# jiangzhengkai/mxdetection

Hardware: AMD Instinct MI355X
Metric: images/sec (whole node) Faster R-CNN R50-FPN 3x800x1333 (higher is better)
Workload: dtype bf16; 1 GPU; Faster R-CNN ResNet-50-FPN bf16 train step, batch 2/GPU, 3x800x1333 (padded 1344); global_batch=2, parallelism=dp1, frozen=stem+C2, frozen BN folded, optimizer=SGD momentum 0.9 wd 1e-4, launch=hipGraph replay, input=resident, wgrad_side_stream=True, rpn_branch_stream=True, grouped_wgrad=True, filter_prefetch_hints=True, params_trainable=41538304

## Files before the change

### include/mxdet.h

```cpp
#ifndef MXDET_H_
#define MXDET_H_

#include <stddef.h>
#include <stdint.h>

#ifdef __cplusplus
extern "C" {
#endif

#define MXDET_OK 0
#define MXDET_EINVAL (-1)
#define MXDET_ESHAPE (-2)
#define MXDET_EWORKSPACE (-3)
#define MXDET_EHIP (-4)
#define MXDET_ERCCL (-5)

#define MXDET_DTYPE_F32 0
#define MXDET_DTYPE_BF16 1

typedef void* mxdet_stream_t;

const char* mxdet_last_error(void);
const char* mxdet_version(void);

int mxdet_box_iou(const float* boxes_a, int64_t na, const float* boxes_b, int64_t nb, float* out,
                  mxdet_stream_t stream);

int mxdet_generate_anchors(const float* base_anchors, int32_t A, int32_t H, int32_t W, int32_t stride,
                           float* out, mxdet_stream_t stream);

size_t mxdet_nms_batched_workspace_bytes(int32_t B, int32_t n_max);
int mxdet_nms_batched(const float* boxes, const int32_t* counts, const uint8_t* invalid, int32_t B,
                      int32_t n_max, float thresh, int32_t max_keep, int32_t* keep_idx,
                      int32_t* num_keep, void* workspace, size_t workspace_bytes,
                      mxdet_stream_t stream);

size_t mxdet_detection_postprocess_workspace_bytes(int32_t N, int32_t rois_per_image, int32_t num_classes);
int mxdet_detection_postprocess(const void* cls_logits, const void* bbox_pred, int32_t dtype, int32_t ld_cls,
                                int32_t ld_reg, const float* rois, const int32_t* num_rois, const float* im_info,
                                int32_t N, int32_t rois_per_image, int32_t num_classes, const float* means,
                                const float* stds, float score_thresh, float nms_thresh, int32_t max_per_image,
                                float* dets, int32_t* num_dets, void* workspace, size_t workspace_bytes,
                                mxdet_stream_t stream);

int mxdet_soft_nms_batched(const float* boxes, const float* scores, const int32_t* counts, int32_t B, int32_t n_max,
                           int32_t method, float nms_thresh, float sigma, float min_score, int32_t max_keep,
                           int32_t* keep_idx, float* keep_scores, int32_t* num_keep, mxdet_stream_t stream);
int mxdet_detection_postprocess_soft(const void* cls_logits, const void* bbox_pred, int32_t dtype, int32_t ld_cls,
                                     int32_t ld_reg, const float* rois, const int32_t* num_rois, const float* im_info,
                                     int32_t N, int32_t rois_per_image, int32_t num_classes, const float* means,
                                     const float* stds, float score_thresh, float nms_thresh, int32_t max_per_image,
                                     float* dets, int32_t* num_dets, void* workspace, size_t workspace_bytes,
                                     int32_t method, float sigma, mxdet_stream_t stream);

typedef struct {
  int32_t num_levels;
  int32_t A;
  int32_t H[8], W[8], stride[8];
  const void* cls[8];
  const void* reg[8];
  int64_t cls_sn[8], cls_sy[8], cls_sx[8], cls_sa[8];
  int64_t reg_sn[8], reg_sy[8], reg_sx[8], reg_sc[8];
  int32_t dtype;
  int32_t classes;
  const float* base_anchors[8];
} mxdet_pyramid_t;

size_t mxdet_proposal_workspace_bytes(const mxdet_pyramid_t* p, int32_t N, int32_t pre_nms_top_n);
int mxdet_proposal(const mxdet_pyramid_t* p, int32_t N, const float* im_info ,
                   int32_t pre_nms_top_n, int32_t post_nms_top_n, float nms_thresh, float min_size,
                   float* rois, float* roi_scores, int32_t* roi_anchor, int32_t* num_rois,
                   void* workspace, size_t workspace_bytes, mxdet_stream_t stream);

size_t mxdet_anchor_target_workspace_bytes(int32_t N, int64_t A_total, int32_t G_max);
int mxdet_anchor_target(const float* anchors, int64_t A_total, const float* gt_boxes, int32_t N,
                        int32_t G_max, const float* im_info, float fg_thresh, float bg_thresh,
                        float allowed_border, int32_t batch_size, float fg_fraction, uint32_t seed,
                        uint32_t step, const uint32_t* step_dev, uint32_t image_offset, int32_t* labels,
                        int32_t* matched_gt,
                        float* bbox_targets, float* max_iou, void* workspace, size_t workspace_bytes,
                        mxdet_stream_t stream);

size_t mxdet_atss_assign_workspace_bytes(int32_t N, int64_t A_total, int32_t G_max);
int mxdet_atss_assign(const float* anchors, int64_t A_total, const int64_t* level_offsets , int32_t L,
                      const float* gt_boxes, int32_t N, int32_t G_max, int32_t topk,
                      int32_t* labels, int32_t* matched_gt, float* bbox_targets, float* matched_iou ,
                      void* workspace, size_t workspace_bytes, mxdet_stream_t stream);

int mxdet_proposal_target(const float* rois, const int32_t* num_rois, int32_t rois_stride,
                          const float* gt_boxes, int32_t N, int32_t G_max, int32_t rois_per_image,
                          float fg_fraction, float fg_thresh, float bg_hi, float bg_lo,
                          int32_t num_classes, int32_t class_agnostic,
                          const float* means , const float* stds ,
                          uint32_t seed, uint32_t step, const uint32_t* step_dev,
                          uint32_t image_offset, float* out_rois, int32_t* labels,
                          float* bbox_targets, float* bbox_weights, int32_t* matched_gt,
                          int32_t* num_fg, mxdet_stream_t stream);

int mxdet_ohem_roi_score(const void* cls_logits, const void* bbox_pred, int32_t dtype, int32_t ld_cls, int32_t ld_reg,
                         const int32_t* labels, const float* bbox_targets, const float* bbox_weights, const float* rois,
                         const int32_t* matched_gt, const float* gt_boxes, int32_t N, int32_t G_max, int64_t R,
                         int32_t num_classes, int32_t reg_dim, int32_t kind, float sigma, float std_x, float std_y,
                         float std_w, float std_h, float reg_weight, float* score, mxdet_stream_t stream);
size_t mxdet_ohem_select_workspace_bytes(int32_t N, int32_t P);
int mxdet_ohem_select(const float* score, const int32_t* labels, const float* rois, int32_t N, int32_t P, int32_t R,
                      float nms_thresh, int32_t* sel, int32_t* num_sel, int32_t* num_fg, void* workspace,
                      size_t workspace_bytes, mxdet_stream_t stream);
int mxdet_ohem_gather(const int32_t* sel, const float* pool_rois, const int32_t* pool_labels,
                      const int32_t* pool_matched_gt, const float* pool_bbox_targets, const float* pool_bbox_weights,
                      int32_t N, int32_t P, int32_t R, int32_t reg_dim, float* out_rois, int32_t* labels,
                      float* bbox_targets, float* bbox_weights, int32_t* matched_gt, mxdet_stream_t stream);

int mxdet_fpn_level_map(const float* rois, int64_t R, int32_t lvl_min, int32_t lvl_max,
                        int32_t* levels, mxdet_stream_t stream);
typedef struct {
  int32_t num_levels, lvl_min;
  int32_t H[8], W[8];
  float spatial_scale[8];
  void* feat[8];
} mxdet_feat_pyramid_t;
int mxdet_roi_align_fwd(const mxdet_feat_pyramid_t* f, int32_t N, int32_t C, const float* rois,
                        const int32_t* levels, int64_t R, int32_t PH, int32_t PW,
                        int32_t sampling_ratio, uint16_t* out, mxdet_stream_t stream);
int mxdet_roi_align_bwd(const mxdet_feat_pyramid_t* f, int32_t N, int32_t C, const float* rois,
                        const int32_t* levels, int64_t R, int32_t PH, int32_t PW,
                        int32_t sampling_ratio, const uint16_t* grad_out, mxdet_stream_t stream);
size_t mxdet_roi_align_bwd_gather_workspace_bytes(const mxdet_feat_pyramid_t* f, int32_t N, int64_t R);
int mxdet_roi_align_bwd_gather(const mxdet_feat_pyramid_t* f, int32_t N, int32_t C, const float* rois,
                               const int32_t* levels, int64_t R, int32_t PH, int32_t PW, int32_t sampling_ratio,
                               const uint16_t* grad_out, int32_t accumulate, void* workspace, size_t workspace_bytes,
                               mxdet_stream_t stream);
int mxdet_roi_align_bwd_gather_prepare(const mxdet_feat_pyramid_t* f, int32_t N, const float* rois,
                                       const int32_t* levels, int64_t R, int32_t PH, int32_t PW, int32_t sampling_ratio,
                                       void* workspace, size_t workspace_bytes, mxdet_stream_t stream);
int mxdet_roi_align_bwd_gather_prepared(const mxdet_feat_pyramid_t* f, int32_t N, int32_t C, const float* rois,
                                        const int32_t* levels, int64_t R, int32_t PH, int32_t PW, int32_t sampling_ratio,
                                        const uint16_t* grad_out, int32_t accumulate, void* workspace,
                                        size_t workspace_bytes, mxdet_stream_t stream);

typedef struct {
  mxdet_feat_pyramid_t pyr;
  int32_t N, C;
  int32_t PH, PW;
  int32_t sample_per_part;
  float trans_std;
  int32_t modulated;
  int32_t trans_stride, mask_stride;
  int32_t accumulate;
} mxdet_dpool_desc_t;
int mxdet_dpool_fwd(const mxdet_dpool_desc_t* d, const float* rois, const int32_t* levels, int64_t R,
                    const uint16_t* trans, const uint16_t* mask_logit, uint16_t* out, mxdet_stream_t stream);
int mxdet_dpool_bwd_trans(const mxdet_dpool_desc_t* d, const float* rois, const int32_t* levels, int64_t R,
                          const uint16_t* trans, const uint16_t* mask_logit, const uint16_t* dout, uint16_t* d_trans,
                          uint16_t* d_mask, mxdet_stream_t stream);
size_t mxdet_dpool_bwd_feat_workspace_bytes(const mxdet_dpool_desc_t* d, int64_t R);
int mxdet_dpool_bwd_feat(const mxdet_dpool_desc_t* d, const float* rois, const int32_t* levels, int64_t R,
                         const uint16_t* trans, const uint16_t* mask_logit, const uint16_t* dout, void* workspace,
                         size_t workspace_bytes, mxdet_stream_t stream);

int mxdet_smooth_l1_fwd(const float* pred, const float* target, const float* weight, int64_t n,
                        float sigma, float* out, mxdet_stream_t stream);
int mxdet_smooth_l1_bwd(const float* pred, const float* target, const float* weight,
                        const float* grad_out, int64_t n, float sigma, int32_t accumulate,
                        float* grad_pred, mxdet_stream_t stream);

size_t mxdet_loss_workspace_bytes(int64_t n);
int mxdet_focal_loss(const void* logits, int32_t dtype, const int32_t* labels, int64_t n, int32_t C,
                     float alpha, float gamma, float grad_scale, float* loss_out, void* grad_logits,
                     void* workspace, size_t workspace_bytes, mxdet_stream_t stream);

int mxdet_anchor_class_labels(const int32_t* labels, const int32_t* matched_gt, const float* gt_boxes, int32_t N,
                              int64_t A_total, int32_t G_max, int32_t* cls_labels, int32_t* num_fg,
                              mxdet_stream_t stream);
int32_t mxdet_retina_loss_num_partials(int32_t N, int32_t H, int32_t W, int32_t A);
int mxdet_retina_loss_level(const uint16_t* cls, const uint16_t* reg, int32_t N, int32_t H, int32_t W, int32_t A,
                            int32_t C, int32_t ld_cls, int32_t ld_reg, const int32_t* cls_labels,
                            const float* bbox_targets, int64_t A_total, int64_t level_offset, float alpha,
                            float gamma, float sigma, const int32_t* num_fg, float loss_scale, uint16_t* grad_cls,
                            uint16_t* grad_reg, float* partial, mxdet_stream_t stream);

int32_t mxdet_rpn_loss_num_partials(int32_t N, int32_t H, int32_t W);
int mxdet_rpn_loss_level(const uint16_t* head, int32_t N, int32_t H, int32_t W, int32_t A,
                         int32_t Cpad, const int32_t* labels, const float* bbox_targets,
                         int64_t A_total, int64_t level_offset, float sigma, float norm,
                         float loss_scale, uint16_t* grad_head, float* partial,
                         mxdet_stream_t stream);
int mxdet_loss_finalize(const float* partial, int32_t count, int32_t ncomp, float* out,
                        mxdet_stream_t stream);

int mxdet_rcnn_loss(const void* cls_logits, const void* bbox_pred, int32_t dtype, int32_t ld_cls,
                    int32_t ld_reg, const int32_t* labels, const float* bbox_targets,
                    const float* bbox_weights, int64_t R, int32_t num_classes, int32_t reg_dim,
                    float sigma, float norm, float loss_scale, float* loss_out, void* grad_cls,
                    void* grad_reg, void* workspace, size_t workspace_bytes, mxdet_stream_t stream);

#define MXDET_IOU_LOSS_IOU 0
#define MXDET_IOU_LOSS_GIOU 1
#define MXDET_IOU_LOSS_DIOU 2
int mxdet_box_iou_loss(const float* boxes, const float* gt, const void* deltas, int32_t dtype, int32_t ld,
                       const float* weight, int64_t n, int32_t kind, float std_x, float std_y, float std_w, float std_h,
                       float grad_scale, float* loss, void* grad_deltas, mxdet_stream_t stream);
int mxdet_rcnn_loss_iou(const void* cls_logits, const void* bbox_pred, int32_t dtype, int32_t ld_cls, int32_t ld_reg,
                        const int32_t* labels, const float* rois, const int32_t* matched_gt, const float* gt_boxes,
                        int32_t N, int32_t G_max, int64_t R, int32_t num_classes, int32_t reg_dim, int32_t kind,
                        float std_x, float std_y, float std_w, float std_h, float reg_weight, float norm, float loss_scale,
                        float* loss_out, void* grad_cls, void* grad_reg, void* workspace, size_t workspace_bytes,
                        mxdet_stream_t stream);
int mxdet_retina_loss_level_iou(const uint16_t* cls, const uint16_t* reg, int32_t N, int32_t H, int32_t W, int32_t A,
                                int32_t C, int32_t ld_cls, int32_t ld_reg, const int32_t* cls_labels, const float* anchors,
                                const int32_t* matched_gt, const float* gt_boxes, int32_t G_max, int64_t A_total,
                                int64_t level_offset, float alpha, float gamma, int32_t kind, float std_x, float std_y,
                                float std_w, float std_h, float reg_weight, const int32_t* num_fg, float loss_scale,
                                uint16_t* grad_cls, uint16_t* grad_reg, float* partial, mxdet_stream_t stream);

#define MXDET_CLS_LOSS_QFL 1
#define MXDET_CLS_LOSS_VFL 2
int mxdet_quality_focal_loss(const void* logits, int32_t dtype, const int32_t* labels, const float* quality, int64_t n,
                             int32_t C, int32_t cls_kind, float alpha, float gamma, float grad_scale, float* loss_out,
                             void* grad_logits, void* workspace, size_t workspace_bytes, mxdet_stream_t stream);
int mxdet_retina_loss_level_quality(const uint16_t* cls, const uint16_t* reg, int32_t N, int32_t H, int32_t W, int32_t A,
                                    int32_t C, int32_t ld_cls, int32_t ld_reg, const int32_t* cls_labels,
                                    const float* anchors, const int32_t* matched_gt, const float* gt_boxes, int32_t G_max,
                                    int64_t A_total, int64_t level_offset, int32_t cls_kind, float alpha, float gamma,
                                    int32_t kind, float std_x, float std_y, float std_w, float std_h, float reg_weight,
                                    const int32_t* num_fg, float loss_scale, uint16_t* grad_cls, uint16_t* grad_reg,
                                    float* partial, mxdet_stream_t stream);

#define MXDET_CLS_LOSS_FOCAL 0
#define MXDET_REG_MAX_LIMIT 31
int mxdet_box_dist_loss(const float* boxes, const float* gt, const void* logits, int32_t dtype, int32_t ld, int64_t n,
                        int32_t reg_max, float stride, int32_t kind, float reg_weight, float dfl_weight, float grad_scale,
                        float* loss_box, float* loss_dfl, float* quality, void* grad_logits, mxdet_stream_t stream);
int mxdet_retina_loss_level_dfl(const uint16_t* cls, const uint16_t* reg, int32_t N, int32_t H, int32_t W, int32_t A,
                                int32_t C, int32_t ld_cls, int32_t ld_reg, const int32_t* cls_labels, const float* anchors,
                                const int32_t* matched_gt, const float* gt_boxes, int32_t G_max, int64_t A_total,
                                int64_t level_offset, int32_t cls_kind, float alpha, float gamma, int32_t kind,
                                int32_t reg_max, float stride, float reg_weight, float dfl_weight, const int32_t* num_fg,
                                float loss_scale, uint16_t* grad_cls, uint16_t* grad_reg, float* partial,
                                mxdet_stream_t stream);

int mxdet_mask_target(const float* rois, const int32_t* matched_gt, const int32_t* labels,
                      const uint8_t* gt_masks, int64_t R, int32_t G_max, int32_t H, int32_t W, int32_t S,
                      uint8_t* targets, int32_t* cls_out, mxdet_stream_t stream);
int mxdet_pixel_shuffle2(const uint16_t* x, int64_t R, int32_t H, int32_t W, int32_t C, int32_t inverse,
                         uint16_t* y, mxdet_stream_t stream);
int mxdet_pixel_shuffle2_inv_relu(const uint16_t* dy_up, const uint16_t* act, int64_t R, int32_t H, int32_t W, int32_t C,
                                  uint16_t* dx, mxdet_stream_t stream);
size_t mxdet_mask_loss_workspace_bytes(int64_t R, int32_t S);
int mxdet_mask_loss(const uint16_t* logits, const int32_t* cls, const uint8_t* targets, int64_t R, int32_t S,
                    int32_t Cpad, float loss_scale, float* loss_out, uint16_t* grad, void* workspace,
                    size_t workspace_bytes, mxdet_stream_t stream);
size_t mxdet_mask_paste_workspace_bytes(int64_t R, int32_t S);
int mxdet_mask_paste(const uint16_t* logits, const float* dets, int64_t R, int32_t S, int32_t Cpad, int32_t H, int32_t W,
                     float thresh, uint8_t* masks, void* workspace, size_t workspace_bytes, mxdet_stream_t stream);
size_t mxdet_maskiou_target_workspace_bytes(int32_t N, int32_t G);
int mxdet_maskiou_target(const float* rois, const int32_t* matched_gt, const int32_t* cls, const float* gt_boxes,
                         const uint8_t* gt_masks, const uint16_t* logits, const uint8_t* targets, int64_t R, int32_t N,
                         int32_t G, int32_t G_boxes, int32_t H, int32_t W, int32_t S, int32_t Cpad, float* out,
                         void* workspace, size_t workspace_bytes, mxdet_stream_t stream);
int mxdet_maskiou_input(const uint16_t* mpooled, const uint16_t* logits, const int32_t* cls, int64_t R, int32_t S,
                        int32_t C, int32_t Cpad, int32_t Ctot, uint16_t* out, mxdet_stream_t stream);
int mxdet_maskiou_input_bwd(const uint16_t* d_in, int64_t pixels, int32_t C, int32_t Ctot, uint16_t* d_mpooled,
                            mxdet_stream_t stream);
int mxdet_maskiou_loss(const uint16_t* pred, const int32_t* cls, const float* targets, int64_t R, int32_t ld,
                       float loss_scale, float weight, float* loss_out, uint16_t* grad, mxdet_stream_t stream);
int mxdet_maskiou_score(const float* dets, const uint16_t* pred, int64_t R, int32_t ld, float* scores,
                        mxdet_stream_t stream);

int mxdet_keypoint_target(const float* rois, const int32_t* matched_gt, const int32_t* labels, const float* gt_keypoints,
                          int64_t R, int32_t N, int32_t G, int32_t K, int32_t S_in, int32_t* targets, mxdet_stream_t stream);
size_t mxdet_keypoint_loss_workspace_bytes(int64_t R);
int mxdet_keypoint_loss(const uint16_t* logits, const int32_t* targets, int64_t R, int32_t S_in, int32_t Kpad, int32_t K,
                        float loss_scale, float weight, float* loss_out, uint16_t* grad, void* workspace,
                        size_t workspace_bytes, mxdet_stream_t stream);
int mxdet_keypoint_decode(const uint16_t* logits, const float* dets, int64_t R, int32_t S_in, int32_t Kpad, int32_t K,
                          float* out, mxdet_stream_t stream);

typedef struct {
  int32_t N, H, W, Cin;
  int32_t Cout, KH, KW;
  int32_t stride, pad;
  int32_t Ho, Wo;
  int32_t relu;
  int32_t res_upsample;
  int32_t accumulate;
  const void* prefetch;
  int64_t prefetch_bytes;
  void* relu_bits;
} mxdet_conv_desc_t;

int mxdet_conv2d_fwd(const mxdet_conv_desc_t* d, const uint16_t* x, const uint16_t* w,
                     const float* bias, const uint16_t* residual, uint16_t* y,
                     mxdet_stream_t stream);
int mxdet_conv2d_fwd_chain(const mxdet_conv_desc_t* d, const uint16_t* x, const uint16_t* w, const float* bias,
                           const uint16_t* w2, const float* bias2, int32_t cout2, int32_t relu2,
                           const uint16_t* residual2, uint16_t* y2, const uint16_t* w3, const float* bias3,
                           int32_t cout3, int32_t relu3, uint16_t* y3, mxdet_stream_t stream);
size_t mxdet_conv2d_fwd_splitk_workspace_bytes(const mxdet_conv_desc_t* d, int32_t ksplit);
int mxdet_conv2d_fwd_splitk(const mxdet_conv_desc_t* d, const uint16_t* x, const uint16_t* w, const float* bias,
                            const uint16_t* residual, uint16_t* y, int32_t ksplit, void* workspace,
                            size_t workspace_bytes, mxdet_stream_t stream);
int mxdet_conv2d_dgrad(const mxdet_conv_desc_t* d, const uint16_t* dy, const uint16_t* wt,
                       const uint16_t* residual, const uint16_t* relu_mask, uint16_t* dx,
                       mxdet_stream_t stream);
size_t mxdet_conv2d_wgrad_workspace_bytes(const mxdet_conv_desc_t* d);
int mxdet_conv2d_wgrad(const mxdet_conv_desc_t* d, const uint16_t* x, const uint16_t* dy, float* dw,
                       float* db, void* workspace, size_t workspace_bytes, mxdet_stream_t stream);
typedef struct {
  mxdet_conv_desc_t desc;
  const void* src;
  const void* filt;
  const float* bias;
  const void* residual;
  const void* relu_mask;
  void* dst;
} mxdet_conv_item_t;
size_t mxdet_conv2d_grouped_table_bytes(int32_t n);
int mxdet_conv2d_grouped_plan(const mxdet_conv_item_t* items, int32_t n, int32_t kind, void* table_host,
                              size_t table_bytes, int32_t* cfg, int32_t* grid);
int mxdet_conv2d_grouped(const void* table_dev, int32_t n, int32_t kind, int32_t cfg, int32_t grid,
                         mxdet_stream_t stream);
typedef struct {
  mxdet_conv_desc_t desc;
  const void* x;
  const void* dy;
  float* dw;
  float* db;
} mxdet_wgrad_item_t;
size_t mxdet_conv2d_wgrad_grouped_table_bytes(int32_t n);
int mxdet_conv2d_wgrad_grouped_plan(const mxdet_wgrad_item_t* items, int32_t n, void* table_host, size_t table_bytes,
                                    size_t* workspace_bytes, int32_t* grid_wgrad, int32_t* grid_big,
                                    int32_t* grid_reduce);
int mxdet_conv2d_wgrad_grouped(const void* table_dev, int32_t n, int32_t grid_wgrad, int32_t grid_big,
                               int32_t grid_reduce, void* workspace, size_t workspace_bytes, size_t workspace_needed,
                               mxdet_stream_t stream);
int mxdet_conv2d_wgrad_grouped_parts(const void* table_dev, int32_t n, int32_t grid_wgrad, int32_t grid_big,
                                     int32_t grid_reduce, int32_t parts, void* workspace, size_t workspace_bytes,
                                     size_t workspace_needed, mxdet_stream_t stream);
int mxdet_filter_transpose(const uint16_t* w, int32_t Cout, int32_t KH, int32_t KW, int32_t Cin,
                           uint16_t* wt, mxdet_stream_t stream);

int mxdet_filter_transpose_batched(const void* descs_dev, int32_t ndesc, int32_t total_tiles,
                                   mxdet_stream_t stream);

#define MXDET_RPN_SPARSE_MAX_LEVELS 8
#define MXDET_RPN_SPARSE_ZERO 1
#define MXDET_RPN_SPARSE_DT 2
#define MXDET_RPN_SPARSE_WGRAD 4
#define MXDET_RPN_SPARSE_DGRAD 8
#define MXDET_RPN_SPARSE_DTMAP 16
#define MXDET_RPN_SPARSE_WGRAD_ORDERED 32
#define MXDET_RPN_ORDERED_WORK_INTS(smax) (10 * (smax) + 32)
typedef struct {
  int32_t kind;
  int32_t H, W;
  int32_t halves_per_slab;
  int32_t slab0;
  int32_t fold_ksplit;
  int32_t bias_pixels;
  int32_t bias_splits;
} mxdet_rpn_ordered_item_t;
typedef struct {
  int32_t num_levels, N, A, C, Ch, smax;
  int32_t H[MXDET_RPN_SPARSE_MAX_LEVELS], W[MXDET_RPN_SPARSE_MAX_LEVELS];
  int32_t accumulate[MXDET_RPN_SPARSE_MAX_LEVELS];
  const void* P[MXDET_RPN_SPARSE_MAX_LEVELS];
  const void* t[MXDET_RPN_SPARSE_MAX_LEVELS];
  const void* tbits[MXDET_RPN_SPARSE_MAX_LEVELS];
  const void* gh[MXDET_RPN_SPARSE_MAX_LEVELS];
  void* dP[MXDET_RPN_SPARSE_MAX_LEVELS];
  void* dt[MXDET_RPN_SPARSE_MAX_LEVELS];
  const mxdet_rpn_ordered_item_t* ordered;
  void* ordered_work;
} mxdet_rpn_sparse_t;
int mxdet_rpn_sparse_list(const mxdet_rpn_sparse_t* d, const int32_t* labels, int32_t* list, int32_t* state,
                          int32_t* map, mxdet_stream_t stream);
int mxdet_rpn_sparse_backward(const mxdet_rpn_sparse_t* d, const int32_t* list, const int32_t* state,
                              const int32_t* map, const uint16_t* wt_out, const uint16_t* wt_conv, uint16_t* dts,
                              uint16_t* ghs, float* dw_out, float* db_out, float* dw_conv, float* db_conv,
                              int32_t parts, mxdet_stream_t stream);
int mxdet_rpn_ordered_schedule(const void* table_host, int32_t n, int32_t num_levels, mxdet_rpn_ordered_item_t* items);

typedef struct {
  int32_t N, H, W, C;
  int32_t Ho, Wo;
  int32_t KH, KW;
  int32_t stride, pad;
  int32_t groups;
  int32_t modulated;
  int32_t off_channels;
  int32_t accumulate;
} mxdet_deform_desc_t;
int mxdet_deform_im2col(const mxdet_deform_desc_t* d, const uint16_t* x, const uint16_t* off, uint16_t* col,
                        mxdet_stream_t stream);
int mxdet_deform_col2im_coord(const mxdet_deform_desc_t* d, const uint16_t* x, const uint16_t* off,
                              const uint16_t* dcol, uint16_t* doff, mxdet_stream_t stream);
size_t mxdet_deform_col2im_workspace_bytes(const mxdet_deform_desc_t* d);
int mxdet_deform_col2im(const mxdet_deform_desc_t* d, const uint16_t* off, const uint16_t* dcol, uint16_t* dx,
                        void* workspace, size_t workspace_bytes, mxdet_stream_t stream);

typedef struct {
  int32_t N, HW, C, G;
  float eps;
  int32_t relu;
  int32_t accumulate;
} mxdet_gn_desc_t;
size_t mxdet_group_norm_workspace_bytes(const mxdet_gn_desc_t* d, int32_t backward);
int mxdet_group_norm_fwd(const mxdet_gn_desc_t* d, const uint16_t* x, const float* gamma, const float* beta, uint16_t* y,
                         float* mean, float* rstd, void* workspace, size_t workspace_bytes, mxdet_stream_t stream);
int mxdet_group_norm_bwd(const mxdet_gn_desc_t* d, const uint16_t* x, const uint16_t* dy, const uint16_t* y,
                         const float* mean, const float* rstd, const float* gamma, const float* beta, uint16_t* dx,
                         float* dgamma, float* dbeta, void* workspace, size_t workspace_bytes, mxdet_stream_t stream);

int mxdet_stem_conv7x7(const void* image, int32_t dtype, int32_t N, int32_t H, int32_t W,
                       const uint16_t* w, const float* bias, uint16_t* y, mxdet_stream_t stream);
int mxdet_stem_conv7x7_pool(const void* image, int32_t dtype, int32_t N, int32_t H, int32_t W,
                            const uint16_t* w, const float* bias, uint16_t* y, mxdet_stream_t stream);
int mxdet_maxpool3x3s2(const uint16_t* x, int32_t N, int32_t H, int32_t W, int32_t C, uint16_t* y,
                       mxdet_stream_t stream);
int mxdet_subsample2(const uint16_t* x, int32_t N, int32_t H, int32_t W, int32_t C, uint16_t* y,
                     mxdet_stream_t stream);
int mxdet_subsample2_bwd(const uint16_t* dy, int32_t N, int32_t H, int32_t W, int32_t C,
                         int32_t accumulate, uint16_t* dx, mxdet_stream_t stream);
int mxdet_upsample2_bwd(const uint16_t* dfine, int32_t N, int32_t Hf, int32_t Wf, int32_t C,
                        int32_t accumulate, uint16_t* dcoarse, mxdet_stream_t stream);
size_t mxdet_retina_detect_workspace_bytes(const mxdet_pyramid_t* p, int32_t N, int32_t pre_nms_top_n);
int mxdet_retina_detect(const mxdet_pyramid_t* p, int32_t N, const float* im_info, int32_t pre_nms_top_n,
                        float score_thresh, float nms_thresh, int32_t max_per_image, float* dets, int32_t* num_dets,
                        void* workspace, size_t workspace_bytes, mxdet_stream_t stream);
int mxdet_retina_detect_soft(const mxdet_pyramid_t* p, int32_t N, const float* im_info, int32_t pre_nms_top_n,
                             float score_thresh, float nms_thresh, int32_t max_per_image, float* dets,
                             int32_t* num_dets, void* workspace, size_t workspace_bytes, int32_t method, float sigma,
                             mxdet_stream_t stream);
int mxdet_retina_detect_dfl(const mxdet_pyramid_t* p, int32_t N, const float* im_info, int32_t pre_nms_top_n,
                            float score_thresh, float nms_thresh, int32_t max_per_image, float* dets, int32_t* num_dets,
                            void* workspace, size_t workspace_bytes, int32_t method, float sigma, int32_t reg_max,
                            mxdet_stream_t stream);

typedef struct {
  const uint8_t* src;
  int32_t src_h, src_w;
  int32_t dst_h, dst_w;
  int32_t flip;
  int32_t pad_;
  double inv_scale;
} mxdet_image_desc_t;
#define MXDET_PREPROCESS_MAX_BATCH 64
int mxdet_image_preprocess(const mxdet_image_desc_t* images , int32_t N, int32_t Hp, int32_t Wp,
                           const float* mean3 , const float* std3 , int32_t swap_rb,
                           uint16_t* out, mxdet_stream_t stream);

int mxdet_polygon_masks(const float* verts, const int32_t* poly_start, const int32_t* inst_first, int32_t N,
                        int32_t G, int32_t H, int32_t W, uint8_t* masks, mxdet_stream_t stream);

int mxdet_add_bf16(const uint16_t* a, const uint16_t* b, int64_t n, uint16_t* out,
                   mxdet_stream_t stream);
int mxdet_relu_bwd_bf16(const uint16_t* dy, const uint16_t* y, int64_t n, uint16_t* dx,
                        mxdet_stream_t stream);
int mxdet_f32_to_bf16(const float* x, int64_t n, uint16_t* y, mxdet_stream_t stream);
int mxdet_f32_accum_to_bf16(const float* x, int64_t n, int32_t accumulate, uint16_t* y,
                            mxdet_stream_t stream);
int mxdet_nchw_to_nhwc_bf16(const void* x, int32_t dtype, int32_t N, int32_t C, int32_t H, int32_t W,
                            uint16_t* y, mxdet_stream_t stream);
int mxdet_nhwc_to_nchw_f32(const uint16_t* x, int32_t N, int32_t C, int32_t H, int32_t W, float* y,
                           mxdet_stream_t stream);

int mxdet_sgd_momentum_update(float* w, const float* grad, float* mom, uint16_t* w_bf16, int64_t n,
                              float lr, float momentum, float wd, float rescale,
                              mxdet_stream_t stream);
int mxdet_sgd_momentum_update_sched(float* w, const float* grad, float* mom, uint16_t* w_bf16, int64_t n,
                                    const float* lr_dev, float momentum, float wd, float rescale,
                                    mxdet_stream_t stream);

typedef struct mxdet_comm mxdet_comm_t;
#define MXDET_COMM_ID_BYTES 128
#define MXDET_COMM_MAX_INFLIGHT 64
int mxdet_comm_unique_id(uint8_t* id );
int mxdet_comm_create(const uint8_t* id, int32_t world, int32_t rank, mxdet_comm_t** comm_out);
int mxdet_comm_destroy(mxdet_comm_t* comm);
int mxdet_allreduce_bucket(mxdet_comm_t* comm, float* grad, int64_t count, mxdet_stream_t stream,
                           int32_t* ticket_out);
int mxdet_comm_wait(mxdet_comm_t* comm, int32_t ticket, mxdet_stream_t stream);
int mxdet_comm_broadcast(mxdet_comm_t* comm, void* buf, size_t bytes, int32_t root, mxdet_stream_t stream);

#ifdef __cplusplus
}
#endif
#endif
```

### mxdetection_amd/_lib.py

```python
import ctypes as C
import os

_HERE = os.path.dirname(os.path.abspath(__file__))
LIB_PATH = os.environ.get("MXDET_LIB") or os.path.join(_HERE, "libmxdet_hip.so")

c_i32, c_i64, c_u32, c_f32, c_sz, c_vp = C.c_int32, C.c_int64, C.c_uint32, C.c_float, C.c_size_t, C.c_void_p


class PyramidT(C.Structure):
    _fields_ = [
        ("num_levels", c_i32), ("A", c_i32),
        ("H", c_i32 * 8), ("W", c_i32 * 8), ("stride", c_i32 * 8),
        ("cls", c_vp * 8), ("reg", c_vp * 8),
        ("cls_sn", c_i64 * 8), ("cls_sy", c_i64 * 8), ("cls_sx", c_i64 * 8), ("cls_sa", c_i64 * 8),
        ("reg_sn", c_i64 * 8), ("reg_sy", c_i64 * 8), ("reg_sx", c_i64 * 8), ("reg_sc", c_i64 * 8),
        ("dtype", c_i32), ("classes", c_i32),
        ("base_anchors", c_vp * 8),
    ]


class FeatPyramidT(C.Structure):
    _fields_ = [
        ("num_levels", c_i32), ("lvl_min", c_i32),
        ("H", c_i32 * 8), ("W", c_i32 * 8),
        ("spatial_scale", c_f32 * 8),
        ("feat", c_vp * 8),
    ]


class ImageDescT(C.Structure):
    _fields_ = [("src", C.c_void_p), ("src_h", C.c_int32), ("src_w", C.c_int32), ("dst_h", C.c_int32),
                ("dst_w", C.c_int32), ("flip", C.c_int32), ("pad_", C.c_int32), ("inv_scale", C.c_double)]


class WgradItemT(C.Structure):
    pass


class ConvItemT(C.Structure):
    pass


class ConvDescT(C.Structure):
    _fields_ = [
        ("N", c_i32), ("H", c_i32), ("W", c_i32), ("Cin", c_i32),
        ("Cout", c_i32), ("KH", c_i32), ("KW", c_i32),
        ("stride", c_i32), ("pad", c_i32),
        ("Ho", c_i32), ("Wo", c_i32),
        ("relu", c_i32), ("res_upsample", c_i32), ("accumulate", c_i32),
        ("prefetch", c_vp), ("prefetch_bytes", c_i64), ("relu_bits", c_vp),
    ]


class DeformDescT(C.Structure):
    _fields_ = [
        ("N", c_i32), ("H", c_i32), ("W", c_i32), ("C", c_i32),
        ("Ho", c_i32), ("Wo", c_i32), ("KH", c_i32), ("KW", c_i32),
        ("stride", c_i32), ("pad", c_i32), ("groups", c_i32), ("modulated", c_i32),
        ("off_channels", c_i32), ("accumulate", c_i32),
    ]


class DpoolDescT(C.Structure):
    _fields_ = [
        ("pyr", FeatPyramidT), ("N", c_i32), ("C", c_i32), ("PH", c_i32), ("PW", c_i32),
        ("sample_per_part", c_i32), ("trans_std", c_f32), ("modulated", c_i32),
        ("trans_stride", c_i32), ("mask_stride", c_i32), ("accumulate", c_i32),
    ]


class GnDescT(C.Structure):
    _fields_ = [("N", c_i32), ("HW", c_i32), ("C", c_i32), ("G", c_i32), ("eps", c_f32), ("relu", c_i32),
                ("accumulate", c_i32)]


class RpnOrderedItemT(C.Structure):
    _fields_ = [("kind", c_i32), ("H", c_i32), ("W", c_i32), ("halves_per_slab", c_i32), ("slab0", c_i32),
                ("fold_ksplit", c_i32), ("bias_pixels", c_i32), ("bias_splits", c_i32)]


class RpnSparseT(C.Structure):
    _fields_ = [("num_levels", c_i32), ("N", c_i32), ("A", c_i32), ("C", c_i32), ("Ch", c_i32), ("smax", c_i32),
                ("H", c_i32 * 8), ("W", c_i32 * 8), ("accumulate", c_i32 * 8),
                ("P", c_vp * 8), ("t", c_vp * 8), ("tbits", c_vp * 8), ("gh", c_vp * 8), ("dP", c_vp * 8), ("dt", c_vp * 8),
                ("ordered", C.POINTER(RpnOrderedItemT)), ("ordered_work", c_vp)]


WgradItemT._fields_ = [("desc", ConvDescT), ("x", c_vp), ("dy", c_vp), ("dw", c_vp), ("db", c_vp)]
ConvItemT._fields_ = [("desc", ConvDescT), ("src", c_vp), ("filt", c_vp), ("bias", c_vp), ("residual", c_vp),
                      ("relu_mask", c_vp), ("dst", c_vp)]

P = C.POINTER

SIGNATURES = {
    "mxdet_last_error": (C.c_char_p, []),
    "mxdet_version": (C.c_char_p, []),
    "mxdet_box_iou": (c_i32, [c_vp, c_i64, c_vp, c_i64, c_vp, c_vp]),
    "mxdet_generate_anchors": (c_i32, [c_vp, c_i32, c_i32, c_i32, c_i32, c_vp, c_vp]),
    "mxdet_nms_batched_workspace_bytes": (c_sz, [c_i32, c_i32]),
    "mxdet_nms_batched": (c_i32, [c_vp, c_vp, c_vp, c_i32, c_i32, c_f32, c_i32, c_vp, c_vp, c_vp, c_sz, c_vp]),
    "mxdet_soft_nms_batched": (c_i32, [c_vp, c_vp, c_vp, c_i32, c_i32, c_i32, c_f32, c_f32, c_f32, c_i32, c_vp, c_vp, c_vp,
                                       c_vp]),
    "mxdet_pixel_shuffle2_inv_relu": (c_i32, [c_vp, c_vp, c_i64, c_i32, c_i32, c_i32, c_vp, c_vp]),
    "mxdet_mask_paste_workspace_bytes": (c_sz, [c_i64, c_i32]),
    "mxdet_mask_paste": (c_i32, [c_vp, c_vp, c_i64, c_i32, c_i32, c_i32, c_i32, c_f32, c_vp, c_vp, c_sz, c_vp]),
    "mxdet_retina_detect_workspace_bytes": (c_sz, [c_vp, c_i32, c_i32]),
    "mxdet_retina_detect": (c_i32, [c_vp, c_i32, c_vp, c_i32, c_f32, c_f32, c_i32, c_vp, c_vp, c_vp, c_sz, c_vp]),
    "mxdet_retina_detect_soft": (c_i32, [c_vp, c_i32, c_vp, c_i32, c_f32, c_f32, c_i32, c_vp, c_vp, c_vp, c_sz, c_i32, c_f32,
                                         c_vp]),
    "mxdet_retina_detect_dfl": (c_i32, [c_vp, c_i32, c_vp, c_i32, c_f32, c_f32, c_i32, c_vp, c_vp, c_vp, c_sz, c_i32, c_f32,
                                        c_i32, c_vp]),
    "mxdet_debug_preprocess_direct": (c_i32, [c_i32]),
    "mxdet_image_preprocess": (c_i32, [c_vp, c_i32, c_i32, c_i32, c_vp, c_vp, c_i32, c_vp, c_vp]),
    "mxdet_polygon_masks": (c_i32, [c_vp, c_vp, c_vp, c_i32, c_i32, c_i32, c_i32, c_vp, c_vp]),
    "mxdet_detection_postprocess_workspace_bytes": (c_sz, [c_i32, c_i32, c_i32]),
    "mxdet_detection_postprocess": (c_i32, [c_vp, c_vp, c_i32, c_i32, c_i32, c_vp, c_vp, c_vp, c_i32, c_i32, c_i32,
                                            P(c_f32), P(c_f32), c_f32, c_f32, c_i32, c_vp, c_vp, c_vp, c_sz, c_vp]),
    "mxdet_detection_postprocess_soft": (c_i32, [c_vp, c_vp, c_i32, c_i32, c_i32, c_vp, c_vp, c_vp, c_i32, c_i32, c_i32,
                                                 P(c_f32), P(c_f32), c_f32, c_f32, c_i32, c_vp, c_vp, c_vp, c_sz, c_i32,
                                                 c_f32, c_vp]),
    "mxdet_proposal_workspace_bytes": (c_sz, [P(PyramidT), c_i32, c_i32]),
    "mxdet_proposal": (c_i32, [P(PyramidT), c_i32, c_vp, c_i32, c_i32, c_f32, c_f32, c_vp, c_vp, c_vp, c_vp,
                               c_vp, c_sz, c_vp]),
    "mxdet_anchor_target_workspace_bytes": (c_sz, [c_i32, c_i64, c_i32]),
    "mxdet_anchor_target": (c_i32, [c_vp, c_i64, c_vp, c_i32, c_i32, c_vp, c_f32, c_f32, c_f32, c_i32, c_f32,
                                    c_u32, c_u32, c_vp, c_u32, c_vp, c_vp, c_vp, c_vp, c_vp, c_sz, c_vp]),
    "mxdet_atss_assign_workspace_bytes": (c_sz, [c_i32, c_i64, c_i32]),
    "mxdet_atss_assign": (c_i32, [c_vp, c_i64, P(c_i64), c_i32, c_vp, c_i32, c_i32, c_i32, c_vp, c_vp, c_vp, c_vp, c_vp, c_sz,
                                  c_vp]),
    "mxdet_proposal_target": (c_i32, [c_vp, c_vp, c_i32, c_vp, c_i32, c_i32, c_i32, c_f32, c_f32, c_f32, c_f32,
                                      c_i32, c_i32, P(c_f32), P(c_f32), c_u32, c_u32, c_vp, c_u32, c_vp, c_vp, c_vp,
                                      c_vp, c_vp, c_vp, c_vp]),
    "mxdet_ohem_roi_score": (c_i32, [c_vp, c_vp, c_i32, c_i32, c_i32, c_vp, c_vp, c_vp, c_vp, c_vp, c_vp, c_i32, c_i32, c_i64,
                                     c_i32, c_i32, c_i32, c_f32, c_f32, c_f32, c_f32, c_f32, c_f32, c_vp, c_vp]),
    "mxdet_ohem_select_workspace_bytes": (c_sz, [c_i32, c_i32]),
    "mxdet_ohem_select": (c_i32, [c_vp, c_vp, c_vp, c_i32, c_i32, c_i32, c_f32, c_vp, c_vp, c_vp, c_vp, c_sz, c_vp]),
    "mxdet_ohem_gather": (c_i32, [c_vp, c_vp, c_vp, c_vp, c_vp, c_vp, c_i32, c_i32, c_i32, c_i32, c_vp, c_vp, c_vp, c_vp,
                                  c_vp, c_vp]),
    "mxdet_fpn_level_map": (c_i32, [c_vp, c_i64, c_i32, c_i32, c_vp, c_vp]),
    "mxdet_roi_align_fwd": (c_i32, [P(FeatPyramidT), c_i32, c_i32, c_vp, c_vp, c_i64, c_i32, c_i32, c_i32, c_vp,
                                    c_vp]),
    "mxdet_roi_align_bwd": (c_i32, [P(FeatPyramidT), c_i32, c_i32, c_vp, c_vp, c_i64, c_i32, c_i32, c_i32, c_vp,
                                    c_vp]),
    "mxdet_roi_align_bwd_gather_workspace_bytes": (c_sz, [P(FeatPyramidT), c_i32, c_i64]),
    "mxdet_roi_align_bwd_gather": (c_i32, [P(FeatPyramidT), c_i32, c_i32, c_vp, c_vp, c_i64, c_i32, c_i32, c_i32, c_vp,
                                           c_i32, c_vp, c_sz, c_vp]),
    "mxdet_roi_align_bwd_gather_prepare": (c_i32, [P(FeatPyramidT), c_i32, c_vp, c_vp, c_i64, c_i32, c_i32, c_i32,
                                                   c_vp, c_sz, c_vp]),
    "mxdet_roi_align_bwd_gather_prepared": (c_i32, [P(FeatPyramidT), c_i32, c_i32, c_vp, c_vp, c_i64, c_i32, c_i32, c_i32,
                                                    c_vp, c_i32, c_vp, c_sz, c_vp]),
    "mxdet_smooth_l1_fwd": (c_i32, [c_vp, c_vp, c_vp, c_i64, c_f32, c_vp, c_vp]),
    "mxdet_smooth_l1_bwd": (c_i32, [c_vp, c_vp, c_vp, c_vp, c_i64, c_f32, c_i32, c_vp, c_vp]),
    "mxdet_loss_workspace_bytes": (c_sz, [c_i64]),
    "mxdet_focal_loss": (c_i32, [c_vp, c_i32, c_vp, c_i64, c_i32, c_f32, c_f32, c_f32, c_vp, c_vp, c_vp, c_sz,
                                 c_vp]),
    "mxdet_anchor_class_labels": (c_i32, [c_vp, c_vp, c_vp, c_i32, c_i64, c_i32, c_vp, c_vp, c_vp]),
    "mxdet_retina_loss_num_partials": (c_i32, [c_i32, c_i32, c_i32, c_i32]),
    "mxdet_retina_loss_level": (c_i32, [c_vp, c_vp, c_i32, c_i32, c_i32, c_i32, c_i32, c_i32, c_i32, c_vp, c_vp, c_i64,
                                        c_i64, c_f32, c_f32, c_f32, c_vp, c_f32, c_vp, c_vp, c_vp, c_vp]),
    "mxdet_rpn_loss_num_partials": (c_i32, [c_i32, c_i32, c_i32]),
    "mxdet_rpn_loss_level": (c_i32, [c_vp, c_i32, c_i32, c_i32, c_i32, c_i32, c_vp, c_vp, c_i64, c_i64, c_f32,
                                     c_f32, c_f32, c_vp, c_vp, c_vp]),
    "mxdet_loss_finalize": (c_i32, [c_vp, c_i32, c_i32, c_vp, c_vp]),
    "mxdet_rcnn_loss": (c_i32, [c_vp, c_vp, c_i32, c_i32, c_i32, c_vp, c_vp, c_vp, c_i64, c_i32, c_i32, c_f32,
                                c_f32, c_f32, c_vp, c_vp, c_vp, c_vp, c_sz, c_vp]),
    "mxdet_box_iou_loss": (c_i32, [c_vp, c_vp, c_vp, c_i32, c_i32, c_vp, c_i64, c_i32, c_f32, c_f32, c_f32, c_f32, c_f32, c_vp,
                                   c_vp, c_vp]),
    "mxdet_rcnn_loss_iou": (c_i32, [c_vp, c_vp, c_i32, c_i32, c_i32, c_vp, c_vp, c_vp, c_vp, c_i32, c_i32, c_i64, c_i32, c_i32,
                                    c_i32, c_f32, c_f32, c_f32, c_f32, c_f32, c_f32, c_f32, c_vp, c_vp, c_vp, c_vp, c_sz,
                                    c_vp]),
    "mxdet_retina_loss_level_iou": (c_i32, [c_vp, c_vp, c_i32, c_i32, c_i32, c_i32, c_i32, c_i32, c_i32, c_vp, c_vp, c_vp, c_vp,
                                            c_i32, c_i64, c_i64, c_f32, c_f32, c_i32, c_f32, c_f32, c_f32, c_f32, c_f32, c_vp,
                                            c_f32, c_vp, c_vp, c_vp, c_vp]),
    "mxdet_quality_focal_loss": (c_i32, [c_vp, c_i32, c_vp, c_vp, c_i64, c_i32, c_i32, c_f32, c_f32, c_f32, c_vp, c_vp, c_vp, c_sz,
                                         c_vp]),
    "mxdet_retina_loss_level_quality": (c_i32, [c_vp, c_vp, c_i32, c_i32, c_i32, c_i32, c_i32, c_i32, c_i32, c_vp, c_vp, c_vp,
                                                c_vp, c_i32, c_i64, c_i64, c_i32, c_f32, c_f32, c_i32, c_f32, c_f32, c_f32, c_f32,
                                                c_f32, c_vp, c_f32, c_vp, c_vp, c_vp, c_vp]),
    "mxdet_box_dist_loss": (c_i32, [c_vp, c_vp, c_vp, c_i32, c_i32, c_i64, c_i32, c_f32, c_i32, c_f32, c_f32, c_f32, c_vp, c_vp,
                                    c_vp, c_vp, c_vp]),
    "mxdet_retina_loss_level_dfl": (c_i32, [c_vp, c_vp, c_i32, c_i32, c_i32, c_i32, c_i32, c_i32, c_i32, c_vp, c_vp, c_vp, c_vp,
                                            c_i32, c_i64, c_i64, c_i32, c_f32, c_f32, c_i32, c_i32, c_f32, c_f32, c_f32, c_vp,
                                            c_f32, c_vp, c_vp, c_vp, c_vp]),
    "mxdet_mask_target": (c_i32, [c_vp, c_vp, c_vp, c_vp, c_i64, c_i32, c_i32, c_i32, c_i32, c_vp, c_vp, c_vp]),
    "mxdet_pixel_shuffle2": (c_i32, [c_vp, c_i64, c_i32, c_i32, c_i32, c_i32, c_vp, c_vp]),
    "mxdet_mask_loss_workspace_bytes": (c_sz, [c_i64, c_i32]),
    "mxdet_mask_loss": (c_i32, [c_vp, c_vp, c_vp, c_i64, c_i32, c_i32, c_f32, c_vp, c_vp, c_vp, c_sz, c_vp]),
    "mxdet_maskiou_target_workspace_bytes": (c_sz, [c_i32, c_i32]),
    "mxdet_maskiou_target": (c_i32, [c_vp, c_vp, c_vp, c_vp, c_vp, c_vp, c_vp, c_i64, c_i32, c_i32, c_i32, c_i32, c_i32, c_i32,
                                     c_i32, c_vp, c_vp, c_sz, c_vp]),
    "mxdet_maskiou_input": (c_i32, [c_vp, c_vp, c_vp, c_i64, c_i32, c_i32, c_i32, c_i32, c_vp, c_vp]),
    "mxdet_maskiou_input_bwd": (c_i32, [c_vp, c_i64, c_i32, c_i32, c_vp, c_vp]),
    "mxdet_maskiou_loss": (c_i32, [c_vp, c_vp, c_vp, c_i64, c_i32, c_f32, c_f32, c_vp, c_vp, c_vp]),
    "mxdet_maskiou_score": (c_i32, [c_vp, c_vp, c_i64, c_i32, c_vp, c_vp]),
    "mxdet_keypoint_target": (c_i32, [c_vp, c_vp, c_vp, c_vp, c_i64, c_i32, c_i32, c_i32, c_i32, c_vp, c_vp]),
    "mxdet_keypoint_loss_workspace_bytes": (c_sz, [c_i64]),
    "mxdet_keypoint_loss": (c_i32, [c_vp, c_vp, c_i64, c_i32, c_i32, c_i32, c_f32, c_f32, c_vp, c_vp, c_vp, c_sz, c_vp]),
    "mxdet_keypoint_decode": (c_i32, [c_vp, c_vp, c_i64, c_i32, c_i32, c_i32, c_vp, c_vp]),
    "mxdet_conv2d_fwd": (c_i32, [P(ConvDescT), c_vp, c_vp, c_vp, c_vp, c_vp, c_vp]),
    "mxdet_conv2d_fwd_chain": (c_i32, [P(ConvDescT), c_vp, c_vp, c_vp, c_vp, c_vp, c_i32, c_i32, c_vp, c_vp, c_vp, c_vp, c_i32,
                                       c_i32, c_vp, c_vp]),
    "mxdet_conv2d_fwd_splitk_workspace_bytes": (c_sz, [P(ConvDescT), c_i32]),
    "mxdet_conv2d_fwd_splitk": (c_i32, [P(ConvDescT), c_vp, c_vp, c_vp, c_vp, c_vp, c_i32, c_vp, c_sz, c_vp]),
    "mxdet_conv2d_dgrad": (c_i32, [P(ConvDescT), c_vp, c_vp, c_vp, c_vp, c_vp, c_vp]),
    "mxdet_conv2d_wgrad_workspace_bytes": (c_sz, [P(ConvDescT)]),
    "mxdet_conv2d_wgrad": (c_i32, [P(ConvDescT), c_vp, c_vp, c_vp, c_vp, c_vp, c_sz, c_vp]),
    "mxdet_conv2d_grouped_table_bytes": (c_sz, [c_i32]),
    "mxdet_conv2d_grouped_plan": (c_i32, [P(ConvItemT), c_i32, c_i32, c_vp, c_sz, P(c_i32), P(c_i32)]),
    "mxdet_conv2d_grouped": (c_i32, [c_vp, c_i32, c_i32, c_i32, c_i32, c_vp]),
    "mxdet_conv2d_wgrad_grouped_table_bytes": (c_sz, [c_i32]),
    "mxdet_conv2d_wgrad_grouped_plan": (c_i32, [P(WgradItemT), c_i32, c_vp, c_sz, P(c_sz), P(c_i32), P(c_i32), P(c_i32)]),
    "mxdet_conv2d_wgrad_grouped": (c_i32, [c_vp, c_i32, c_i32, c_i32, c_i32, c_vp, c_sz, c_sz, c_vp]),
    "mxdet_conv2d_wgrad_grouped_parts": (c_i32, [c_vp, c_i32, c_i32, c_i32, c_i32, c_i32, c_vp, c_sz, c_sz, c_vp]),
    "mxdet_debug_force_conv_cfg": (c_i32, [c_i32]),
    "mxdet_debug_force_wgrad_ksplit": (c_i32, [c_i32]),
    "mxdet_rpn_sparse_list": (c_i32, [P(RpnSparseT), c_vp, c_vp, c_vp, c_vp, c_vp]),
    "mxdet_rpn_sparse_backward": (c_i32, [P(RpnSparseT), c_vp, c_vp, c_vp, c_vp, c_vp, c_vp, c_vp, c_vp, c_vp, c_vp, c_vp,
                                          c_i32, c_vp]),
    "mxdet_rpn_ordered_schedule": (c_i32, [c_vp, c_i32, c_i32, P(RpnOrderedItemT)]),
    "mxdet_filter_transpose": (c_i32, [c_vp, c_i32, c_i32, c_i32, c_i32, c_vp, c_vp]),
    "mxdet_filter_transpose_batched": (c_i32, [c_vp, c_i32, c_i32, c_vp]),
    "mxdet_deform_im2col": (c_i32, [P(DeformDescT), c_vp, c_vp, c_vp, c_vp]),
    "mxdet_deform_col2im_coord": (c_i32, [P(DeformDescT), c_vp, c_vp, c_vp, c_vp, c_vp]),
    "mxdet_deform_col2im_workspace_bytes": (c_sz, [P(DeformDescT)]),
    "mxdet_deform_col2im": (c_i32, [P(DeformDescT), c_vp, c_vp, c_vp, c_vp, c_sz, c_vp]),
    "mxdet_dpool_fwd": (c_i32, [P(DpoolDescT), c_vp, c_vp, c_i64, c_vp, c_vp, c_vp, c_vp]),
    "mxdet_dpool_bwd_trans": (c_i32, [P(DpoolDescT), c_vp, c_vp, c_i64, c_vp, c_vp, c_vp, c_vp, c_vp, c_vp]),
    "mxdet_dpool_bwd_feat_workspace_bytes": (c_sz, [P(DpoolDescT), c_i64]),
    "mxdet_dpool_bwd_feat": (c_i32, [P(DpoolDescT), c_vp, c_vp, c_i64, c_vp, c_vp, c_vp, c_vp, c_sz, c_vp]),
    "mxdet_group_norm_workspace_bytes": (c_sz, [P(GnDescT), c_i32]),
    "mxdet_group_norm_fwd": (c_i32, [P(GnDescT), c_vp, c_vp, c_vp, c_vp, c_vp, c_vp, c_vp, c_sz, c_vp]),
    "mxdet_group_norm_bwd": (c_i32, [P(GnDescT), c_vp, c_vp, c_vp, c_vp, c_vp, c_vp, c_vp, c_vp, c_vp, c_vp, c_vp, c_sz,
                                     c_vp]),
    "mxdet_debug_group_norm_route": (c_i32, [P(GnDescT)]),
    "mxdet_stem_conv7x7": (c_i32, [c_vp, c_i32, c_i32, c_i32, c_i32, c_vp, c_vp, c_vp, c_vp]),
    "mxdet_stem_conv7x7_pool": (c_i32, [c_vp, c_i32, c_i32, c_i32, c_i32, c_vp, c_vp, c_vp, c_vp]),
    "mxdet_maxpool3x3s2": (c_i32, [c_vp, c_i32, c_i32, c_i32, c_i32, c_vp, c_vp]),
    "mxdet_subsample2": (c_i32, [c_vp, c_i32, c_i32, c_i32, c_i32, c_vp, c_vp]),
    "mxdet_subsample2_bwd": (c_i32, [c_vp, c_i32, c_i32, c_i32, c_i32, c_i32, c_vp, c_vp]),
    "mxdet_upsample2_bwd": (c_i32, [c_vp, c_i32, c_i32, c_i32, c_i32, c_i32, c_vp, c_vp]),
    "mxdet_add_bf16": (c_i32, [c_vp, c_vp, c_i64, c_vp, c_vp]),
    "mxdet_relu_bwd_bf16": (c_i32, [c_vp, c_vp, c_i64, c_vp, c_vp]),
    "mxdet_f32_to_bf16": (c_i32, [c_vp, c_i64, c_vp, c_vp]),
    "mxdet_f32_accum_to_bf16": (c_i32, [c_vp, c_i64, c_i32, c_vp, c_vp]),
    "mxdet_nchw_to_nhwc_bf16": (c_i32, [c_vp, c_i32, c_i32, c_i32, c_i32, c_i32, c_vp, c_vp]),
    "mxdet_nhwc_to_nchw_f32": (c_i32, [c_vp, c_i32, c_i32, c_i32, c_i32, c_vp, c_vp]),
    "mxdet_sgd_momentum_update": (c_i32, [c_vp, c_vp, c_vp, c_vp, c_i64, c_f32, c_f32, c_f32, c_f32, c_vp]),
    "mxdet_sgd_momentum_update_sched": (c_i32, [c_vp, c_vp, c_vp, c_vp, c_i64, c_vp, c_f32, c_f32, c_f32, c_vp]),
    "mxdet_comm_unique_id": (c_i32, [c_vp]),
    "mxdet_comm_create": (c_i32, [c_vp, c_i32, c_i32, P(c_vp)]),
    "mxdet_comm_destroy": (c_i32, [c_vp]),
    "mxdet_allreduce_bucket": (c_i32, [c_vp, c_vp, c_i64, c_vp, P(c_i32)]),
    "mxdet_comm_wait": (c_i32, [c_vp, c_i32, c_vp]),
    "mxdet_comm_broadcast": (c_i32, [c_vp, c_vp, c_sz, c_i32, c_vp]),
    "mxdet_debug_set_tuning": (c_i32, [c_i32, c_i64]),
    "mxdet_debug_get_tuning": (c_i64, [c_i32]),
    "mxdet_debug_route_probe": (c_i32, [c_i32]),
    "mxdet_debug_route_read": (c_i32, [P(c_i32), c_i32]),
}

DEBUG_SYMBOLS = ("mxdet_debug_force_conv_cfg", "mxdet_debug_force_wgrad_ksplit", "mxdet_debug_preprocess_direct",
                 "mxdet_debug_set_tuning", "mxdet_debug_get_tuning", "mxdet_debug_route_probe", "mxdet_debug_route_read",
                 "mxdet_debug_group_norm_route")
TUNING_KEYS = {"T64": 0, "T128": 1, "PAR64": 2, "WG_TARGET": 3, "WG_MINSTEPS": 4, "WG_MAXSTEPS": 5, "T3_ENABLE": 6,
               "T3_TARGET": 7, "T3_MINSTEPS": 8, "T3_NS": 9, "TAIL": 10, "WG_NS": 11, "ROI_TABLE": 12, "ROI_ROWS": 13, "STATIC_TAPS": 14,
               "T128W": 15, "T3_MIX": 16, "SPLITK_TILE": 17, "T3_PER_ITEM": 18}
ROUTE_KINDS = {"CONV": 1, "WGRAD": 2, "CONV_GROUPED": 3, "WGRAD_GROUPED": 4, "RETINA_LOSS": 5, "RETINA_LOSS_IOU": 6,
               "RETINA_LOSS_QUALITY": 7, "RETINA_LOSS_DFL": 8}

IOU_LOSS_KINDS = {"iou": 0, "giou": 1, "diou": 2}
CLS_LOSS_KINDS = {"qfl": 1, "vfl": 2}
CLS_LOSS_KINDS_DFL = {"focal": 0, "qfl": 1, "vfl": 2}
REG_MAX_LIMIT = 31

_lib = None


class MxdetError(RuntimeError):
    pass


def load():
    global _lib
    if _lib is not None:
        return _lib
    if not os.path.exists(LIB_PATH):
        raise MxdetError(
            "libmxdet_hip.so not found at %s -- build it with `python -m mxdetection_amd.build` "
            "(there is no CPU fallback)" % LIB_PATH)
    import torch
    lib = C.CDLL(LIB_PATH)
    for name, (res, args) in SIGNATURES.items():
        fn = getattr(lib, name, None)
        if fn is None:
            continue
        fn.restype = res
        fn.argtypes = args
    _lib = lib
    for key, idx in TUNING_KEYS.items():
        v = os.environ.get("MXDET_TUNE_" + key)
        if v:
            lib.mxdet_debug_set_tuning(idx, int(v))
    return lib


def check(rc, what=""):
    if rc != 0:
        msg = load().mxdet_last_error().decode("utf-8", "replace")
        raise MxdetError("%s failed (%d): %s" % (what or "mxdet call", rc, msg))


def ptr(t):
    return None if t is None else C.c_void_p(t.data_ptr())


def stream_ptr():
    import torch
    return C.c_void_p(torch.cuda.current_stream().cuda_stream)
```

### mxdetection_amd/csrc/conv.hip

```cpp
#include <stdlib.h>

#include "common.h"

namespace mxdet {

struct ConvP {
  const uint16_t* x;
  const uint16_t* w;
  const float* bias;
  const uint16_t* res;
  const uint16_t* mask;
  uint16_t* y;
  int N, Hs, Ws, C;
  int Hd, Wd, Ncols;
  int KH, KW, stride, pad;
  int relu, res_up;
  int M;
  int tiles_m, tiles_n;
  int par_tile0[5];
  int par_hc[2], par_wc[2];
  int par_h0[2], par_w0[2];
  int m_begin;
  int ksplit;
  float* partial;
  const void* pf;
  long long pf_bytes;
  unsigned char* bits_out;
  const unsigned char* bits_in;
  int force_cfg;
  const uint16_t* chain_w;
  const float* chain_bias;
  const uint16_t* chain_res;
  uint16_t* chain_y;
  int chain_relu;
  const uint16_t* chain3_w;
  const float* chain3_bias;
  uint16_t* chain3_y;
  int chain3_relu;
};

__device__ __forceinline__ int lds_off(int row, int chunk) {
  return row * 64 + ((chunk ^ ((row >> 1) & 7)) << 3);
}

#ifdef MXDET_CONV_STAMP
__device__ unsigned long long g_conv_stamp[2][8];
#define MXDET_CS(k) do { if (cs_on) cs[k] = __builtin_amdgcn_s_memtime(); } while (0)
#else
#define MXDET_CS(k) do { } while (0)
#endif

template <int BM, int BN, int WM, int WN, int NS, bool DGRAD, bool PAR = false, int TAPS = 0, int CHAIN = 0>
__device__ __forceinline__ void conv_igemm_tile(const ConvP& p, int bid, const int nwg) {
  constexpr int NW = WM * WN, NTHR = 64 * NW;
  constexpr int WTM = BM / WM, WTN = BN / WN;
  constexpr int MT = WTM / 16, NT = WTN / 16;
  constexpr int RPI = 8;
  constexpr int GA = BM / RPI / NW, GB = BN / RPI / NW;
  constexpr int STAGE = (BM + BN) * 64;
  static_assert(BM % (RPI * NW) == 0 && BN % (RPI * NW) == 0, "rows must split evenly over the waves");
  static_assert(MT % 2 == 0, "epilogue stages two m-tiles at a time");
  static_assert(NS >= 2 && (NS - 2) * (GA + GB) <= 63, "vmcnt is a 6-bit counter");
  static_assert(TAPS == 0 || ((TAPS == 1 || TAPS == 9) && !PAR), "static taps: 1x1 or 3x3");
  constexpr int EP_STRIDE = WTN + 4;
  constexpr int EP_BYTES = NW * 32 * EP_STRIDE * 4;
  constexpr int MAIN_BYTES = NS * STAGE * 2;
  static_assert(CHAIN == 0 || (TAPS == 9 && !DGRAD && WN == 1 && BN == 64 && CHAIN % (8 * NW) == 0),
                "chain: forward 3x3 whose waves own all 64 mid channels of their rows");
  constexpr int CHAIN_OFF = MAIN_BYTES > EP_BYTES ? MAIN_BYTES : EP_BYTES;
  constexpr int SMEM_BYTES = CHAIN_OFF + CHAIN * 128;
  __shared__ __attribute__((aligned(1024))) unsigned char smem_raw[SMEM_BYTES];
  uint16_t* smem = (uint16_t*)smem_raw;

  const int tid = threadIdx.x, lane = tid & 63;
  const int wid = __builtin_amdgcn_readfirstlane(tid >> 6);
  const int wm = wid / WN, wn = wid % WN;
#ifdef MXDET_CONV_STAMP
  const bool cs_on = (blockIdx.x == 0 || blockIdx.x == 300) && wid == 0;
  unsigned long long cs[8] = {0, 0, 0, 0, 0, 0, 0, 0};
#endif
  MXDET_CS(0);

  const int pf_bid = bid, pf_nwg = nwg;
  int ks = 0, sl_begin = 0, sl_end = p.C >> 6;
  int nwg_ = nwg;
  if constexpr (TAPS == 1) {
    if (p.ksplit > 1) {
      const int tiles = p.tiles_m * p.tiles_n;
      ks = bid / tiles;
      bid -= ks * tiles;
      nwg_ = tiles;
      const int per = ((p.C >> 6) + p.ksplit - 1) / p.ksplit;
      sl_begin = ks * per;
      sl_end = sl_begin + per < sl_end ? sl_begin + per : sl_end;
      sl_end = sl_end < sl_begin ? sl_begin : sl_end;
    }
  }
  if constexpr (!PAR) {
    bid = xcd_tile_order(bid, nwg_);
  }
  const int tile_m = bid / p.tiles_n, tile_n = bid - tile_m * p.tiles_n;
  int m0 = p.m_begin + tile_m * BM;
  const int n0 = tile_n * BN;
  int par_ph = 0, par_pw = 0, par_rows = 0, par_hc = 1, par_wc = 1, nkh = p.KH, nkw = p.KW;
  if constexpr (PAR) {
    int c = 0;
    while (c < 3 && tile_m >= p.par_tile0[c + 1]) ++c;
    par_ph = c >> 1; par_pw = c & 1;
    par_hc = p.par_hc[par_ph]; par_wc = p.par_wc[par_pw];
    par_rows = p.N * par_hc * par_wc;
    m0 = (tile_m - p.par_tile0[c]) * BM;
    nkh = (p.KH - par_ph + 1) >> 1; nkw = (p.KW - par_pw + 1) >> 1;
    nkh = nkh < 0 ? 0 : nkh; nkw = nkw < 0 ? 0 : nkw;
  }

  const int lrow = lane >> 3, lslot = lane & 7;
  constexpr int SWZ = 7;
  const __amdgpu_buffer_rsrc_t rsrc_x = make_rsrc(p.x, 2u * (unsigned)(p.N * p.Hs * p.Ws) * (unsigned)p.C);
  const __amdgpu_buffer_rsrc_t rsrc_w = make_rsrc(p.w, 2u * (unsigned)p.Ncols * (unsigned)(p.KH * p.KW * p.C));
  const int ntaps = p.KH * p.KW;
  const int hw_d = p.Hd * p.Wd;
  const bool smallm = p.M < (1 << 24);
  const float rcp_hw = 1.0f / (float)hw_d, rcp_w = 1.0f / (float)p.Wd;
  const int Ktot = ntaps * p.C;
  const int KT = PAR ? (nkh * nkw * p.C) >> 6 : Ktot >> 6;
  int wrow[GB];
#pragma unroll
  for (int i = 0; i < GB; ++i) {
    int rb = (wid * GB + i) * RPI + lrow;
    int n = n0 + rb;
    n = n < p.Ncols ? n : p.Ncols - 1;
    wrow[i] = n * Ktot + ((lslot ^ ((rb >> 1) & SWZ)) << 3);
  }
  auto issue_b = [&](int buf, int tap, int c0, bool live) {
    const int so_b = live ? 2 * (tap * p.C + c0) : 0;
    unsigned char* sbase = smem_raw + (size_t)buf * (STAGE * 2);
#pragma unroll
    for (int i = 0; i < GB; ++i)
#if !defined(MXDET_ABL_NOLOAD) && !defined(MXDET_ABL_NOBLOAD)
      __builtin_amdgcn_raw_ptr_buffer_load_lds(rsrc_w, (lptr_t)(sbase + BM * 128 + (wid * GB + i) * 1024), 16,
                                               (int)(2u * (unsigned)wrow[i]), so_b, 0, 0);
#else
      asm volatile("" ::"v"(wrow[i]), "s"(so_b));
#endif
  };
  if constexpr (TAPS > 0) {
#pragma unroll
    for (int s0 = 0; s0 < NS - 1; ++s0)
      issue_b(s0, s0 % TAPS, (sl_begin + s0 / TAPS) * 64, s0 < (sl_end - sl_begin) * TAPS);
  }
  if constexpr (CHAIN > 0) {
    const __amdgpu_buffer_rsrc_t rsrc_c = make_rsrc(p.chain_w, 2u * (unsigned)CHAIN * 64u);
#pragma unroll
    for (int i = 0; i < CHAIN / 8 / NW; ++i) {
      const int r = (wid * (CHAIN / 8 / NW) + i) * 8 + lrow;
      const unsigned vo = 2u * (unsigned)(r * 64 + ((lslot ^ ((r >> 1) & 7)) << 3));
      __builtin_amdgcn_raw_ptr_buffer_load_lds(rsrc_c, (lptr_t)(smem_raw + CHAIN_OFF + (wid * (CHAIN / 8 / NW) + i) * 1024), 16,
                                               (int)vo, 0, 0, 0);
    }
  }
  int a_off[GA];
  unsigned a_mask[GA];
#pragma unroll
  for (int i = 0; i < GA; ++i) {
    int ra = (wid * GA + i) * RPI + lrow;
    int m = m0 + ra;
    int coff = (lslot ^ ((ra >> 1) & SWZ)) << 3;
    unsigned mask = 0;
    int off = 0;
    if constexpr (PAR) {
      if (m < par_rows) {
        int img = m / (par_hc * par_wc);
        int rem = m - img * (par_hc * par_wc);
        int ih = rem / par_wc, iw = rem - ih * par_wc;
        int hd = p.par_h0[par_ph] + 2 * ih, wd = p.par_w0[par_pw] + 2 * iw;
        int hs0 = (hd + p.pad - par_ph) >> 1, ws0 = (wd + p.pad - par_pw) >> 1;
        off = ((img * p.Hs + hs0) * p.Ws + ws0) * p.C + coff;
        for (int a = 0; a < nkh; ++a)
          for (int b = 0; b < nkw; ++b) {
            int hs = hs0 - a, ws = ws0 - b;
            if (hs >= 0 && ws >= 0 && hs < p.Hs && ws < p.Ws) mask |= 1u << (a * nkw + b);
          }
      }
    } else if (ntaps == 1 && p.stride == 1 && p.pad == 0) {
      if (m < p.M) { off = m * p.C + coff; mask = 1u; }
    } else
    if (m < p.M) {
      int img, hd, wd, rem;
      if (smallm) {
        img = fast_divmod(m, hw_d, rcp_hw, &rem);
        hd = fast_divmod(rem, p.Wd, rcp_w, &wd);
      } else {
        img = m / hw_d; rem = m - img * hw_d;
        hd = rem / p.Wd; wd = rem - hd * p.Wd;
      }
      int h0, w0;
      if (DGRAD) {
        if (p.stride == 1) { h0 = hd + p.pad; w0 = wd + p.pad; }
        else { h0 = (hd + p.pad) / p.stride; w0 = (wd + p.pad) / p.stride; }
      } else { h0 = hd * p.stride - p.pad; w0 = wd * p.stride - p.pad; }
      off = ((img * p.Hs + h0) * p.Ws + w0) * p.C + coff;
      if (DGRAD && p.stride != 1) {
        for (int kh = 0; kh < p.KH; ++kh)
          for (int kw = 0; kw < p.KW; ++kw) {
            int th = hd + p.pad - kh, tw = wd + p.pad - kw;
            int hs = th / p.stride, ws = tw / p.stride;
            bool ok = th >= 0 && tw >= 0 && th == hs * p.stride && tw == ws * p.stride && hs < p.Hs && ws < p.Ws;
            if (ok) mask |= 1u << (kh * p.KW + kw);
          }
      } else if (TAPS == 9) {
        const unsigned rlo = (DGRAD ? h0 < p.Hs : h0 >= 0) ? 1u : 0u, rhi = (DGRAD ? h0 - 2 >= 0 : h0 + 2 < p.Hs) ? 4u : 0u;
        const unsigned clo = (DGRAD ? w0 < p.Ws : w0 >= 0) ? 1u : 0u, chi = (DGRAD ? w0 - 2 >= 0 : w0 + 2 < p.Ws) ? 4u : 0u;
        const unsigned rowm = rlo | 2u | rhi, colm = clo | 2u | chi;
        mask = ((rowm & 1u) ? colm : 0u) | (colm << 3) | ((rowm & 4u) ? colm << 6 : 0u);
      } else {
        unsigned rowm = 0, colm = 0;
        for (int kh = 0; kh < p.KH; ++kh) {
          const int hs = DGRAD ? h0 - kh : h0 + kh;
          if (hs >= 0 && hs < p.Hs) rowm |= 1u << kh;
        }
        for (int kw = 0; kw < p.KW; ++kw) {
          const int ws = DGRAD ? w0 - kw : w0 + kw;
          if (ws >= 0 && ws < p.Ws) colm |= 1u << kw;
        }
        for (int kh = 0; kh < p.KH; ++kh)
          if ((rowm >> kh) & 1u) mask |= colm << (kh * p.KW);
      }
    }
    a_off[i] = off;
    a_mask[i] = mask;
  }

  int ld_kt = 0, ld_kh = 0, ld_kw = 0, ld_c0 = 0;
  auto issue_stage = [&](int buf) {
    unsigned char* sbase = smem_raw + (size_t)buf * (STAGE * 2);
    const bool live = ld_kt < KT;
    int tap, delta, koff;
    if constexpr (PAR) {
      tap = live ? ld_kh * nkw + ld_kw : 31;
      delta = ld_c0 - (ld_kh * p.Ws + ld_kw) * p.C;
      koff = live ? ((par_ph + 2 * ld_kh) * p.KW + (par_pw + 2 * ld_kw)) * p.C + ld_c0 : 0;
    } else {
      tap = live ? ld_kh * p.KW + ld_kw : 31;
      if (DGRAD) delta = ld_c0 - ((ld_kh / p.stride) * p.Ws + (ld_kw / p.stride)) * p.C;
      else delta = ld_c0 + (ld_kh * p.Ws + ld_kw) * p.C;
      koff = live ? (ld_kh * p.KW + ld_kw) * p.C + ld_c0 : 0;
    }
#pragma unroll
    for (int i = 0; i < GA; ++i) {
      unsigned vo = ((a_mask[i] >> tap) & 1u) ? 2u * (unsigned)(a_off[i] + delta) : kDmaOob;
#ifdef MXDET_ABL_ZEROSRC
      vo = kDmaOob;
#endif
#ifndef MXDET_ABL_NOLOAD
      __builtin_amdgcn_raw_ptr_buffer_load_lds(rsrc_x, (lptr_t)(sbase + (wid * GA + i) * 1024), 16, (int)vo, 0, 0, 0);
#else
      asm volatile("" ::"v"(vo));
#endif
    }
#pragma unroll
    for (int i = 0; i < GB; ++i) {
      unsigned wo = 2u * (unsigned)(wrow[i] + koff);
#ifdef MXDET_ABL_ZEROSRC
      wo = kDmaOob;
#endif
#ifndef MXDET_ABL_NOLOAD
      __builtin_amdgcn_raw_ptr_buffer_load_lds(rsrc_w, (lptr_t)(sbase + BM * 128 + (wid * GB + i) * 1024), 16, (int)wo, 0, 0, 0);
#else
      asm volatile("" ::"v"(wo));
#endif
    }
    ++ld_kt;
    if (++ld_kw == nkw) {
      ld_kw = 0;
      if (++ld_kh == nkh) { ld_kh = 0; ld_c0 += 64; }
    }
  };

  f32x4_t acc[MT][NT];
#pragma unroll
  for (int i = 0; i < MT; ++i)
#pragma unroll
    for (int j = 0; j < NT; ++j) acc[i][j] = (f32x4_t){0.f, 0.f, 0.f, 0.f};
  MXDET_CS(1);

  const int frow = lane & 15, fq = lane >> 4;
  if constexpr (TAPS > 0) {
  constexpr int TKW = TAPS == 9 ? 3 : 1;
  constexpr int SL = (NS % TAPS == 0 || TAPS % NS == 0) ? (TAPS % NS == 0 ? 1 : NS) : NS;
  static_assert((SL * TAPS) % NS == 0, "the ring position must repeat with the unrolled block");
  const int bias_el = (p.pad * p.Ws + p.pad) * p.C;
  const int rebase = DGRAD ? ((p.KH - 1) * p.Ws + (p.KW - 1)) * p.C : 0;
  const __amdgpu_buffer_rsrc_t rsrc_xs =
      make_rsrc(p.x - bias_el, 2u * (unsigned)(p.N * p.Hs * p.Ws) * (unsigned)p.C + 2u * (unsigned)bias_el);
  unsigned voa[GA];
#pragma unroll
  for (int i = 0; i < GA; ++i) {
    voa[i] = 2u * (unsigned)(a_off[i] - rebase + bias_el);
    if (TAPS == 1) voa[i] = (a_mask[i] & 1u) ? voa[i] : kDmaOob;
  }
  auto issue_a = [&](int buf, int tap, int c0, bool live) {
    const int kh = tap / TKW, kw = tap % TKW;
    const int disp = DGRAD ? ((p.KH - 1 - kh) * p.Ws + (p.KW - 1 - kw)) * p.C : (kh * p.Ws + kw) * p.C;
    const int so_a = live ? 2 * (disp + c0) : 0;
    unsigned char* sbase = smem_raw + (size_t)buf * (STAGE * 2);
#pragma unroll
    for (int i = 0; i < GA; ++i) {
      unsigned vo = voa[i];
      if (TAPS != 1) vo = ((a_mask[i] >> tap) & 1u) ? vo : kDmaOob;
      if (!live) vo = kDmaOob;
#ifndef MXDET_ABL_NOLOAD
      __builtin_amdgcn_raw_ptr_buffer_load_lds(rsrc_xs, (lptr_t)(sbase + (wid * GA + i) * 1024), 16, (int)vo, so_a, 0, 0);
#else
      asm volatile("" ::"v"(vo), "s"(so_a));
#endif
    }
  };
  const uint16_t* fa0 = smem + lds_off(wm * WTM + frow, fq);
  const uint16_t* fa1 = smem + lds_off(wm * WTM + frow, 4 + fq);
  const uint16_t* fb0 = smem + BM * 64 + lds_off(wn * WTN + frow, fq);
  const uint16_t* fb1 = smem + BM * 64 + lds_off(wn * WTN + frow, 4 + fq);
  const int nslices = sl_end;
#pragma unroll
  for (int s0 = 0; s0 < NS - 1; ++s0)
    issue_a(s0, s0 % TAPS, (sl_begin + s0 / TAPS) * 64, s0 < (sl_end - sl_begin) * TAPS);
  asm volatile("s_waitcnt vmcnt(%0)" ::"n"((NS - 2) * GA) : "memory");
#ifdef MXDET_ABL_NOBFRAG
  bf16x8_t bf0[NT], bf1[NT];
#pragma unroll
  for (int j = 0; j < NT; ++j) { bf0[j] = *(const bf16x8_t*)(fb0 + j * 1024); bf1[j] = *(const bf16x8_t*)(fb1 + j * 1024); }
#endif
#ifdef MXDET_ABL_NOKLOOP
  for (int cs = sl_begin; cs < sl_begin; cs += SL) {
#else
  for (int cs = sl_begin; cs < nslices; cs += SL) {
#endif
#pragma unroll
    for (int sl = 0; sl < SL; ++sl) {
      if (SL > 1 && cs + sl >= nslices) break;
#pragma unroll
      for (int tp = 0; tp < TAPS; ++tp) {
        const int step = sl * TAPS + tp;
        const int cur = step % NS, nxt = (step + NS - 1) % NS;
        asm volatile("s_waitcnt vmcnt(%0)" ::"n"((NS - 2) * (GA + GB)) : "memory");
        __builtin_amdgcn_s_barrier();
        asm volatile("" ::: "memory");
#ifdef MXDET_ABL_NOBFRAG
        bf16x8_t af0[MT], af1[MT];
#else
        bf16x8_t af0[MT], bf0[NT], af1[MT], bf1[NT];
#endif
#pragma unroll
        for (int i = 0; i < MT; ++i) af0[i] = *(const bf16x8_t*)(fa0 + cur * STAGE + i * 1024);
#ifndef MXDET_ABL_NOBFRAG
#pragma unroll
        for (int j = 0; j < NT; ++j) bf0[j] = *(const bf16x8_t*)(fb0 + cur * STAGE + j * 1024);
#endif
#pragma unroll
        for (int i = 0; i < MT; ++i) af1[i] = *(const bf16x8_t*)(fa1 + cur * STAGE + i * 1024);
#ifndef MXDET_ABL_NOBFRAG
#pragma unroll
        for (int j = 0; j < NT; ++j) bf1[j] = *(const bf16x8_t*)(fb1 + cur * STAGE + j * 1024);
#endif
        __builtin_amdgcn_sched_barrier(0);
        {
          const int ahead = tp + NS - 1;
          const int atap = ahead % TAPS, aslice = ahead / TAPS;
          issue_a(nxt, atap, (cs + sl + aslice) * 64, cs + sl + aslice < nslices);
          issue_b(nxt, atap, (cs + sl + aslice) * 64, cs + sl + aslice < nslices);
        }
        __builtin_amdgcn_sched_barrier(0);
        __builtin_amdgcn_s_setprio(1);
#ifndef MXDET_ABL_NOMFMA
#pragma unroll
        for (int i = 0; i < MT; ++i)
#pragma unroll
          for (int j = 0; j < NT; ++j)
            acc[i][j] = __builtin_amdgcn_mfma_f32_16x16x32_bf16(af0[i], bf0[j], acc[i][j], 0, 0, 0);
#pragma unroll
        for (int i = 0; i < MT; ++i)
#pragma unroll
          for (int j = 0; j < NT; ++j)
            acc[i][j] = __builtin_amdgcn_mfma_f32_16x16x32_bf16(af1[i], bf1[j], acc[i][j], 0, 0, 0);
#else
#pragma unroll
        for (int i = 0; i < MT; ++i) { asm volatile("" ::"v"(af0[i])); asm volatile("" ::"v"(af1[i])); }
#pragma unroll
        for (int j = 0; j < NT; ++j) { asm volatile("" ::"v"(bf0[j])); asm volatile("" ::"v"(bf1[j])); }
#endif
        __builtin_amdgcn_sched_barrier(0);
        __builtin_amdgcn_s_setprio(0);
      }
    }
  }
  } else {
#pragma unroll
  for (int s0 = 0; s0 < NS - 1; ++s0) issue_stage(s0);

  int cur = 0, nxt = NS - 1;
  for (int kt = 0; kt < KT; ++kt) {
    asm volatile("s_waitcnt vmcnt(%0)" ::"n"((NS - 2) * (GA + GB)) : "memory");
    __builtin_amdgcn_s_barrier();
    asm volatile("" ::: "memory");
#ifdef MXDET_CONV_STAMP
    if (kt == 0) MXDET_CS(2);
#endif
    const uint16_t* sa = smem + cur * STAGE;
    const uint16_t* sb = sa + BM * 64;
    bf16x8_t af0[MT], bf0[NT], af1[MT], bf1[NT];
#pragma unroll
    for (int i = 0; i < MT; ++i) af0[i] = *(const bf16x8_t*)(sa + lds_off(wm * WTM + i * 16 + frow, fq));
#pragma unroll
    for (int j = 0; j < NT; ++j) bf0[j] = *(const bf16x8_t*)(sb + lds_off(wn * WTN + j * 16 + frow, fq));
    issue_stage(nxt);
    __builtin_amdgcn_s_setprio(1);
    __builtin_amdgcn_sched_barrier(0);
#pragma unroll
    for (int i = 0; i < MT; ++i) af1[i] = *(const bf16x8_t*)(sa + lds_off(wm * WTM + i * 16 + frow, 4 + fq));
#pragma unroll
    for (int j = 0; j < NT; ++j) bf1[j] = *(const bf16x8_t*)(sb + lds_off(wn * WTN + j * 16 + frow, 4 + fq));
#ifndef MXDET_ABL_NOMFMA
#pragma unroll
    for (int i = 0; i < MT; ++i)
#pragma unroll
      for (int j = 0; j < NT; ++j)
        acc[i][j] = __builtin_amdgcn_mfma_f32_16x16x32_bf16(af0[i], bf0[j], acc[i][j], 0, 0, 0);
#pragma unroll
    for (int g = 0; g < MT + NT; ++g) {
      __builtin_amdgcn_sched_group_barrier(0x008, (MT * NT) / (MT + NT), 0);
      __builtin_amdgcn_sched_group_barrier(0x100, 1, 0);
    }
#pragma unroll
    for (int i = 0; i < MT; ++i)
#pragma unroll
      for (int j = 0; j < NT; ++j)
        acc[i][j] = __builtin_amdgcn_mfma_f32_16x16x32_bf16(af1[i], bf1[j], acc[i][j], 0, 0, 0);
#else
#pragma unroll
    for (int i = 0; i < MT; ++i) { asm volatile("" ::"v"(af0[i])); asm volatile("" ::"v"(af1[i])); }
#pragma unroll
    for (int j = 0; j < NT; ++j) { asm volatile("" ::"v"(bf0[j])); asm volatile("" ::"v"(bf1[j])); }
#endif
    __builtin_amdgcn_sched_barrier(0);
    __builtin_amdgcn_s_setprio(0);
    cur = (cur + 1 == NS) ? 0 : cur + 1;
    nxt = (nxt + 1 == NS) ? 0 : nxt + 1;
  }
  }
  MXDET_CS(3);
  asm volatile("s_waitcnt vmcnt(0)" ::: "memory");
  __syncthreads();
  MXDET_CS(4);

  uint4 pfv[4] = {make_uint4(0u, 0u, 0u, 0u), make_uint4(0u, 0u, 0u, 0u), make_uint4(0u, 0u, 0u, 0u), make_uint4(0u, 0u, 0u, 0u)};
  if (p.pf != nullptr) {
    const long long pf_stride = (long long)pf_nwg * NTHR * 16;
    long long off = ((long long)pf_bid * NTHR + tid) * 16;
#pragma unroll
    for (int k = 0; k < 4; ++k, off += pf_stride)
      if (off + 16 <= p.pf_bytes) pfv[k] = *(const uint4*)((const char*)p.pf + off);
  }

  float* ep = (float*)smem_raw + wid * 32 * EP_STRIDE;
  constexpr int LPR = WTN / 8;
  constexpr int RPP = 64 / LPR;
  constexpr int PASSES = 32 / RPP;
  const int rl = lane / LPR, cg = lane - rl * LPR;
  bf16x8_t af2[CHAIN > 0 ? MT : 1][2];
  if constexpr (CHAIN > 0) {
#pragma unroll
    for (int i = 0; i < MT; ++i)
#pragma unroll
      for (int j = 0; j < NT; ++j)
#pragma unroll
        for (int r = 0; r < 4; ++r)
          ep[(i * 16 + fq * 4 + r) * EP_STRIDE + j * 16 + frow] = acc[i][j][r];
#pragma unroll
    for (int hf = 0; hf < 2; ++hf) {
      float4 c0 = make_float4(0.f, 0.f, 0.f, 0.f), c1 = c0;
      if (p.bias) {
        c0 = *(const float4*)(p.bias + hf * 32 + fq * 8);
        c1 = *(const float4*)(p.bias + hf * 32 + fq * 8 + 4);
      }
#pragma unroll
      for (int i = 0; i < MT; ++i) {
        const float4 v0 = *(const float4*)(ep + (i * 16 + frow) * EP_STRIDE + hf * 32 + fq * 8);
        const float4 v1 = *(const float4*)(ep + (i * 16 + frow) * EP_STRIDE + hf * 32 + fq * 8 + 4);
        float v[8] = {v0.x + c0.x, v0.y + c0.y, v0.z + c0.z, v0.w + c0.w, v1.x + c1.x, v1.y + c1.y, v1.z + c1.z, v1.w + c1.w};
        if (p.relu) {
#pragma unroll
          for (int k = 0; k < 8; ++k) v[k] = v[k] > 0.0f ? v[k] : 0.0f;
        }
        af2[i][hf] = __builtin_bit_cast(bf16x8_t, pack8_bf16_hw(v));
      }
    }
  }
  static_assert(CHAIN == 0 || MT == 2, "chain: one epilogue half covers the wave's rows");
  constexpr int NCH = CHAIN > 0 ? CHAIN / BN : 1;
  const bool c3 = CHAIN > 0 && p.chain3_w != nullptr;
  f32x4_t acc3[CHAIN > 0 ? MT : 1][CHAIN > 0 ? NT : 1];
  if constexpr (CHAIN > 0) {
#pragma unroll
    for (int i = 0; i < MT; ++i)
#pragma unroll
      for (int j = 0; j < NT; ++j) acc3[i][j] = f32x4_t{0.f, 0.f, 0.f, 0.f};
  }
#pragma unroll 1
  for (int chunk = 0; chunk < (CHAIN > 0 ? NCH + (c3 ? 1 : 0) : 1); ++chunk) {
  const bool last3 = CHAIN > 0 && chunk == NCH;
  const int e_ncols = CHAIN > 0 ? (last3 ? BN : CHAIN) : p.Ncols;
  const float* const e_bias = CHAIN > 0 ? (last3 ? p.chain3_bias : p.chain_bias) : p.bias;
  const uint16_t* const e_res = CHAIN > 0 ? (last3 ? nullptr : p.chain_res) : p.res;
  uint16_t* const e_y = CHAIN > 0 ? (last3 ? p.chain3_y : p.chain_y) : p.y;
  const int e_relu = CHAIN > 0 ? (last3 ? p.chain3_relu : p.chain_relu) : p.relu;
  const int n0c = CHAIN > 0 ? (last3 ? 0 : chunk * BN) : n0;
  if constexpr (CHAIN > 0) {
    if (last3) {
#pragma unroll
      for (int i = 0; i < MT; ++i)
#pragma unroll
        for (int j = 0; j < NT; ++j) acc[i][j] = acc3[i][j];
    }
  }
  bf16x8_t b3[2][CHAIN > 0 ? NT : 1];
  if constexpr (CHAIN > 0) {
    if (c3 && !last3) {
#pragma unroll
      for (int hf = 0; hf < 2; ++hf)
#pragma unroll
        for (int j = 0; j < NT; ++j)
          b3[hf][j] = *(const bf16x8_t*)(p.chain3_w + (size_t)(j * 16 + frow) * CHAIN + chunk * BN + hf * 32 + fq * 8);
    }
  }
  if (CHAIN > 0 && !last3) {
    const uint16_t* wl = (const uint16_t*)(smem_raw + CHAIN_OFF);
#pragma unroll
    for (int i = 0; i < MT; ++i)
#pragma unroll
      for (int j = 0; j < NT; ++j) acc[i][j] = f32x4_t{0.f, 0.f, 0.f, 0.f};
#pragma unroll
    for (int hf = 0; hf < 2; ++hf) {
      bf16x8_t bw[NT];
#pragma unroll
      for (int j = 0; j < NT; ++j) bw[j] = *(const bf16x8_t*)(wl + lds_off(n0c + j * 16 + frow, hf * 4 + fq));
#pragma unroll
      for (int i = 0; i < MT; ++i)
#pragma unroll
        for (int j = 0; j < NT; ++j)
          acc[i][j] = __builtin_amdgcn_mfma_f32_16x16x32_bf16(af2[i][hf], bw[j], acc[i][j], 0, 0, 0);
    }
  }
  const int col = n0c + wn * WTN + cg * 8;
  const bool colok = col < e_ncols;
  float4 b0 = make_float4(0.f, 0.f, 0.f, 0.f), b1 = b0;
  if (e_bias) {
    const int cb = colok ? col : 0;
    b0 = *(const float4*)(e_bias + cb);
    b1 = *(const float4*)(e_bias + cb + 4);
  }
#pragma unroll
  for (int h = 0; h < MT / 2; ++h) {
    size_t pixs[PASSES];
    bool oks[PASSES];
    uint4 rres[PASSES], rmsk[PASSES];
#pragma unroll
    for (int ps = 0; ps < PASSES; ++ps) {
      const int row = ps * RPP + rl;
      const int m = m0 + wm * WTM + h * 32 + row;
      bool rowok = m < p.M;
      size_t pix = (size_t)m;
      if constexpr (PAR) {
        rowok = m < par_rows;
        int img = m / (par_hc * par_wc);
        int rem = m - img * (par_hc * par_wc);
        int ih = rem / par_wc, iw = rem - ih * par_wc;
        pix = (size_t)(img * p.Hd + p.par_h0[par_ph] + 2 * ih) * p.Wd + (p.par_w0[par_pw] + 2 * iw);
      }
      oks[ps] = rowok && colok;
      pixs[ps] = oks[ps] ? pix : 0;
    }
    if (e_res) {
#pragma unroll
      for (int ps = 0; ps < PASSES; ++ps) {
        size_t ri = pixs[ps] * e_ncols + (oks[ps] ? col : 0);
        if (CHAIN == 0 && p.res_up) {
          const int m = (int)pixs[ps];
          int img = m / (p.Hd * p.Wd);
          int rem = m - img * (p.Hd * p.Wd);
          int hd = rem / p.Wd, wd = rem - hd * p.Wd;
          int Hc = (p.Hd + 1) >> 1, Wc = (p.Wd + 1) >> 1;
          ri = ((size_t)(img * Hc + (hd >> 1)) * Wc + (wd >> 1)) * e_ncols + (oks[ps] ? col : 0);
        }
        rres[ps] = *(const uint4*)(e_res + ri);
      }
    }
    if (CHAIN == 0 && p.mask) {
#pragma unroll
      for (int ps = 0; ps < PASSES; ++ps)
        rmsk[ps] = *(const uint4*)(p.mask + pixs[ps] * e_ncols + (oks[ps] ? col : 0));
    }
    unsigned rbits[PASSES];
    if (CHAIN == 0 && p.bits_in) {
#pragma unroll
      for (int ps = 0; ps < PASSES; ++ps)
        rbits[ps] = p.bits_in[(pixs[ps] * e_ncols + (oks[ps] ? col : 0)) >> 3];
    }
#pragma unroll
    for (int t = 0; t < 2; ++t)
#pragma unroll
      for (int j = 0; j < NT; ++j)
#pragma unroll
        for (int r = 0; r < 4; ++r)
          ep[(t * 16 + fq * 4 + r) * EP_STRIDE + j * 16 + frow] = acc[2 * h + t][j][r];
#pragma unroll
    for (int ps = 0; ps < PASSES; ++ps) {
      const int row = ps * RPP + rl;
      float4 v0 = *(const float4*)(ep + row * EP_STRIDE + cg * 8);
      float4 v1 = *(const float4*)(ep + row * EP_STRIDE + cg * 8 + 4);
      if constexpr (TAPS == 1) {
        if (p.ksplit > 1) {
          if (oks[ps]) {
            float* dst = p.partial + ((size_t)ks * p.M + pixs[ps]) * e_ncols + col;
            *(float4*)dst = v0;
            *(float4*)(dst + 4) = v1;
          }
          continue;
        }
      }
      float v[8] = {v0.x + b0.x, v0.y + b0.y, v0.z + b0.z, v0.w + b0.w, v1.x + b1.x, v1.y + b1.y, v1.z + b1.z, v1.w + b1.w};
      if (e_res) {
        const uint4 rv = rres[ps];
        v[0] += __uint_as_float(rv.x << 16); v[1] += __uint_as_float(rv.x & 0xffff0000u);
        v[2] += __uint_as_float(rv.y << 16); v[3] += __uint_as_float(rv.y & 0xffff0000u);
        v[4] += __uint_as_float(rv.z << 16); v[5] += __uint_as_float(rv.z & 0xffff0000u);
        v[6] += __uint_as_float(rv.w << 16); v[7] += __uint_as_float(rv.w & 0xffff0000u);
      }
      if (CHAIN == 0 && p.mask) {
        const unsigned mm[4] = {rmsk[ps].x, rmsk[ps].y, rmsk[ps].z, rmsk[ps].w};
#pragma unroll
        for (int k = 0; k < 4; ++k) {
          unsigned lo = mm[k] & 0xffffu, hi = mm[k] >> 16;
          if (!(lo != 0u && lo < 0x8000u)) v[2 * k] = 0.0f;
          if (!(hi != 0u && hi < 0x8000u)) v[2 * k + 1] = 0.0f;
        }
      }
      if (CHAIN == 0 && p.bits_in) {
        const unsigned mb = rbits[ps];
#pragma unroll
        for (int k = 0; k < 8; ++k)
          if (!((mb >> k) & 1u)) v[k] = 0.0f;
      }
      if (e_relu && (CHAIN > 0 || (!p.mask && !p.bits_in))) {
#pragma unroll
        for (int k = 0; k < 8; ++k) v[k] = v[k] > 0.0f ? v[k] : 0.0f;
      }
      const uint4 o = pack8_bf16_hw(v);
      if (oks[ps]) *(uint4*)(e_y + pixs[ps] * e_ncols + col) = o;
      if constexpr (CHAIN > 0) {
        if (c3 && !last3) *(uint4*)((unsigned char*)ep + row * (EP_STRIDE * 4) + ((cg ^ (row & 7)) << 4)) = o;
      }
      if (CHAIN == 0 && p.bits_out && oks[ps]) {
        const unsigned w4[4] = {o.x, o.y, o.z, o.w};
        unsigned mb = 0;
#pragma unroll
        for (int k = 0; k < 4; ++k) {
          const unsigned lo = w4[k] & 0xffffu, hi = w4[k] >> 16;
          mb |= ((lo != 0u && lo < 0x8000u) ? 1u : 0u) << (2 * k);
          mb |= ((hi != 0u && hi < 0x8000u) ? 1u : 0u) << (2 * k + 1);
        }
        p.bits_out[(pixs[ps] * e_ncols + col) >> 3] = (unsigned char)mb;
      }
    }
  }
  if constexpr (CHAIN > 0) {
    if (c3 && !last3) {
#pragma unroll
      for (int hf = 0; hf < 2; ++hf) {
        bf16x8_t a3[MT];
#pragma unroll
        for (int i = 0; i < MT; ++i)
          a3[i] = *(const bf16x8_t*)((const unsigned char*)ep + (i * 16 + frow) * (EP_STRIDE * 4) +
                                     (((hf * 4 + fq) ^ ((i * 16 + frow) & 7)) << 4));
#pragma unroll
        for (int i = 0; i < MT; ++i)
#pragma unroll
          for (int j = 0; j < NT; ++j)
            acc3[i][j] = __builtin_amdgcn_mfma_f32_16x16x32_bf16(a3[i], b3[hf][j], acc3[i][j], 0, 0, 0);
      }
    }
  }
  }
  if (p.pf != nullptr) asm volatile("" ::"v"(pfv[0].x), "v"(pfv[1].x), "v"(pfv[2].x), "v"(pfv[3].x));
#ifdef MXDET_CONV_STAMP
  if (cs_on) {
    asm volatile("s_waitcnt vmcnt(0)" ::: "memory");
    cs[5] = __builtin_amdgcn_s_memtime();
    if (lane == 0)
      for (int k = 0; k < 6; ++k) g_conv_stamp[blockIdx.x == 0 ? 0 : 1][k] = cs[k];
  }
#endif
}

template <int BM, int BN, int WM, int WN, int NS, bool DGRAD, bool PAR = false, int TAPS = 0, int CHAIN = 0>
__global__ void __launch_bounds__(64 * WM * WN)
conv_igemm_kernel(ConvP p) {
  conv_igemm_tile<BM, BN, WM, WN, NS, DGRAD, PAR, TAPS, CHAIN>(p, (int)blockIdx.x, (int)gridDim.x);
}

struct ConvG {
  ConvP p;
  int block0, nblocks;
};

template <int BM, int BN, int WM, int WN, int NS, bool DGRAD, int TAPS = 0>
__global__ void __launch_bounds__(64 * WM * WN)
conv_igemm_grouped_kernel(const ConvG* __restrict__ table, int n) {
  int lo = 0, hi = n - 1;
  const int bid = (int)blockIdx.x;
  while (lo < hi) {
    int mid = (lo + hi + 1) >> 1;
    if (table[mid].block0 <= bid) lo = mid; else hi = mid - 1;
  }
  const int b = bid - table[lo].block0;
  const int nb = table[lo].nblocks;
  if (b >= nb) return;
  const ConvP p = table[lo].p;
  conv_igemm_tile<BM, BN, WM, WN, NS, DGRAD, false, TAPS>(p, b, nb);
}

static thread_local int g_force_cfg = 0;

static int thr_t64() { return (int)tuning(MXDET_TUNE_T64); }
static int thr_t128() { return (int)tuning(MXDET_TUNE_T128); }
static int thr_par64() { return (int)tuning(MXDET_TUNE_PAR64); }

template <int BM_, int BN_, int WM_, int WN_, int NS_>
struct Tile { static constexpr int BM = BM_, BN = BN_, WM = WM_, WN = WN_, NS = NS_; };
using T128x64 = Tile<128, 64, 4, 1, 2>;
using T128x128 = Tile<128, 128, 2, 2, 2>;
using T64x128 = Tile<64, 128, 2, 2, 2>;
using T64x64 = Tile<64, 64, 2, 2, 3>;
using T128x128w8 = Tile<128, 128, 2, 4, 2>;
using T256x256 = Tile<256, 256, 2, 4, 2>;
using T128x128s4 = Tile<128, 128, 2, 2, 4>;
#define MXDET_GROUPED_TILES(X) X(0, T128x64) X(1, T128x128) X(2, T64x128) X(3, T64x64)

template <class T, bool DGRAD, bool PAR = false, int TAPS = 0, int CHAIN = 0>
static int launch_cfg(ConvP& p, hipStream_t s) {
  constexpr int BM = T::BM, BN = T::BN, WM = T::WM, WN = T::WN, NS = T::NS;
  if (PAR) {
    int t = 0;
    for (int c = 0; c < 4; ++c) {
      p.par_tile0[c] = t;
      t += ceil_div(p.N * p.par_hc[c >> 1] * p.par_wc[c & 1], BM);
    }
    p.par_tile0[4] = t;
    p.tiles_m = t;
  }
  if (p.tiles_m <= 0) p.tiles_m = ceil_div(p.M - p.m_begin, BM);
  p.tiles_n = ceil_div(p.Ncols, BN);
  long long nwg = (long long)p.tiles_m * p.tiles_n;
  if (TAPS == 1 && p.ksplit > 1) nwg *= p.ksplit;
  if (route_probe_on()) {
    const int32_t rec[kRouteWords] = {MXDET_ROUTE_CONV, BM, BN, WM, WN, NS, DGRAD, PAR, TAPS, CHAIN, p.tiles_m, p.tiles_n,
                                      p.m_begin, p.ksplit, (int32_t)nwg, 0};
    route_record(rec);
    return MXDET_OK;
  }
  hipLaunchKernelGGL((conv_igemm_kernel<BM, BN, WM, WN, NS, DGRAD, PAR, TAPS, CHAIN>), dim3((unsigned)nwg),
                     dim3(64 * WM * WN), 0, s, p);
  return check_launch("conv2d");
}

template <bool DGRAD>
static int launch(ConvP& p, hipStream_t s) {
  const int force = g_force_cfg;
  const long long t128 = (long long)ceil_div(p.M, 128) * ceil_div(p.Ncols, 128);
  const long long t64 = (long long)ceil_div(p.M, 64) * ceil_div(p.Ncols, 128);
  const int K = p.KH * p.KW * p.C;
#define MXDET_FORCE_ST(T) (p.KH * p.KW == 1 ? launch_cfg<T, DGRAD, false, 1>(p, s) : launch_cfg<T, DGRAD, false, 9>(p, s))
  switch (force) {
    case 3: return launch_cfg<T128x128s4, DGRAD>(p, s);
    case 5: return launch_cfg<T64x64, DGRAD>(p, s);
    case 6: return launch_cfg<T64x128, DGRAD>(p, s);
    case 7: return launch_cfg<T128x128, DGRAD>(p, s);
    case 8: return launch_cfg<T128x64, DGRAD>(p, s);
    case 15: return launch_cfg<T256x256, DGRAD>(p, s);
    case 40: return MXDET_FORCE_ST(T64x64);
    case 41: return MXDET_FORCE_ST(T64x128);
    case 45: return MXDET_FORCE_ST(T128x128);
    case 46: return MXDET_FORCE_ST(T128x64);
    case 49: return MXDET_FORCE_ST(T128x128w8);
    default: break;
  }
#undef MXDET_FORCE_ST
  const int taps = p.KH * p.KW;
  const int st = ((p.stride != 1 && (DGRAD || taps == 1)) || tuning(MXDET_TUNE_STATIC_TAPS) == 0) ? 0
                 : (taps == 1 && p.pad == 0) ? 1 : (p.KH == 3 && p.KW == 3 && p.pad == 1) ? 9 : 0;
#define MXDET_LAUNCH_ST(T)                                      \
  (st == 1 ? launch_cfg<T, DGRAD, false, 1>(p, s)               \
           : st == 9 ? launch_cfg<T, DGRAD, false, 9>(p, s)     \
                     : launch_cfg<T, DGRAD>(p, s))
  if constexpr (DGRAD) {
    if (p.stride == 2 && force == 0) {
      for (int par = 0; par < 2; ++par) {
        int h0 = ((par - p.pad) % 2 + 2) % 2, w0 = h0;
        p.par_h0[par] = h0; p.par_w0[par] = w0;
        p.par_hc[par] = p.Hd > h0 ? (p.Hd - h0 + 1) / 2 : 0;
        p.par_wc[par] = p.Wd > w0 ? (p.Wd - w0 + 1) / 2 : 0;
      }
      if (p.Ncols <= 64) return launch_cfg<T128x64, true, true>(p, s);
      if (t64 >= thr_par64()) return launch_cfg<T64x128, true, true>(p, s);
      return launch_cfg<T64x64, true, true>(p, s);
    }
  }
  if (p.Ncols <= 64) return MXDET_LAUNCH_ST(T128x64);
  if (t128 >= thr_t128() && K > 256) {
    const int tn = ceil_div(p.Ncols, 256);
    const long long full = (long long)(p.M / 256) * tn;
    const long long rounds = full / 256;
    if (rounds >= 1 && p.Ncols % 256 == 0) {
      ConvP big = p;
      big.tiles_m = (int)(rounds * 256 / tn);
      int rc = launch_cfg<T256x256, DGRAD>(big, s);
      if (rc) return rc;
      p.m_begin = big.tiles_m * 256;
      if (p.m_begin >= p.M) return rc;
    }
    switch ((int)tuning(MXDET_TUNE_TAIL)) {
      case 1: return MXDET_LAUNCH_ST(T64x128);
      case 2: return MXDET_LAUNCH_ST(T64x64);
      default: return MXDET_LAUNCH_ST(T128x128);
    }
  }
  {
    const long long t256 = (long long)(p.M / 256) * (p.Ncols / 256);
    if (p.M % 256 == 0 && p.Ncols % 256 == 0 && t256 >= 160 && t256 <= 256 && K >= 1024 && p.m_begin == 0)
      return launch_cfg<T256x256, DGRAD>(p, s);
  }
  if (st != 0 && p.Ncols >= 128 && t128 >= tuning(MXDET_TUNE_T128W)) return MXDET_LAUNCH_ST(T128x128w8);
  if (t64 >= thr_t64()) return MXDET_LAUNCH_ST(T64x128);
  return MXDET_LAUNCH_ST(T64x64);
#undef MXDET_LAUNCH_ST
}

static int validate(const mxdet_conv_desc_t* d, const char* who) {
  MXDET_REQUIRE(d != nullptr, MXDET_EINVAL, "%s: null descriptor", who);
  MXDET_REQUIRE(d->N > 0 && d->H > 0 && d->W > 0 && d->Cin > 0 && d->Cout > 0 && d->KH > 0 && d->KW > 0 &&
                    d->stride > 0 && d->pad >= 0,
                MXDET_ESHAPE, "%s: non-positive dimension", who);
  MXDET_REQUIRE(d->KH * d->KW <= 25, MXDET_ESHAPE, "%s: at most 25 filter taps (use the stem kernel for 7x7)", who);
  MXDET_REQUIRE(d->Ho == (d->H + 2 * d->pad - d->KH) / d->stride + 1 &&
                    d->Wo == (d->W + 2 * d->pad - d->KW) / d->stride + 1,
                MXDET_ESHAPE, "%s: Ho/Wo do not match the convolution arithmetic", who);
  MXDET_REQUIRE((long long)d->N * d->H * d->W * d->Cin < (1ll << 31) &&
                    (long long)d->N * d->Ho * d->Wo * d->Cout < (1ll << 31),
                MXDET_ESHAPE, "%s: tensor exceeds 2^31 elements", who);
  return MXDET_OK;
}

static void fill_fwd(ConvP& p, const mxdet_conv_desc_t* d) {
  memset(&p, 0, sizeof(p));
  p.N = d->N; p.Hs = d->H; p.Ws = d->W; p.C = d->Cin;
  p.Hd = d->Ho; p.Wd = d->Wo; p.Ncols = d->Cout;
  p.KH = d->KH; p.KW = d->KW; p.stride = d->stride; p.pad = d->pad;
  p.relu = d->relu; p.res_up = d->res_upsample;
  p.M = d->N * d->Ho * d->Wo;
  p.pf = d->prefetch; p.pf_bytes = d->prefetch ? d->prefetch_bytes : 0;
  p.bits_out = (unsigned char*)d->relu_bits;
}
static void fill_dgrad(ConvP& p, const mxdet_conv_desc_t* d) {
  memset(&p, 0, sizeof(p));
  p.N = d->N; p.Hs = d->Ho; p.Ws = d->Wo; p.C = d->Cout;
  p.Hd = d->H; p.Wd = d->W; p.Ncols = d->Cin;
  p.KH = d->KH; p.KW = d->KW; p.stride = d->stride; p.pad = d->pad;
  p.M = d->N * d->H * d->W;
  p.pf = d->prefetch; p.pf_bytes = d->prefetch ? d->prefetch_bytes : 0;
}

}

using namespace mxdet;

#ifdef MXDET_CONV_STAMP
extern "C" int mxdet_debug_read_conv_stamps(unsigned long long* out ) {
  return hipMemcpyFromSymbol(out, HIP_SYMBOL(g_conv_stamp), sizeof(unsigned long long) * 16) == hipSuccess ? 0 : -4;
}
#endif

extern "C" int mxdet_debug_force_conv_cfg(int32_t cfg) {
  g_force_cfg = cfg;
  return MXDET_OK;
}

extern "C" int mxdet_conv2d_fwd(const mxdet_conv_desc_t* d, const uint16_t* x, const uint16_t* w,
                                const float* bias, const uint16_t* residual, uint16_t* y,
                                mxdet_stream_t stream) {
  clear_error();
  int rc = validate(d, "conv2d_fwd");
  if (rc) return rc;
  MXDET_REQUIRE(d->Cin % 64 == 0, MXDET_ESHAPE, "conv2d_fwd: Cin %d must be a multiple of 64", d->Cin);
  MXDET_REQUIRE(d->Cout % 8 == 0, MXDET_ESHAPE, "conv2d_fwd: Cout %d must be a multiple of 8", d->Cout);
  MXDET_REQUIRE(x && w && y, MXDET_EINVAL, "conv2d_fwd: null pointer");
  ConvP p;
  fill_fwd(p, d);
  p.x = x; p.w = w; p.bias = bias; p.res = residual; p.y = y;
  MXDET_REQUIRE(!d->relu_bits || d->Cout % 8 == 0, MXDET_ESHAPE, "conv2d_fwd: relu_bits needs Cout %% 8 == 0");
  return launch<false>(p, as_stream(stream));
}

extern "C" int mxdet_conv2d_fwd_chain(const mxdet_conv_desc_t* d, const uint16_t* x, const uint16_t* w, const float* bias,
                                      const uint16_t* w2, const float* bias2, int32_t cout2, int32_t relu2,
                                      const uint16_t* residual2, uint16_t* y2, const uint16_t* w3, const float* bias3,
                                      int32_t cout3, int32_t relu3, uint16_t* y3, mxdet_stream_t stream) {
  clear_error();
  int rc = validate(d, "conv2d_fwd_chain");
  if (rc) return rc;
  MXDET_REQUIRE(d->KH == 3 && d->KW == 3 && d->stride == 1 && d->pad == 1, MXDET_ESHAPE,
                "conv2d_fwd_chain: the first convolution must be 3x3, stride 1, pad 1");
  MXDET_REQUIRE(d->Cin % 64 == 0 && d->Cout == 64 && cout2 == 256, MXDET_ESHAPE,
                "conv2d_fwd_chain: Cin %d must be a multiple of 64, Cout %d must be 64 and cout2 %d must be 256", d->Cin,
                d->Cout, cout2);
  MXDET_REQUIRE(!d->res_upsample && !d->relu_bits, MXDET_EINVAL, "conv2d_fwd_chain: no upsampled residual / relu_bits");
  MXDET_REQUIRE(x && w && w2 && y2, MXDET_EINVAL, "conv2d_fwd_chain: null pointer");
  MXDET_REQUIRE((long long)d->N * d->Ho * d->Wo * cout2 < (1ll << 31), MXDET_ESHAPE, "conv2d_fwd_chain: output exceeds 2^31");
  ConvP p;
  fill_fwd(p, d);
  p.x = x; p.w = w; p.bias = bias;
  p.chain_w = w2; p.chain_bias = bias2; p.chain_res = residual2; p.chain_y = y2; p.chain_relu = relu2;
  if (w3 != nullptr) {
    MXDET_REQUIRE(cout3 == 64 && y3 != nullptr, MXDET_ESHAPE, "conv2d_fwd_chain: the third convolution needs cout3 == 64 (got %d) and y3",
                  cout3);
    p.chain3_w = w3; p.chain3_bias = bias3; p.chain3_y = y3; p.chain3_relu = relu3;
  }
  return launch_cfg<T128x64, false, false, 9, 256>(p, as_stream(stream));
}

namespace mxdet {
__global__ void __launch_bounds__(256)
conv_splitk_fold_kernel(const float* __restrict__ partial, int ksplit, long long M, int Ncols, const float* __restrict__ bias,
                        const uint16_t* __restrict__ res, int relu, uint16_t* __restrict__ y) {
  const long long i = ((long long)blockIdx.x * blockDim.x + threadIdx.x) * 8;
  const long long total = M * Ncols;
  if (i >= total) return;
  const int col = (int)(i % Ncols);
  float v[8];
  {
    const float4 a = *(const float4*)(partial + i), b = *(const float4*)(partial + i + 4);
    v[0] = a.x; v[1] = a.y; v[2] = a.z; v[3] = a.w; v[4] = b.x; v[5] = b.y; v[6] = b.z; v[7] = b.w;
  }
  for (int k = 1; k < ksplit; ++k) {
    const float4 a = *(const float4*)(partial + (size_t)k * total + i), b = *(const float4*)(partial + (size_t)k * total + i + 4);
    v[0] += a.x; v[1] += a.y; v[2] += a.z; v[3] += a.w; v[4] += b.x; v[5] += b.y; v[6] += b.z; v[7] += b.w;
  }
  if (bias) {
    const float4 a = *(const float4*)(bias + col), b = *(const float4*)(bias + col + 4);
    v[0] += a.x; v[1] += a.y; v[2] += a.z; v[3] += a.w; v[4] += b.x; v[5] += b.y; v[6] += b.z; v[7] += b.w;
  }
  if (res) {
    float rf[8];
    unpack8_bf16(*(const uint4*)(res + i), rf);
#pragma unroll
    for (int k = 0; k < 8; ++k) v[k] += rf[k];
  }
  if (relu) {
#pragma unroll
    for (int k = 0; k < 8; ++k) v[k] = v[k] > 0.0f ? v[k] : 0.0f;
  }
  *(uint4*)(y + i) = pack8_bf16_hw(v);
}
}

extern "C" size_t mxdet_conv2d_fwd_splitk_workspace_bytes(const mxdet_conv_desc_t* d, int32_t ksplit) {
  if (!d || ksplit < 1) return 0;
  return (size_t)ksplit * (size_t)d->N * d->Ho * d->Wo * d->Cout * sizeof(float);
}

extern "C" int mxdet_conv2d_fwd_splitk(const mxdet_conv_desc_t* d, const uint16_t* x, const uint16_t* w, const float* bias,
                                       const uint16_t* residual, uint16_t* y, int32_t ksplit, void* workspace,
                                       size_t workspace_bytes, mxdet_stream_t stream) {
  clear_error();
  int rc = validate(d, "conv2d_fwd_splitk");
  if (rc) return rc;
  MXDET_REQUIRE(d->KH == 1 && d->KW == 1 && d->stride == 1 && d->pad == 0 && !d->res_upsample, MXDET_ESHAPE,
                "conv2d_fwd_splitk: 1x1 / stride 1 / pad 0 layers (fully connected) only");
  MXDET_REQUIRE(d->Cin % 64 == 0 && d->Cout % 8 == 0, MXDET_ESHAPE, "conv2d_fwd_splitk: Cin %% 64, Cout %% 8");
  MXDET_REQUIRE(ksplit >= 1 && ksplit <= d->Cin / 64, MXDET_ESHAPE, "conv2d_fwd_splitk: 1 <= ksplit <= Cin / 64");
  MXDET_REQUIRE(x && w && y, MXDET_EINVAL, "conv2d_fwd_splitk: null pointer");
  if (ksplit == 1) return mxdet_conv2d_fwd(d, x, w, bias, residual, y, stream);
  const size_t need = mxdet_conv2d_fwd_splitk_workspace_bytes(d, ksplit);
  MXDET_REQUIRE(workspace && workspace_bytes >= need, MXDET_EWORKSPACE, "conv2d_fwd_splitk: workspace %zu < %zu", workspace_bytes, need);
  ConvP p;
  fill_fwd(p, d);
  p.x = x; p.w = w; p.y = y;
  p.relu = 0; p.bits_out = nullptr; p.pf = nullptr; p.pf_bytes = 0;
  p.ksplit = ksplit; p.partial = (float*)workspace;
  const int big = (int)tuning(MXDET_TUNE_SPLITK_TILE);
  const int BT = big ? 128 : 64;
  const long long tiles = (long long)ceil_div(p.M, BT) * ceil_div(p.Ncols, BT);
  MXDET_REQUIRE(tiles % 8 == 0, MXDET_ESHAPE, "conv2d_fwd_splitk: the tile count (%lld) must be a multiple of 8", tiles);
  hipStream_t s = as_stream(stream);
  if (big == 1) rc = launch_cfg<T128x128, false, false, 1>(p, s);
  else if (big == 2) rc = launch_cfg<T128x128w8, false, false, 1>(p, s);
  else rc = launch_cfg<T64x64, false, false, 1>(p, s);
  if (rc || route_probe_on()) return rc;
  const long long total = (long long)p.M * p.Ncols;
  hipLaunchKernelGGL(conv_splitk_fold_kernel, dim3((unsigned)ceil_div<long long>(total / 8, 256)), dim3(256), 0, s,
                     (const float*)workspace, ksplit, (long long)p.M, p.Ncols, bias, residual, d->relu, y);
  return check_launch("conv2d_fwd_splitk");
}

extern "C" int mxdet_conv2d_dgrad(const mxdet_conv_desc_t* d, const uint16_t* dy, const uint16_t* wt,
                                  const uint16_t* residual, const uint16_t* relu_mask, uint16_t* dx,
                                  mxdet_stream_t stream) {
  clear_error();
  int rc = validate(d, "conv2d_dgrad");
  if (rc) return rc;
  MXDET_REQUIRE(d->Cout % 64 == 0, MXDET_ESHAPE, "conv2d_dgrad: Cout %d must be a multiple of 64", d->Cout);
  MXDET_REQUIRE(d->Cin % 8 == 0, MXDET_ESHAPE, "conv2d_dgrad: Cin %d must be a multiple of 8", d->Cin);
  MXDET_REQUIRE(dy && wt && dx, MXDET_EINVAL, "conv2d_dgrad: null pointer");
  ConvP p;
  fill_dgrad(p, d);
  p.x = dy; p.w = wt; p.y = dx;
  p.res = residual ? residual : (d->accumulate ? dx : nullptr);
  p.mask = (d->relu && !d->relu_bits) ? relu_mask : nullptr;
  p.bits_in = d->relu ? (const unsigned char*)d->relu_bits : nullptr;
  MXDET_REQUIRE(!d->relu || relu_mask || d->relu_bits, MXDET_EINVAL, "conv2d_dgrad: relu set without relu_mask / relu_bits");
  return launch<true>(p, as_stream(stream));
}

template <class T, bool DGRAD>
static void launch_grouped_cfg(const ConvG* table, int n, int grid, hipStream_t s, int tapclass) {
  constexpr int BM = T::BM, BN = T::BN, WM = T::WM, WN = T::WN, NS = T::NS;
  if (route_probe_on()) {
    const int32_t rec[kRouteWords] = {MXDET_ROUTE_CONV_GROUPED, BM, BN, WM, WN, NS, DGRAD, 0, tapclass == 1 ? 1 : tapclass == 2 ? 9 : 0,
                                      0, 0, 0, 0, 0, grid, n};
    route_record(rec);
    return;
  }
  if (tapclass == 1)
    hipLaunchKernelGGL((conv_igemm_grouped_kernel<BM, BN, WM, WN, NS, DGRAD, 1>), dim3((unsigned)grid), dim3(64 * WM * WN),
                       0, s, table, n);
  else if (tapclass == 2)
    hipLaunchKernelGGL((conv_igemm_grouped_kernel<BM, BN, WM, WN, NS, DGRAD, 9>), dim3((unsigned)grid), dim3(64 * WM * WN),
                       0, s, table, n);
  else
    hipLaunchKernelGGL((conv_igemm_grouped_kernel<BM, BN, WM, WN, NS, DGRAD>), dim3((unsigned)grid), dim3(64 * WM * WN),
                       0, s, table, n);
}

extern "C" size_t mxdet_conv2d_grouped_table_bytes(int32_t n) { return n > 0 ? (size_t)n * sizeof(ConvG) : 0; }

extern "C" int mxdet_conv2d_grouped_plan(const mxdet_conv_item_t* items, int32_t n, int32_t kind, void* table_host,
                                         size_t table_bytes, int32_t* cfg_out, int32_t* grid_out) {
  clear_error();
  MXDET_REQUIRE(items && n > 0 && table_host && cfg_out && grid_out, MXDET_EINVAL, "conv2d_grouped_plan: null pointer");
  MXDET_REQUIRE(kind == 0 || kind == 1, MXDET_EINVAL, "conv2d_grouped_plan: kind must be 0 (forward) or 1 (dgrad)");
  MXDET_REQUIRE(table_bytes >= (size_t)n * sizeof(ConvG), MXDET_EWORKSPACE, "conv2d_grouped_plan: table too small");
  ConvG* t = (ConvG*)table_host;
  long long t64 = 0, t128_max = 0;
  int max_cols = 0, kmax = 0;
  int tapclass = -1;
  for (int i = 0; i < n; ++i) {
    const mxdet_conv_desc_t* d = &items[i].desc;
    int rc = validate(d, "conv2d_grouped_plan");
    if (rc) return rc;
    ConvP& p = t[i].p;
    if (kind == 0) fill_fwd(p, d); else fill_dgrad(p, d);
    MXDET_REQUIRE(items[i].src && items[i].filt && items[i].dst, MXDET_EINVAL, "conv2d_grouped_plan: item %d: null pointer", i);
    if (kind == 0) {
      MXDET_REQUIRE(d->Cin % 64 == 0 && d->Cout % 8 == 0, MXDET_ESHAPE, "conv2d_grouped_plan: item %d: Cin %% 64, Cout %% 8", i);
      p.x = (const uint16_t*)items[i].src; p.w = (const uint16_t*)items[i].filt; p.bias = items[i].bias;
      p.res = (const uint16_t*)items[i].residual; p.y = (uint16_t*)items[i].dst;
    } else {
      MXDET_REQUIRE(d->Cout % 64 == 0 && d->Cin % 8 == 0, MXDET_ESHAPE, "conv2d_grouped_plan: item %d: Cout %% 64, Cin %% 8", i);
      MXDET_REQUIRE(d->stride == 1, MXDET_ESHAPE, "conv2d_grouped_plan: item %d: strided data gradients are not grouped", i);
      MXDET_REQUIRE(!d->relu || items[i].relu_mask || d->relu_bits, MXDET_EINVAL, "conv2d_grouped_plan: item %d: relu without mask", i);
      p.x = (const uint16_t*)items[i].src; p.w = (const uint16_t*)items[i].filt; p.y = (uint16_t*)items[i].dst;
      p.res = items[i].residual ? (const uint16_t*)items[i].residual : (d->accumulate ? (const uint16_t*)items[i].dst : nullptr);
      p.mask = (d->relu && !d->relu_bits) ? (const uint16_t*)items[i].relu_mask : nullptr;
      p.bits_in = d->relu ? (const unsigned char*)d->relu_bits : nullptr;
    }
    {
      const int tc = (d->stride != 1 && (kind == 1 || d->KH * d->KW == 1)) ? 0
                     : (d->KH == 1 && d->KW == 1 && d->pad == 0) ? 1 : (d->KH == 3 && d->KW == 3 && d->pad == 1) ? 2 : 0;
      tapclass = tapclass < 0 ? tc : (tapclass == tc ? tc : 0);
    }
    t64 += (long long)ceil_div(p.M, 64) * ceil_div(p.Ncols, 128);
    long long t128 = (long long)ceil_div(p.M, 128) * ceil_div(p.Ncols, 128);
    t128_max = t128 > t128_max ? t128 : t128_max;
    max_cols = p.Ncols > max_cols ? p.Ncols : max_cols;
    kmax = p.KH * p.KW * p.C > kmax ? p.KH * p.KW * p.C : kmax;
  }
  int cfg;
  if (max_cols <= 64) cfg = 0;
  else if (t128_max >= thr_t128() && kmax > 256) cfg = 1;
  else if (t64 >= thr_t64()) cfg = 2;
  else cfg = 3;
  int BM = 0, BN = 0;
  switch (cfg) {
#define X(k, T) case k: BM = T::BM; BN = T::BN; break;
    MXDET_GROUPED_TILES(X)
#undef X
  }
  long long blocks = 0;
  for (int i = 0; i < n; ++i) {
    ConvP& p = t[i].p;
    p.tiles_m = ceil_div(p.M, BM);
    p.tiles_n = ceil_div(p.Ncols, BN);
    t[i].nblocks = p.tiles_m * p.tiles_n;
    t[i].block0 = (int)blocks;
    blocks += (long long)align_up((size_t)t[i].nblocks, 8);
    MXDET_REQUIRE(blocks < (1ll << 30), MXDET_ESHAPE, "conv2d_grouped_plan: group too large");
  }
  if (tuning(MXDET_TUNE_STATIC_TAPS) == 0 || tapclass < 0) tapclass = 0;
  *cfg_out = cfg + 4 * tapclass;
  *grid_out = (int32_t)blocks;
  return MXDET_OK;
}

extern "C" int mxdet_conv2d_grouped(const void* table_dev, int32_t n, int32_t kind, int32_t cfg, int32_t grid,
                                    mxdet_stream_t stream) {
  clear_error();
  MXDET_REQUIRE(table_dev && n > 0 && grid > 0, MXDET_EINVAL, "conv2d_grouped: empty group");
  MXDET_REQUIRE((kind == 0 || kind == 1) && cfg >= 0 && cfg <= 11, MXDET_EINVAL, "conv2d_grouped: bad kind / cfg");
  const ConvG* t = (const ConvG*)table_dev;
  hipStream_t s = as_stream(stream);
  const int tc = cfg >> 2;
  cfg &= 3;
  switch (cfg) {
#define X(k, T)                                                            \
    case k:                                                                \
      if (kind == 0) launch_grouped_cfg<T, false>(t, n, grid, s, tc);      \
      else launch_grouped_cfg<T, true>(t, n, grid, s, tc);                 \
      break;
    MXDET_GROUPED_TILES(X)
#undef X
  }
  if (route_probe_on()) return MXDET_OK;
  return check_launch("conv2d_grouped");
}
```

### mxdetection_amd/models/necks/fpn.py

```python
import torch

from ...ops import dense
from ..utils.layers import ConvLayer, cached_buf


class FPN:
    def __init__(self, in_channels, out_channels, arena, ws, device, gen, extra_p6=True):
        kw = dict(arena=arena, ws=ws, device=device, gen=gen)
        L = len(in_channels)
        self.outs = [ConvLayer("fpn.out%d" % (i + 2), out_channels, out_channels, 3,
                               init_std=(1.0 / (9 * out_channels)) ** 0.5, **kw) for i in range(L)]
        self.lats = [ConvLayer("fpn.lat%d" % (i + 2), in_channels[i], out_channels, 1,
                               init_std=(1.0 / in_channels[i]) ** 0.5, **kw) for i in range(L)]
        self.L, self.C, self.extra_p6 = L, out_channels, extra_p6
        self.device = device
        self.bufs = {}
        self.inner = self.feats = self.P = None

    def layers(self):
        return self.outs + self.lats

    def plan(self, c_shapes):
        for i, s in enumerate(c_shapes):
            self.lats[i].plan(s)
            self.outs[i].plan((s[0], s[1], s[2], self.C))

    def _buf(self, key, shape):
        return cached_buf(self.bufs, key, shape, torch.bfloat16, self.device)

    def forward(self, feats):
        L = self.L
        self.feats = feats
        inner = [None] * L
        for i in reversed(range(L)):
            shape = feats[i].shape[:3] + (self.C,)
            res = inner[i + 1] if i + 1 < L else None
            inner[i] = self.lats[i].forward(feats[i], residual=res, res_upsample=res is not None,
                                            out=self._buf("inner%d" % i, shape))
        P = [self._buf("P%d" % i, inner[i].shape) for i in range(L)]
        self.outs[0].forward(inner[0], out=P[0])
        dense.conv2d_group("fwd", [self.outs[i].fwd_call(inner[i], out=P[i]) for i in range(1, L)], self.device)
        if self.extra_p6:
            N, H, W, Cc = P[-1].shape
            P.append(dense.subsample2(P[-1], self._buf("P6", (N, (H + 1) // 2, (W + 1) // 2, Cc))))
        self.inner, self.P = inner, P
        return P

    def backward(self, dP, dC, c_needs_grad):
        L = self.L
        if self.extra_p6:
            dense.subsample2_backward(dP[L], dP[L - 1], accumulate=True)
        dinner = [self._buf("dinner%d" % i, self.inner[i].shape) for i in range(L)]
        for i in range(L):
            self.outs[i].backward_weight(self.inner[i], dP[i])
        self.outs[0].backward_data(dP[0], self.inner[0].shape, out=dinner[0])
        dense.conv2d_group("dgrad", [self.outs[i].dgrad_call(dP[i], self.inner[i].shape, out=dinner[i])
                                     for i in range(1, L)], self.device)
        for i in range(1, L):
            dense.upsample2_backward(dinner[i - 1], dinner[i], accumulate=True)
        calls = []
        for i in range(L):
            self.lats[i].backward_weight(self.feats[i], dinner[i])
            if c_needs_grad[i]:
                top = i == L - 1
                calls.append(self.lats[i].dgrad_call(dinner[i], self.feats[i].shape,
                                                     relu_mask=self.feats[i] if top else None, out=dC[i]))
        if calls:
            dense.conv2d_group("dgrad", calls, self.device)

class RetinaFPN:

    def __init__(self, in_channels, out_channels, arena, ws, device, gen):
        kw = dict(arena=arena, ws=ws, device=device, gen=gen)
        L = len(in_channels)
        xav = lambda cin, k: (1.0 / (k * k * cin)) ** 0.5
        self.p7 = ConvLayer("fpn.p7", out_channels, out_channels, 3, 2, init_std=xav(out_channels, 3), **kw)
        self.outs = [ConvLayer("fpn.out%d" % (i + 3), out_channels, out_channels, 3, init_std=xav(out_channels, 3), **kw)
                     for i in range(L)]
        self.p6 = ConvLayer("fpn.p6", in_channels[-1], out_channels, 3, 2, init_std=xav(in_channels[-1], 3), **kw)
        self.lats = [ConvLayer("fpn.lat%d" % (i + 3), in_channels[i], out_channels, 1, init_std=xav(in_channels[i], 1), **kw)
                     for i in range(L)]
        self.L, self.C, self.device = L, out_channels, device
        self.bufs = {}

    def layers(self):
        return [self.p7] + self.outs + [self.p6] + self.lats

    def _buf(self, key, shape):
        return cached_buf(self.bufs, key, shape, torch.bfloat16, self.device)

    def plan(self, c_shapes):
        for i, s in enumerate(c_shapes):
            self.lats[i].plan(s)
            self.outs[i].plan((s[0], s[1], s[2], self.C))
        self.p6.plan(c_shapes[-1])
        self.p7.plan(self.p6.out_shape(c_shapes[-1]))
        s6 = self.p6.out_shape(c_shapes[-1])
        return [(s[0], s[1], s[2], self.C) for s in c_shapes] + [s6, self.p7.out_shape(s6)]

    def forward(self, feats):
        L = self.L
        self.feats = feats
        inner = [None] * L
        for i in reversed(range(L)):
            res = inner[i + 1] if i + 1 < L else None
            inner[i] = self.lats[i].forward(feats[i], residual=res, res_upsample=res is not None,
                                            out=self._buf("inner%d" % i, feats[i].shape[:3] + (self.C,)))
        P = [self.outs[i].forward(inner[i], out=self._buf("P%d" % i, inner[i].shape)) for i in range(L)]
        self.p6_raw = self.p6.forward(feats[-1], out=self._buf("P6", self.p6.out_shape(feats[-1].shape)))
        self.p6_relu = dense.relu_forward(self.p6_raw, self._buf("P6r", self.p6_raw.shape))
        p7 = self.p7.forward(self.p6_relu, out=self._buf("P7", self.p7.out_shape(self.p6_relu.shape)))
        self.inner, self.P = inner, P + [self.p6_raw, p7]
        return self.P

    def backward(self, dP, dC):
        L = self.L
        self.p7.backward_weight(self.p6_relu, dP[L + 1])
        t = self.p7.backward_data(dP[L + 1], self.p6_relu.shape, relu_mask=self.p6_relu, out=self._buf("dP6r", self.p6_relu.shape))
        dense.add_bf16(dP[L], t, dP[L])
        dinner = [None] * L
        for i in range(L):
            self.outs[i].backward_weight(self.inner[i], dP[i])
            dinner[i] = self.outs[i].backward_data(dP[i], self.inner[i].shape, out=self._buf("dinner%d" % i, self.inner[i].shape))
            if i > 0:
                dense.upsample2_backward(dinner[i - 1], dinner[i], accumulate=True)
        self.p6.backward_weight(self.feats[-1], dP[L])
        self.p6.backward_data(dP[L], self.feats[-1].shape, out=dC[L - 1])
        for i in range(L):
            self.lats[i].backward_weight(self.feats[i], dinner[i])
            top = i == L - 1
            self.lats[i].backward_data(dinner[i], self.feats[i].shape, residual=dC[i] if top else None,
                                       relu_mask=self.feats[i] if top else None, out=dC[i])
```

### mxdetection_amd/models/rpn_heads/rpn_head.py

```python
import os

import torch

from ...core import anchor as A_
from ...core import loss as L_
from ...ops import dense
from ...ops.proposal import PyramidProposal
from ...ops import rpn_sparse as RS
from ...ops.rpn_sparse import MAX_SLOTS, RPNSparse
from ..utils.layers import ConvLayer, cached_buf

HEAD_CPAD = 64


RELU_BITS = os.environ.get("MXDET_TUNE_RELU_BITS", "1") == "1"
RPN_SPARSE = int(os.environ.get("MXDET_TUNE_RPN_SPARSE", "1"))
RPN_ORDERED = int(os.environ.get("MXDET_TUNE_RPN_ORDERED", "1"))


class RPNHead:
    def __init__(self, channels, strides, arena, ws, device, gen, ratios=(0.5, 1.0, 2.0), scales=(8,),
                 pre_nms_top_n=2000, post_nms_top_n=2000, nms_thresh=0.7, min_size=0.0, batch_size=256,
                 fg_fraction=0.5, fg_thresh=0.7, bg_thresh=0.3, sigma=3.0, seed=99):
        kw = dict(arena=arena, ws=ws, device=device, gen=gen)
        self.A = len(ratios) * len(scales)
        assert 5 * self.A <= HEAD_CPAD
        self.out = ConvLayer("rpn.out", channels, HEAD_CPAD, 1, init_std=0.01, cout_real=5 * self.A, **kw)
        self.conv = ConvLayer("rpn.conv", channels, channels, 3, init_std=0.01, **kw)
        self.strides = list(strides)
        self.base = [torch.from_numpy(A_.generate_base_anchors(s, ratios, scales)).to(device) for s in strides]
        self.proposal = PyramidProposal(self.base, strides, pre_nms_top_n, post_nms_top_n, nms_thresh, min_size)
        self.batch_size, self.fg_fraction, self.fg_thresh, self.bg_thresh = batch_size, fg_fraction, fg_thresh, bg_thresh
        self.sigma, self.seed, self.device, self.C = sigma, seed, device, channels
        self.bufs = {}
        self.anchors = None
        self.level_shapes = None

    def layers(self):
        return [self.out, self.conv]

    def _buf(self, key, shape, dtype=torch.bfloat16, zero=False):
        return cached_buf(self.bufs, key, shape, dtype, self.device, zero)

    def plan(self, p_shapes, g_max):
        for s in p_shapes:
            self.conv.plan(s)
            self.out.plan(s)
        self.level_shapes = [(s[1], s[2]) for s in p_shapes]
        N = p_shapes[0][0]
        self.anchors = torch.cat([A_.generate_anchors(self.base[l], H, W, self.strides[l])
                                  for l, (H, W) in enumerate(self.level_shapes)])
        self.level_offsets = [0]
        for (H, W) in self.level_shapes:
            self.level_offsets.append(self.level_offsets[-1] + H * W * self.A)
        At = self.anchors.shape[0]
        self.at_ws = A_.AnchorTargetWorkspace(N, At, g_max, self.device)
        self.at_out = (torch.empty((N, At), dtype=torch.int32, device=self.device),
                       torch.empty((N, At), dtype=torch.int32, device=self.device),
                       torch.empty((N, At, 4), dtype=torch.float32, device=self.device),
                       torch.empty((N, At), dtype=torch.float32, device=self.device))
        self.nparts = [L_.rpn_loss_num_partials(N, H, W) for (H, W) in self.level_shapes]
        self.partial = torch.zeros((2 * sum(self.nparts),), dtype=torch.float32, device=self.device)
        self.loss = torch.zeros((2,), dtype=torch.float32, device=self.device)
        smax = N * self.batch_size
        self.sparse = (RPNSparse(self.level_shapes, N, self.A, self.C, HEAD_CPAD, smax, self.device)
                       if RPN_SPARSE and 0 < smax <= MAX_SLOTS else None)
        self.sparse_wgrad = int(RPN_SPARSE) == 2
        self.dt_map = None
        if self.sparse is not None and not self.sparse_wgrad:
            sizes = [s[0] * s[1] * s[2] * s[3] for s in p_shapes]
            flat = self._buf("dt_map", (sum(sizes),))
            self.dt_map, off = [], 0
            for s, n in zip(p_shapes, sizes):
                self.dt_map.append(flat[off:off + n].view(tuple(s)))
                off += n

    def forward(self, P):
        self.P = P
        tb = [self._buf("t%d" % l, p.shape) for l, p in enumerate(P)]
        hb = [self._buf("h%d" % l, p.shape[:3] + (HEAD_CPAD,)) for l, p in enumerate(P)]
        self.tbits = [self._buf("tb%d" % l, p.shape[:3] + (p.shape[3] // 8,), dtype=torch.uint8) if RELU_BITS else None
                      for l, p in enumerate(P)]
        self.conv.forward(P[0], relu=True, out=tb[0], bits_out=self.tbits[0])
        dense.conv2d_group("fwd", [self.conv.fwd_call(P[l], relu=True, out=tb[l], bits_out=self.tbits[l])
                                   for l in range(1, len(P))], self.device)
        self.out.forward(tb[0], out=hb[0])
        dense.conv2d_group("fwd", [self.out.fwd_call(tb[l], out=hb[l]) for l in range(1, len(P))], self.device)
        self.t, self.h = tb, hb
        return self.h

    def get_proposals(self, im_info):
        return self.proposal(self.h, self.h, im_info, layout="nhwc_fused")

    def assign_targets(self, gt_boxes, im_info, step, image_offset, step_dev=None):
        labels, _, targets, _ = A_.assign_anchor(self.anchors, gt_boxes, im_info, self.fg_thresh, self.bg_thresh, 0.0,
                                                 self.batch_size, self.fg_fraction, self.seed, step, image_offset,
                                                 self.at_ws, self.at_out, step_dev)
        self._assigned = (labels, targets)
        if self.sparse is not None:
            self.sparse.build_list(labels)

    def loss_and_grad(self, gt_boxes, im_info, step, image_offset, loss_scale=1.0, step_dev=None, assigned=False):
        if not assigned:
            self.assign_targets(gt_boxes, im_info, step, image_offset, step_dev)
        labels, targets = self._assigned
        N = gt_boxes.shape[0]
        norm = 1.0 / float(N * self.batch_size)
        self.gh = []
        off = 0
        for l, h in enumerate(self.h):
            g = self._buf("gh%d" % l, h.shape)
            L_.rpn_loss_level(h, self.A, labels, targets, self.level_offsets[l], self.sigma, norm, loss_scale, g,
                              self.partial[2 * off:])
            off += self.nparts[l]
            self.gh.append(g)
        L_.loss_finalize(self.partial, off, 2, self.loss)
        return self.loss

    def backward(self, dP, dP_has_grad, flush=True):
        if self.sparse is not None:
            return self._backward_sparse(dP, dP_has_grad, flush)
        L = len(self.h)
        dt = [self._buf("dt%d" % l, self.t[l].shape) for l in range(L)]
        grouped = self.out.ws.grouping
        for l in range(L):
            self.out.backward_weight(self.t[l], self.gh[l], accumulate=(l > 0) and not grouped)
        self.out.backward_data(self.gh[0], self.t[0].shape, relu_mask=self.t[0], out=dt[0], relu_bits=self.tbits[0])
        dense.conv2d_group("dgrad", [self.out.dgrad_call(self.gh[l], self.t[l].shape, relu_mask=self.t[l], out=dt[l],
                                                         relu_bits=self.tbits[l])
                                     for l in range(1, L)], self.device)
        for l in range(L):
            self.conv.backward_weight(self.P[l], dt[l], accumulate=(l > 0) and not grouped)
        self.conv.backward_data(dt[0], self.P[0].shape, accumulate=dP_has_grad[0], out=dP[0])
        dense.conv2d_group("dgrad", [self.conv.dgrad_call(dt[l], self.P[l].shape, accumulate=dP_has_grad[l], out=dP[l])
                                     for l in range(1, L)], self.device)
        if flush:
            self.out.ws.flush()

    def _backward_sparse(self, dP, dP_has_grad, flush=True):
        g = self.out.arena
        grads = (g.view(self.out.wi, "g"), g.view(self.out.bi, "g"), g.view(self.conv.wi, "g"), g.view(self.conv.bi, "g"))
        if self.sparse_wgrad:
            self.sparse.backward(self.P, self.t, self.tbits, self.gh, dP, dP_has_grad, self.out.wt, self.conv.wt, *grads)
            return
        L = len(self.h)
        grouped = self.out.ws.grouping
        if grouped and RPN_ORDERED and self.out.train_bias and self.conv.train_bias:
            if self.sparse.ordered is None and not torch.cuda.is_current_stream_capturing():
                self.sparse.plan_ordered(
                    [(self.t[l], self.gh[l], 1, 1, 1, 0, grads[0], grads[1], False) for l in range(L)] +
                    [(self.P[l], self.dt_map[l], 3, 3, 1, 1, grads[2], grads[3], False) for l in range(L)])
            if self.sparse.ordered is not None:
                self.sparse.backward(self.P, self.t, self.tbits, self.gh, dP, dP_has_grad, self.out.wt, self.conv.wt, *grads,
                                     parts=RS.ZERO | RS.DT | RS.DGRAD | RS.WGRAD_ORDERED)
                return
        for l in range(L):
            self.out.backward_weight(self.t[l], self.gh[l], accumulate=(l > 0) and not grouped)
        self.sparse.backward(self.P, self.t, self.tbits, self.gh, dP, dP_has_grad, self.out.wt, self.conv.wt, *grads,
                             parts=RS.ZERO | RS.DT | RS.DTMAP | RS.DGRAD, dt=self.dt_map)
        for l in range(L):
            self.conv.backward_weight(self.P[l], self.dt_map[l], accumulate=(l > 0) and not grouped)
        if flush:
            self.out.ws.flush()
```

### mxdetection_amd/models/utils/layers.py

```python
import contextlib
import functools
import math
import os

import torch

from ...ops import dense


def cached_buf(bufs, key, shape, dtype=torch.bfloat16, device=None, zero=False):
    k = (key, tuple(shape), dtype)
    b = bufs.get(k)
    if b is None:
        b = (torch.zeros if zero else torch.empty)(tuple(shape), dtype=dtype, device=device)
        bufs[k] = b
    return b


def buf_cache(device):
    bufs = {}
    return bufs, functools.partial(cached_buf, bufs, device=device)


class Workspace:
    abl_skip = frozenset()

    def __init__(self, device):
        self.device = device
        self.need = 0
        self.buf = None
        self._retired = []
        self.side = None
        self.grouping = False
        self.pending = []
        self.plans = {}
        self.gbuf = None

    def defer(self, layer, x, dy):
        self.pending.append((layer, x, dy))

    def flush(self):
        if not self.pending:
            return
        items, self.pending = self.pending, []
        if "wgrad" in self.abl_skip:
            return
        key = tuple((id(l), x.data_ptr(), dy.data_ptr()) for l, x, dy in items)
        plan = self.plans.get(key)
        capturing = torch.cuda.is_current_stream_capturing()
        if plan is None and not capturing:
            calls = [(x, dy, l.k, l.k, l.stride, l.pad, l.arena.view(l.wi, "g"),
                      l.arena.view(l.bi, "g") if l.train_bias else None, False) for l, x, dy in items]
            plan = dense.GroupedWgrad(calls, self.device)
            self.plans[key] = plan
            if self.gbuf is None or self.gbuf.numel() < plan.workspace_bytes:
                self._retired.append(self.gbuf)
                self.gbuf = torch.empty((max(plan.workspace_bytes, 256),), dtype=torch.uint8, device=self.device)
        ctx = self.fork()
        with (ctx if ctx is not None else contextlib.nullcontext()):
            if plan is None or self.gbuf is None or self.gbuf.numel() < plan.workspace_bytes:
                for l, x, dy in items:
                    dense.conv2d_wgrad(x, dy, l.k, l.k, l.stride, l.pad, l.arena.view(l.wi, "g"),
                                       l.arena.view(l.bi, "g") if l.train_bias else None, False, self.get())
            else:
                plan.launch(self.gbuf)
    def fork(self):
        if self.side is None:
            return None
        self.side.wait_stream(torch.cuda.current_stream())
        return torch.cuda.stream(self.side)

    def join(self):
        if self.side is not None:
            torch.cuda.current_stream().wait_stream(self.side)

    def require(self, nbytes):
        self.need = max(self.need, int(nbytes))

    def get(self):
        if self.buf is None or self.buf.numel() < self.need:
            self._retired.append(self.buf)
            self.buf = torch.empty((self.need,), dtype=torch.uint8, device=self.device)
        return self.buf


class ParamArena:
    def __init__(self, device):
        self.device = device
        self.entries = []
        self.size = 0
        self.w = self.g = self.m = self.wb = None

    def register(self, name, shape):
        n = 1
        for s in shape:
            n *= s
        off = self.size
        self.entries.append((name, tuple(shape), off, n))
        self.size += (n + 63) // 64 * 64
        return len(self.entries) - 1

    def finalize(self):
        dev = self.device
        self.w = torch.zeros((self.size,), dtype=torch.float32, device=dev)
        self.g = torch.zeros((self.size,), dtype=torch.float32, device=dev)
        self.m = torch.zeros((self.size,), dtype=torch.float32, device=dev)
        self.wb = torch.zeros((self.size,), dtype=torch.bfloat16, device=dev)

    def view(self, idx, which):
        _, shape, off, n = self.entries[idx]
        return getattr(self, which)[off:off + n].view(shape)

    def offset_of(self, idx):
        return self.entries[idx][2]

    def refresh_bf16(self):
        dense.f32_to_bf16(self.w, self.wb)

    def sgd_step(self, lr, momentum, wd, rescale):
        dense.sgd_momentum_update(self.w, self.g, self.m, self.wb, lr, momentum, wd, rescale)


class ConvLayer:

    def __init__(self, name, cin, cout, k, stride=1, pad=None, bias=True, trainable=True, arena=None, ws=None,
                 device="cuda", gen=None, init_std=None, zero_init=False, train_bias=True, cout_real=None):
        self.name, self.cin, self.cout, self.k, self.stride = name, cin, cout, k, stride
        self.pad = (k // 2) if pad is None else pad
        self.trainable = trainable
        self.arena, self.ws = arena, ws
        self.has_bias = bias
        std = init_std if init_std is not None else math.sqrt(2.0 / (k * k * cin))
        w0 = torch.zeros((cout, k, k, cin)) if zero_init else torch.randn((cout, k, k, cin), generator=gen) * std
        self.cout_real = cout if cout_real is None else cout_real
        if self.cout_real < cout:
            w0[self.cout_real:] = 0
        self._w0 = w0
        self.train_bias = bias and trainable and train_bias
        self.frozen_bias = None
        if bias and not self.train_bias:
            self.frozen_bias = torch.zeros((cout,), dtype=torch.float32, device=device)
        if trainable:
            self.wi = arena.register(name + ".weight", (cout, k, k, cin))
            self.bi = arena.register(name + ".bias", (cout,)) if self.train_bias else None
        else:
            self.w_bf16 = w0.to(torch.bfloat16).to(device)
            self.bias_f32 = self.frozen_bias
        self.wt = None
        self.device = device
        self.pf_fwd = self.pf_bwd = None

    def materialize(self):
        if not self.trainable:
            return
        self.arena.view(self.wi, "w").copy_(self._w0.to(self.device))
        self.w_bf16 = self.arena.view(self.wi, "wb")
        self.bias_f32 = self.arena.view(self.bi, "w") if self.train_bias else self.frozen_bias
        self.wt = torch.empty((self.cin, self.k, self.k, self.cout), dtype=torch.bfloat16, device=self.device)
        self._w0 = None

    def plan(self, x_shape):
        if self.trainable:
            self.ws.require(dense.conv2d_wgrad_workspace_bytes(x_shape, self.cout, self.k, self.k, self.stride, self.pad))

    def out_shape(self, x_shape):
        N, H, W, _ = x_shape
        return (N, (H + 2 * self.pad - self.k) // self.stride + 1, (W + 2 * self.pad - self.k) // self.stride + 1,
                self.cout)

    def refresh_transposed(self):
        if self.trainable:
            dense.filter_transpose(self.w_bf16, self.wt)

    def forward(self, x, relu=False, residual=None, res_upsample=False, out=None, bits_out=None):
        if dense.PF_TRACE is not None:
            dense.PF_TRACE.append((self, "f", dense.mem_range(self.w_bf16), None))
        return dense.conv2d_forward(x, self.w_bf16, self.bias_f32, residual, self.stride, self.pad, relu, res_upsample,
                                    out, prefetch=self.pf_fwd, bits_out=bits_out)

    def fwd_call(self, x, relu=False, residual=None, res_upsample=False, out=None, bits_out=None):
        t = (x, self.w_bf16, self.bias_f32, residual, self.stride, self.pad, relu, res_upsample, out)
        return t if bits_out is None else t + (bits_out,)

    def dgrad_call(self, dy, x_shape, residual=None, relu_mask=None, accumulate=False, out=None, relu_bits=None):
        t = (dy, self.wt, tuple(x_shape), self.k, self.k, self.stride, self.pad, residual, relu_mask, accumulate, out)
        return t if relu_bits is None else t + (relu_bits,)

    def backward_data(self, dy, x_shape, residual=None, relu_mask=None, accumulate=False, out=None, relu_bits=None):
        if dense.PF_TRACE is not None:
            dense.PF_TRACE.append((self, "b", dense.mem_range(self.wt), None))
        return dense.conv2d_dgrad(dy, self.wt, x_shape, self.k, self.k, self.stride, self.pad, residual,
                                  None if relu_bits is not None else relu_mask, accumulate, out, prefetch=self.pf_bwd,
                                  relu_bits=relu_bits)

    def backward_weight(self, x, dy, accumulate=False):
        if self.ws.grouping and not accumulate:
            self.ws.defer(self, x, dy)
            return
        dw = self.arena.view(self.wi, "g")
        db = self.arena.view(self.bi, "g") if self.train_bias else None
        ctx = self.ws.fork()
        if ctx is None:
            dense.conv2d_wgrad(x, dy, self.k, self.k, self.stride, self.pad, dw, db, accumulate, self.ws.get())
        else:
            with ctx:
                dense.conv2d_wgrad(x, dy, self.k, self.k, self.stride, self.pad, dw, db, accumulate, self.ws.get())


class GroupNormLayer:
    trainable = True

    def __init__(self, name, channels, groups, arena, device="cuda", eps=1e-5):
        if groups <= 0 or channels % groups or (channels // groups) % 8:
            raise ValueError("GroupNorm %s: %d groups do not divide %d channels into multiples of 8" % (name, groups, channels))
        self.name, self.C, self.G, self.eps = name, channels, groups, eps
        self.arena, self.device = arena, device
        self.gi = arena.register(name + ".gamma", (channels,))
        self.bi = arena.register(name + ".beta", (channels,))
        self.bufs = {}
        self.plans = {}
        self.gamma = self.beta = None
        self.x = self.y = self.mean = self.rstd = None
        self.relu = False

    def materialize(self):
        self.gamma, self.beta = self.arena.view(self.gi, "w"), self.arena.view(self.bi, "w")
        self.gamma.fill_(1.0)
        self.beta.zero_()

    def named_params(self):
        return [(self.name + ".gamma", self.gi), (self.name + ".beta", self.bi)]

    def plan(self, x_shape):
        x_shape = tuple(x_shape)
        p = self.plans.get(x_shape)
        if p is None:
            from ...ops import group_norm as GN
            stats = [cached_buf(self.bufs, k, (x_shape[0], self.G), torch.float32, self.device) for k in ("mean", "rstd")]
            ws = [cached_buf(self.bufs, "ws%d" % b, (max(GN.workspace_bytes(x_shape, self.G, bool(b)), 256),), torch.uint8,
                             self.device) for b in (0, 1)]
            p = self.plans[x_shape] = (stats[0], stats[1], ws[0], ws[1])
        return p

    def forward(self, x, relu=False, out=None):
        from ...ops import group_norm as GN
        mean, rstd, ws, _ = self.plan(x.shape)
        y, _, _ = GN.group_norm_forward(x, self.gamma, self.beta, self.G, self.eps, relu, out=out, mean=mean, rstd=rstd,
                                        workspace=ws)
        self.x, self.y, self.mean, self.rstd, self.relu = x, y, mean, rstd, relu
        return y

    def backward(self, dy, out=None):
        from ...ops import group_norm as GN
        return GN.group_norm_backward(self.x, dy, self.mean, self.rstd, self.gamma, self.G, self.arena.view(self.gi, "g"),
                                      self.arena.view(self.bi, "g"), y=None, beta=self.beta, eps=self.eps, relu=self.relu,
                                      out=out, workspace=self.plan(self.x.shape)[3])


def fc_ksplit():
    return int(os.environ.get("MXDET_TUNE_FC1_KSPLIT", "4"))


def fc_forward(fc, x, ksplit, buf, relu=True, out=None):
    R = x.shape[0]
    if ksplit > 1 and (R * fc.cout) % (64 * 64 * 8) == 0 and R % 64 == 0:
        ws = buf(("splitk", fc.name), (4 * ksplit * R * fc.cout,), dtype=torch.uint8)
        return dense.conv2d_forward_splitk(x, fc.w_bf16, fc.bias_f32, None, relu, ksplit, out, ws)
    return fc.forward(x, relu=relu, out=out)


class LayerChain:

    def __init__(self, specs, arena, ws, device, gen, norm="none", gn_groups=32):
        n = len(specs)
        self.gn = norm == "gn"
        self.relu = [s.get("relu", True) for s in specs]
        self.split = [s.get("split", False) for s in specs]
        self.ksplit = fc_ksplit() if any(self.split) else 1
        self.convs, self.norms = [None] * n, [None] * n
        for i in reversed(range(n)):
            s = {k: v for k, v in specs[i].items() if k not in ("relu", "split")}
            if self.gn:
                self.norms[i] = GroupNormLayer(s["name"] + "_gn", s["cout"], gn_groups, arena, device)
            self.convs[i] = ConvLayer(bias=not self.gn, arena=arena, ws=ws, device=device, gen=gen, **s)
        self.acts = None

    def layers(self):
        return list(reversed(self.convs))

    def norm_layers(self):
        return [n for n in reversed(self.norms) if n is not None]

    def plan(self, x_shape):
        for c, n in zip(self.convs, self.norms):
            c.plan(x_shape)
            x_shape = c.out_shape(x_shape)
            if n is not None:
                n.plan(x_shape)
        return x_shape

    def forward(self, x, buf):
        self.acts = [x]
        for c, n, relu, split in zip(self.convs, self.norms, self.relu, self.split):
            out = buf(("a", c.name), c.out_shape(x.shape))
            if n is not None:
                x = n.forward(c.forward(x, out=buf(("c", c.name), out.shape)), relu=relu, out=out)
            elif split:
                x = fc_forward(c, x, self.ksplit, buf, relu=relu, out=out)
            else:
                x = c.forward(x, relu=relu, out=out)
            self.acts.append(x)
        return x

    def _mask(self, i):
        return self.acts[i] if i > 0 and self.relu[i - 1] and not self.gn else None

    @property
    def out_mask(self):
        return self._mask(len(self.convs))

    def backward(self, g, buf, first_mask=None, add_to=None):
        for i in reversed(range(len(self.convs))):
            c, n, x = self.convs[i], self.norms[i], self.acts[i]
            if n is not None:
                g = n.backward(g, out=buf(("dn", c.name), g.shape))
            c.backward_weight(x, g)
            mask = self._mask(i) if i > 0 else first_mask
            if i == 0 and add_to is not None:
                g = c.backward_data(g, x.shape, relu_mask=mask, accumulate=True, out=add_to)
            else:
                g = c.backward_data(g, x.shape, relu_mask=mask, out=buf(("g", c.name), x.shape))
        return g


class DeformConvLayer:

    def __init__(self, name, cin, cout, stride=1, groups=1, modulated=True, arena=None, ws=None, device="cuda", gen=None,
                 train_bias=False):
        self.name, self.cin, self.cout, self.stride, self.pad = name, cin, cout, stride, 1
        self.groups, self.modulated = groups, bool(modulated)
        self.k = 3
        self.trainable = True
        self.conv = ConvLayer(name, 9 * cin, cout, 1, 1, 0, arena=arena, ws=ws, device=device, gen=gen,
                              train_bias=train_bias)
        self.conv.dcn_khwc = (3, 3, cin)
        nreal = (27 if self.modulated else 18) * groups
        self.offset = ConvLayer(name + "_offset", cin, (nreal + 63) // 64 * 64, 3, stride, 1, arena=arena, ws=ws,
                                device=device, gen=gen, zero_init=True, cout_real=nreal)
        self.ws = ws
        self.device = device
        self.bufs, self._buf = buf_cache(device)
        self.x = self.off = self.col = None

    def layers(self):
        return [self.conv, self.offset]

    def out_shape(self, x_shape):
        return self.offset.out_shape(x_shape)[:3] + (self.cout,)

    def plan(self, x_shape):
        N, Ho, Wo, _ = self.out_shape(x_shape)
        self.offset.plan(x_shape)
        self.conv.plan((N, Ho, Wo, 9 * self.cin))

    def forward(self, x, relu=False, residual=None, out=None, bits_out=None):
        from ...ops import deform_conv
        N, Ho, Wo, _ = self.out_shape(x.shape)
        off = self.offset.forward(x, out=self._buf("off", (N, Ho, Wo, self.offset.cout)))
        col = deform_conv.im2col(x, off, self.stride, self.pad, self.groups, self.modulated,
                                 out=self._buf("col", (N, Ho, Wo, 9 * self.cin)))
        self.x, self.off, self.col = x, off, col
        return self.conv.forward(col, relu=relu, residual=residual, out=out, bits_out=bits_out)

    def backward_weight(self, x, dy, accumulate=False):
        self.conv.backward_weight(self.col, dy, accumulate)

    def backward_data(self, dy, x_shape, residual=None, relu_mask=None, accumulate=False, out=None, relu_bits=None):
        from ...ops import deform_conv
        assert residual is None and not accumulate, "DeformConvLayer.backward_data: no residual / accumulate"
        x_shape = tuple(x_shape)
        dcol = self.conv.backward_data(dy, self.col.shape, out=self._buf("dcol", self.col.shape))
        a = (self.stride, self.pad, self.groups, self.modulated)
        doff = deform_conv.col2im_coord(self.x, self.off, dcol, *a, out=self._buf("doff", self.off.shape))
        nws = deform_conv.col2im_workspace_bytes(x_shape, *a, self.off.shape[3])
        dxu = deform_conv.col2im(self.off, dcol, x_shape, *a, out=self._buf("dxu", x_shape),
                                 workspace=self._buf("c2i_ws", (max(nws, 256),), torch.uint8))
        self.offset.backward_weight(self.x, doff)
        return self.offset.backward_data(doff, x_shape, residual=dxu, relu_mask=relu_mask, out=out, relu_bits=relu_bits)
```

### mxdetection_amd/ops/dense.py

```python
import ctypes as C

import torch

from .. import _lib
from .._lib import ConvDescT, check, ptr, stream_ptr

_DT = {torch.float32: 0, torch.bfloat16: 1}


def mem_range(*tensors):
    spans = [(t.data_ptr(), t.numel() * t.element_size()) for t in tensors]
    bases = {t.untyped_storage().data_ptr() for t in tensors}
    if len(bases) == 1:
        lo = min(p for p, _ in spans)
        hi = max(p + n for p, n in spans)
        if hi - lo <= 2 * sum(n for _, n in set(spans)):
            return (lo, hi - lo)
    return spans[0]


def conv_desc(N, H, W, Cin, Cout, KH, KW, stride, pad, relu=False, res_upsample=False, accumulate=False, prefetch=None,
              relu_bits=None):
    d = ConvDescT()
    if relu_bits is not None:
        d.relu_bits = relu_bits.data_ptr()
    if prefetch is not None:
        d.prefetch, d.prefetch_bytes = prefetch if isinstance(prefetch, tuple) else mem_range(prefetch)
    d.N, d.H, d.W, d.Cin, d.Cout, d.KH, d.KW, d.stride, d.pad = N, H, W, Cin, Cout, KH, KW, stride, pad
    d.Ho = (H + 2 * pad - KH) // stride + 1
    d.Wo = (W + 2 * pad - KW) // stride + 1
    d.relu, d.res_upsample, d.accumulate = int(relu), int(res_upsample), int(accumulate)
    return d


def conv2d_forward(x, w, bias=None, residual=None, stride=1, pad=0, relu=False, res_upsample=False, out=None, prefetch=None,
                   bits_out=None):
    lib = _lib.load()
    N, H, W, Cin = x.shape
    Cout, KH, KW, _ = w.shape
    d = conv_desc(N, H, W, Cin, Cout, KH, KW, stride, pad, relu, res_upsample, prefetch=prefetch, relu_bits=bits_out)
    if out is None:
        out = torch.empty((N, d.Ho, d.Wo, Cout), dtype=torch.bfloat16, device=x.device)
    check(lib.mxdet_conv2d_fwd(C.byref(d), ptr(x), ptr(w), ptr(bias), ptr(residual), ptr(out), stream_ptr()),
          "conv2d_fwd")
    return out


def conv2d_forward_splitk(x, w, bias=None, residual=None, relu=False, ksplit=4, out=None, workspace=None):
    lib = _lib.load()
    N, H, W, Cin = x.shape
    Cout = w.shape[0]
    d = conv_desc(N, H, W, Cin, Cout, 1, 1, 1, 0, relu, False)
    if out is None:
        out = torch.empty((N, d.Ho, d.Wo, Cout), dtype=torch.bfloat16, device=x.device)
    need = lib.mxdet_conv2d_fwd_splitk_workspace_bytes(C.byref(d), ksplit)
    if workspace is None or workspace.numel() < need:
        workspace = torch.empty((need,), dtype=torch.uint8, device=x.device)
    check(lib.mxdet_conv2d_fwd_splitk(C.byref(d), ptr(x), ptr(w), ptr(bias), ptr(residual), ptr(out), ksplit, ptr(workspace),
                                      workspace.numel(), stream_ptr()), "conv2d_fwd_splitk")
    return out


def conv2d_forward_chain(x, w, bias, w2, bias2=None, residual2=None, relu=True, relu2=True, out=None, prefetch=None,
                         w3=None, bias3=None, relu3=True, out3=None):
    lib = _lib.load()
    N, H, W, Cin = x.shape
    Cmid, Cout2 = w.shape[0], w2.shape[0]
    d = conv_desc(N, H, W, Cin, Cmid, 3, 3, 1, 1, relu, False, prefetch=prefetch)
    if out is None:
        out = torch.empty((N, H, W, Cout2), dtype=torch.bfloat16, device=x.device)
    if w3 is not None and out3 is None:
        out3 = torch.empty((N, H, W, w3.shape[0]), dtype=torch.bfloat16, device=x.device)
    check(lib.mxdet_conv2d_fwd_chain(C.byref(d), ptr(x), ptr(w), ptr(bias), ptr(w2), ptr(bias2), Cout2, int(relu2),
                                     ptr(residual2), ptr(out), ptr(w3), ptr(bias3), 0 if w3 is None else w3.shape[0],
                                     int(relu3), ptr(out3), stream_ptr()), "conv2d_fwd_chain")
    return out if w3 is None else (out, out3)


def conv2d_dgrad(dy, wt, x_shape, KH, KW, stride=1, pad=0, residual=None, relu_mask=None, accumulate=False, out=None,
                 prefetch=None, relu_bits=None):
    lib = _lib.load()
    N, H, W, Cin = x_shape
    Cout = dy.shape[3]
    d = conv_desc(N, H, W, Cin, Cout, KH, KW, stride, pad, relu=(relu_mask is not None or relu_bits is not None),
                  accumulate=accumulate, prefetch=prefetch, relu_bits=relu_bits)
    if out is None:
        out = torch.empty(tuple(x_shape), dtype=torch.bfloat16, device=dy.device)
    check(lib.mxdet_conv2d_dgrad(C.byref(d), ptr(dy), ptr(wt), ptr(residual), ptr(relu_mask), ptr(out), stream_ptr()),
          "conv2d_dgrad")
    return out


def conv2d_wgrad_workspace_bytes(x_shape, Cout, KH, KW, stride, pad):
    N, H, W, Cin = x_shape
    d = conv_desc(N, H, W, Cin, Cout, KH, KW, stride, pad)
    return _lib.load().mxdet_conv2d_wgrad_workspace_bytes(C.byref(d))


def conv2d_wgrad(x, dy, KH, KW, stride=1, pad=0, dw=None, db=None, accumulate=False, workspace=None):
    lib = _lib.load()
    N, H, W, Cin = x.shape
    Cout = dy.shape[3]
    d = conv_desc(N, H, W, Cin, Cout, KH, KW, stride, pad, accumulate=accumulate)
    need = lib.mxdet_conv2d_wgrad_workspace_bytes(C.byref(d))
    if workspace is None:
        workspace = torch.empty((need,), dtype=torch.uint8, device=x.device)
    if dw is None:
        dw = torch.empty((Cout, KH, KW, Cin), dtype=torch.float32, device=x.device)
    check(lib.mxdet_conv2d_wgrad(C.byref(d), ptr(x), ptr(dy), ptr(dw), ptr(db), ptr(workspace), workspace.numel(),
                                 stream_ptr()), "conv2d_wgrad")
    return dw


class GroupedConv:

    def __init__(self, kind, calls, device, hint=None):
        lib = _lib.load()
        n = len(calls)
        items = (_lib.ConvItemT * n)()
        self.keep, self.kind = calls, 0 if kind == "fwd" else 1
        self.flops = 0.0
        dp = lambda t: None if t is None else t.data_ptr()
        for it, c in zip(items, calls):
            if self.kind == 0:
                x, w, bias, residual, stride, pad, relu, res_up, out = c[:9]
                bits = c[9] if len(c) > 9 else None
                N, H, W, Cin = x.shape
                Cout, KH, KW, _ = w.shape
                it.desc = conv_desc(N, H, W, Cin, Cout, KH, KW, stride, pad, relu, res_up, prefetch=hint, relu_bits=bits)
                hint = None
                it.src, it.filt, it.bias, it.residual, it.relu_mask, it.dst = dp(x), dp(w), dp(bias), dp(residual), None, dp(out)
                self.flops += 2.0 * N * it.desc.Ho * it.desc.Wo * Cout * KH * KW * Cin
            else:
                dy, wt, x_shape, KH, KW, stride, pad, residual, relu_mask, accumulate, out = c[:11]
                bits = c[11] if len(c) > 11 else None
                N, H, W, Cin = x_shape
                Cout = dy.shape[3]
                it.desc = conv_desc(N, H, W, Cin, Cout, KH, KW, stride, pad, relu=(relu_mask is not None or bits is not None),
                                    accumulate=accumulate, prefetch=hint, relu_bits=bits)
                hint = None
                it.src, it.filt, it.bias, it.residual, it.relu_mask, it.dst = (dp(dy), dp(wt), None, dp(residual),
                                                                              None if bits is not None else dp(relu_mask), dp(out))
                self.flops += 2.0 * N * dy.shape[1] * dy.shape[2] * Cout * KH * KW * Cin
        nbytes = lib.mxdet_conv2d_grouped_table_bytes(n)
        host = (C.c_ubyte * nbytes)()
        cfg, grid = C.c_int32(0), C.c_int32(0)
        check(lib.mxdet_conv2d_grouped_plan(items, n, self.kind, host, nbytes, C.byref(cfg), C.byref(grid)),
              "conv2d_grouped_plan")
        self.table = torch.frombuffer(bytearray(host), dtype=torch.uint8).clone().to(device)
        self.n, self.cfg, self.grid = n, cfg.value, grid.value

    def launch(self):
        check(_lib.load().mxdet_conv2d_grouped(ptr(self.table), self.n, self.kind, self.cfg, self.grid, stream_ptr()),
              "conv2d_grouped")


_group_plans = {}


PF_TRACE = None
GROUP_HINTS = {}


def conv2d_group(kind, calls, device):
    key = (kind,) + tuple(tuple(t.data_ptr() if torch.is_tensor(t) else t for t in c) for c in calls)
    if PF_TRACE is not None and calls:
        PF_TRACE.append((None, "g", mem_range(*[c[1] for c in calls]), key if len(calls) > 1 else None))
    if len(calls) == 1:
        plan = None
    else:
        plan = _group_plans.get(key)
        if plan is None and not torch.cuda.is_current_stream_capturing():
            plan = GroupedConv(kind, calls, device, GROUP_HINTS.get(key))
            _group_plans[key] = plan
    if plan is not None:
        plan.launch()
        return
    for c in calls:
        if kind == "fwd":
            x, w, bias, residual, stride, pad, relu, res_up, out = c[:9]
            conv2d_forward(x, w, bias, residual, stride, pad, relu, res_up, out, bits_out=c[9] if len(c) > 9 else None)
        else:
            dy, wt, x_shape, KH, KW, stride, pad, residual, relu_mask, accumulate, out = c[:11]
            conv2d_dgrad(dy, wt, x_shape, KH, KW, stride, pad, residual, relu_mask, accumulate, out,
                         relu_bits=c[11] if len(c) > 11 else None)


def plan_wgrad_group(calls):
    lib = _lib.load()
    n = len(calls)
    items = (_lib.WgradItemT * n)()
    for it, (x, dy, KH, KW, stride, pad, dw, db, accumulate) in zip(items, calls):
        N, H, W, Cin = x.shape
        it.desc = conv_desc(N, H, W, Cin, dy.shape[3], KH, KW, stride, pad, accumulate=accumulate)
        it.x, it.dy, it.dw, it.db = x.data_ptr(), dy.data_ptr(), dw.data_ptr(), (db.data_ptr() if db is not None else None)
    nbytes = lib.mxdet_conv2d_wgrad_grouped_table_bytes(n)
    host = (C.c_ubyte * nbytes)()
    ws, gw, gb, gr = C.c_size_t(0), C.c_int32(0), C.c_int32(0), C.c_int32(0)
    check(lib.mxdet_conv2d_wgrad_grouped_plan(items, n, host, nbytes, C.byref(ws), C.byref(gw), C.byref(gb),
                                              C.byref(gr)), "conv2d_wgrad_grouped_plan")
    return host, ws.value, gw.value, gb.value, gr.value


class GroupedWgrad:

    def __init__(self, calls, device):
        self.keep = calls
        self.flops = 0.0
        self.heaviest = (0.0, "")
        for x, dy, KH, KW, stride, pad, dw, db, accumulate in calls:
            N, H, W, Cin = x.shape
            fl = 2.0 * dy.shape[0] * dy.shape[1] * dy.shape[2] * dy.shape[3] * KH * KW * Cin
            self.flops += fl
            if fl > self.heaviest[0]:
                self.heaviest = (fl, "N=%d %dx%d %d->%d %dx%d" % (N, H, W, Cin, dy.shape[3], KH, KW))
        host, ws, gw, gb, gr = plan_wgrad_group(calls)
        self.grid_big = gb
        self.table = torch.frombuffer(bytearray(host), dtype=torch.uint8).clone().to(device)
        self.n, self.grid_wgrad, self.grid_reduce, self.workspace_bytes = len(calls), gw, gr, ws

    def launch(self, workspace):
        check(_lib.load().mxdet_conv2d_wgrad_grouped(ptr(self.table), self.n, self.grid_wgrad, self.grid_big, self.grid_reduce,
                                                     ptr(workspace), workspace.numel() if workspace is not None else 0,
                                                     self.workspace_bytes, stream_ptr()), "conv2d_wgrad_grouped")


def filter_transpose(w, out=None):
    lib = _lib.load()
    Cout, KH, KW, Cin = w.shape
    if out is None:
        out = torch.empty((Cin, KH, KW, Cout), dtype=torch.bfloat16, device=w.device)
    check(lib.mxdet_filter_transpose(ptr(w), Cout, KH, KW, Cin, ptr(out), stream_ptr()), "filter_transpose")
    return out


def make_transpose_table(pairs, device):
    import struct
    buf = bytearray()
    tile0 = 0
    for w, wt in pairs:
        Cout, KH, KW, Cin = w.shape
        buf += struct.pack("<QQiiii", w.data_ptr(), wt.data_ptr(), Cout, KH * KW, Cin, tile0)
        tile0 += ((Cin + 63) // 64) * ((Cout + 63) // 64) * KH * KW
    table = torch.frombuffer(buf, dtype=torch.uint8).clone().to(device)
    return table, len(pairs), tile0


def filter_transpose_batched(table, ndesc, total_tiles):
    check(_lib.load().mxdet_filter_transpose_batched(ptr(table), ndesc, total_tiles, stream_ptr()),
          "filter_transpose_batched")


def stem_conv7x7(image, w, bias=None, out=None):
    lib = _lib.load()
    N, _, H, W = image.shape
    Ho, Wo = (H - 1) // 2 + 1, (W - 1) // 2 + 1
    if out is None:
        out = torch.empty((N, Ho, Wo, 64), dtype=torch.bfloat16, device=image.device)
    check(lib.mxdet_stem_conv7x7(ptr(image), _DT[image.dtype], N, H, W, ptr(w), ptr(bias), ptr(out), stream_ptr()),
          "stem_conv7x7")
    return out


def stem_conv7x7_pool(image, w, bias=None, out=None):
    lib = _lib.load()
    N, _, H, W = image.shape
    Ho, Wo = (H - 1) // 2 + 1, (W - 1) // 2 + 1
    Hp, Wp = (Ho - 1) // 2 + 1, (Wo - 1) // 2 + 1
    if out is None:
        out = torch.empty((N, Hp, Wp, 64), dtype=torch.bfloat16, device=image.device)
    check(lib.mxdet_stem_conv7x7_pool(ptr(image), _DT[image.dtype], N, H, W, ptr(w), ptr(bias), ptr(out), stream_ptr()),
          "stem_conv7x7_pool")
    return out


def maxpool3x3s2(x, out=None):
    lib = _lib.load()
    N, H, W, Cc = x.shape
    Ho, Wo = (H - 1) // 2 + 1, (W - 1) // 2 + 1
    if out is None:
        out = torch.empty((N, Ho, Wo, Cc), dtype=torch.bfloat16, device=x.device)
    check(lib.mxdet_maxpool3x3s2(ptr(x), N, H, W, Cc, ptr(out), stream_ptr()), "maxpool3x3s2")
    return out


def subsample2(x, out=None):
    lib = _lib.load()
    N, H, W, Cc = x.shape
    if out is None:
        out = torch.empty((N, (H + 1) // 2, (W + 1) // 2, Cc), dtype=torch.bfloat16, device=x.device)
    check(lib.mxdet_subsample2(ptr(x), N, H, W, Cc, ptr(out), stream_ptr()), "subsample2")
    return out


def subsample2_backward(dy, dx, accumulate=False):
    lib = _lib.load()
    N, H, W, Cc = dx.shape
    check(lib.mxdet_subsample2_bwd(ptr(dy), N, H, W, Cc, int(accumulate), ptr(dx), stream_ptr()), "subsample2_bwd")
    return dx


def upsample2_backward(dfine, dcoarse, accumulate=False):
    lib = _lib.load()
    N, Hf, Wf, Cc = dfine.shape
    check(lib.mxdet_upsample2_bwd(ptr(dfine), N, Hf, Wf, Cc, int(accumulate), ptr(dcoarse), stream_ptr()),
          "upsample2_bwd")
    return dcoarse


def pixel_shuffle2_inv_relu(dy_up, act, out=None):
    R, H, W, C4 = act.shape
    if out is None:
        out = torch.empty_like(act)
    check(_lib.load().mxdet_pixel_shuffle2_inv_relu(ptr(dy_up), ptr(act), R, H, W, C4 // 4, ptr(out), stream_ptr()),
          "pixel_shuffle2_inv_relu")
    return out


def pixel_shuffle2(x, out=None, inverse=False):
    lib = _lib.load()
    if not inverse:
        R, H, W, C4 = x.shape
        Cc = C4 // 4
        if out is None:
            out = torch.empty((R, 2 * H, 2 * W, Cc), dtype=torch.bfloat16, device=x.device)
    else:
        R, H2, W2, Cc = x.shape
        H, W = H2 // 2, W2 // 2
        if out is None:
            out = torch.empty((R, H, W, 4 * Cc), dtype=torch.bfloat16, device=x.device)
    check(lib.mxdet_pixel_shuffle2(ptr(x), R, H, W, Cc, int(inverse), ptr(out), stream_ptr()), "pixel_shuffle2")
    return out


def add_bf16(a, b, out=None):
    lib = _lib.load()
    if out is None:
        out = torch.empty_like(a)
    check(lib.mxdet_add_bf16(ptr(a), ptr(b), a.numel(), ptr(out), stream_ptr()), "add_bf16")
    return out


def relu_backward(dy, y, out=None):
    lib = _lib.load()
    if out is None:
        out = torch.empty_like(dy)
    check(lib.mxdet_relu_bwd_bf16(ptr(dy), ptr(y), dy.numel(), ptr(out), stream_ptr()), "relu_bwd_bf16")
    return out


def relu_forward(x, out=None):
    return relu_backward(x, x, out)


def f32_to_bf16(x, out=None):
    lib = _lib.load()
    if out is None:
        out = torch.empty(x.shape, dtype=torch.bfloat16, device=x.device)
    check(lib.mxdet_f32_to_bf16(ptr(x), x.numel(), ptr(out), stream_ptr()), "f32_to_bf16")
    return out


def f32_accum_to_bf16(x, y, accumulate):
    check(_lib.load().mxdet_f32_accum_to_bf16(ptr(x), x.numel(), int(accumulate), ptr(y), stream_ptr()),
          "f32_accum_to_bf16")
    return y


def nchw_to_nhwc(x):
    lib = _lib.load()
    N, Cc, H, W = x.shape
    out = torch.empty((N, H, W, Cc), dtype=torch.bfloat16, device=x.device)
    check(lib.mxdet_nchw_to_nhwc_bf16(ptr(x), _DT[x.dtype], N, Cc, H, W, ptr(out), stream_ptr()), "nchw_to_nhwc_bf16")
    return out


def nhwc_to_nchw(x):
    lib = _lib.load()
    N, H, W, Cc = x.shape
    out = torch.empty((N, Cc, H, W), dtype=torch.float32, device=x.device)
    check(lib.mxdet_nhwc_to_nchw_f32(ptr(x), N, Cc, H, W, ptr(out), stream_ptr()), "nhwc_to_nchw_f32")
    return out


def sgd_momentum_update(w, grad, mom, w_bf16, lr, momentum=0.9, wd=1e-4, rescale=1.0):
    if torch.is_tensor(lr):
        check(_lib.load().mxdet_sgd_momentum_update_sched(ptr(w), ptr(grad), ptr(mom), ptr(w_bf16), w.numel(), ptr(lr),
                                                          momentum, wd, rescale, stream_ptr()), "sgd_momentum_update_sched")
        return
    check(_lib.load().mxdet_sgd_momentum_update(ptr(w), ptr(grad), ptr(mom), ptr(w_bf16), w.numel(), lr, momentum, wd,
                                                rescale, stream_ptr()), "sgd_momentum_update")
```

Before: 460.8 images/sec.

## Fold lead conv's tail tiles into the grouped launch of other pyramid levels

For the FPN output convs and the RPN head conv, the largest-level conv now launches only its 256x256 bulk tiles standalone. Its leftover row range is added as a ranged item to the grouped launch covering the other pyramid levels. This removes the separate tail launch of the lead conv and lets the tail tiles share a grid with the smaller levels, improving occupancy. It adds row-range plumbing through the descriptor and grouped planner, plus a failure path if a ranged plan is first seen under stream capture.

```diff
diff --git a/include/mxdet.h b/include/mxdet.h
--- a/include/mxdet.h
+++ b/include/mxdet.h
@@ -287,7 +287,11 @@
   const void* prefetch;
   int64_t prefetch_bytes;
   void* relu_bits;
+  int32_t row_begin, row_end;
+  int32_t bulk_only;
 } mxdet_conv_desc_t;
+
+int64_t mxdet_conv2d_bulk_rows(const mxdet_conv_desc_t* d, int32_t kind);
 
 int mxdet_conv2d_fwd(const mxdet_conv_desc_t* d, const uint16_t* x, const uint16_t* w,
                      const float* bias, const uint16_t* residual, uint16_t* y,
diff --git a/mxdetection_amd/_lib.py b/mxdetection_amd/_lib.py
--- a/mxdetection_amd/_lib.py
+++ b/mxdetection_amd/_lib.py
@@ -49,6 +49,7 @@
         ("Ho", c_i32), ("Wo", c_i32),
         ("relu", c_i32), ("res_upsample", c_i32), ("accumulate", c_i32),
         ("prefetch", c_vp), ("prefetch_bytes", c_i64), ("relu_bits", c_vp),
+        ("row_begin", c_i32), ("row_end", c_i32), ("bulk_only", c_i32),
     ]
 
 
@@ -203,6 +204,7 @@
     "mxdet_conv2d_fwd_splitk_workspace_bytes": (c_sz, [P(ConvDescT), c_i32]),
     "mxdet_conv2d_fwd_splitk": (c_i32, [P(ConvDescT), c_vp, c_vp, c_vp, c_vp, c_vp, c_i32, c_vp, c_sz, c_vp]),
     "mxdet_conv2d_dgrad": (c_i32, [P(ConvDescT), c_vp, c_vp, c_vp, c_vp, c_vp, c_vp]),
+    "mxdet_conv2d_bulk_rows": (c_i64, [P(ConvDescT), c_i32]),
     "mxdet_conv2d_wgrad_workspace_bytes": (c_sz, [P(ConvDescT)]),
     "mxdet_conv2d_wgrad": (c_i32, [P(ConvDescT), c_vp, c_vp, c_vp, c_vp, c_vp, c_sz, c_vp]),
     "mxdet_conv2d_grouped_table_bytes": (c_sz, [c_i32]),
diff --git a/mxdetection_amd/csrc/conv.hip b/mxdetection_amd/csrc/conv.hip
--- a/mxdetection_amd/csrc/conv.hip
+++ b/mxdetection_amd/csrc/conv.hip
@@ -772,9 +772,22 @@
   return check_launch("conv2d");
 }
 
+static int bulk_tiles_m(const ConvP& p) {
+  if (p.Ncols <= 64 || p.Ncols % 256 != 0) return 0;
+  const long long t128 = (long long)ceil_div(p.M, 128) * ceil_div(p.Ncols, 128);
+  if (t128 < thr_t128() || p.KH * p.KW * p.C <= 256) return 0;
+  const int tn = ceil_div(p.Ncols, 256);
+  const long long rounds = (long long)(p.M / 256) * tn / 256;
+  return (int)(rounds * 256 / tn);
+}
+static int bulk_tiles_m(const ConvP& p, bool dgrad) {
+  return (g_force_cfg != 0 || (dgrad && p.stride == 2)) ? 0 : bulk_tiles_m(p);
+}
+
 template <bool DGRAD>
-static int launch(ConvP& p, hipStream_t s) {
+static int launch(ConvP& p, hipStream_t s, bool bulk_only = false) {
   const int force = g_force_cfg;
+  MXDET_REQUIRE(!bulk_only || bulk_tiles_m(p, DGRAD) > 0, MXDET_ESHAPE, "conv2d: bulk_only on a layer without 256x256 rounds");
   const long long t128 = (long long)ceil_div(p.M, 128) * ceil_div(p.Ncols, 128);
   const long long t64 = (long long)ceil_div(p.M, 64) * ceil_div(p.Ncols, 128);
   const int K = p.KH * p.KW * p.C;
@@ -816,16 +829,14 @@
   }
   if (p.Ncols <= 64) return MXDET_LAUNCH_ST(T128x64);
   if (t128 >= thr_t128() && K > 256) {
-    const int tn = ceil_div(p.Ncols, 256);
-    const long long full = (long long)(p.M / 256) * tn;
-    const long long rounds = full / 256;
-    if (rounds >= 1 && p.Ncols % 256 == 0) {
+    const int bulk = bulk_tiles_m(p);
+    if (bulk > 0) {
       ConvP big = p;
-      big.tiles_m = (int)(rounds * 256 / tn);
+      big.tiles_m = bulk;
       int rc = launch_cfg<T256x256, DGRAD>(big, s);
       if (rc) return rc;
       p.m_begin = big.tiles_m * 256;
-      if (p.m_begin >= p.M) return rc;
+      if (p.m_begin >= p.M || bulk_only) return rc;
     }
     switch ((int)tuning(MXDET_TUNE_TAIL)) {
       case 1: return MXDET_LAUNCH_ST(T64x128);
@@ -859,6 +870,18 @@
   return MXDET_OK;
 }
 
+static int validate_rows(const mxdet_conv_desc_t* d, const char* who, bool ranged, bool bulk, long long rows = 0) {
+  MXDET_REQUIRE(d->bulk_only == 0 || (bulk && d->bulk_only == 1), MXDET_ESHAPE, "%s: bulk_only %d is not taken here", who,
+                d->bulk_only);
+  if (d->row_begin == 0 && d->row_end == 0) return MXDET_OK;
+  MXDET_REQUIRE(ranged, MXDET_ESHAPE, "%s: a row range [%d, %d) belongs to an item of a grouped launch", who, d->row_begin,
+                d->row_end);
+  MXDET_REQUIRE(d->row_begin >= 0 && d->row_begin < d->row_end && d->row_end <= rows, MXDET_ESHAPE,
+                "%s: row range [%d, %d) of a layer with %lld rows", who, d->row_begin, d->row_end, rows);
+  MXDET_REQUIRE(d->row_begin % 256 == 0, MXDET_ESHAPE, "%s: row_begin %d must be a multiple of 256", who, d->row_begin);
+  return MXDET_OK;
+}
+
 static void fill_fwd(ConvP& p, const mxdet_conv_desc_t* d) {
   memset(&p, 0, sizeof(p));
   p.N = d->N; p.Hs = d->H; p.Ws = d->W; p.C = d->Cin;
@@ -899,6 +922,7 @@
   clear_error();
   int rc = validate(d, "conv2d_fwd");
   if (rc) return rc;
+  if ((rc = validate_rows(d, "conv2d_fwd", false, true))) return rc;
   MXDET_REQUIRE(d->Cin % 64 == 0, MXDET_ESHAPE, "conv2d_fwd: Cin %d must be a multiple of 64", d->Cin);
   MXDET_REQUIRE(d->Cout % 8 == 0, MXDET_ESHAPE, "conv2d_fwd: Cout %d must be a multiple of 8", d->Cout);
   MXDET_REQUIRE(x && w && y, MXDET_EINVAL, "conv2d_fwd: null pointer");
@@ -906,7 +930,7 @@
   fill_fwd(p, d);
   p.x = x; p.w = w; p.bias = bias; p.res = residual; p.y = y;
   MXDET_REQUIRE(!d->relu_bits || d->Cout % 8 == 0, MXDET_ESHAPE, "conv2d_fwd: relu_bits needs Cout %% 8 == 0");
-  return launch<false>(p, as_stream(stream));
+  return launch<false>(p, as_stream(stream), d->bulk_only != 0);
 }
 
 extern "C" int mxdet_conv2d_fwd_chain(const mxdet_conv_desc_t* d, const uint16_t* x, const uint16_t* w, const float* bias,
@@ -916,6 +940,7 @@
   clear_error();
   int rc = validate(d, "conv2d_fwd_chain");
   if (rc) return rc;
+  if ((rc = validate_rows(d, "conv2d_fwd_chain", false, false))) return rc;
   MXDET_REQUIRE(d->KH == 3 && d->KW == 3 && d->stride == 1 && d->pad == 1, MXDET_ESHAPE,
                 "conv2d_fwd_chain: the first convolution must be 3x3, stride 1, pad 1");
   MXDET_REQUIRE(d->Cin % 64 == 0 && d->Cout == 64 && cout2 == 256, MXDET_ESHAPE,
@@ -982,6 +1007,7 @@
   clear_error();
   int rc = validate(d, "conv2d_fwd_splitk");
   if (rc) return rc;
+  if ((rc = validate_rows(d, "conv2d_fwd_splitk", false, false))) return rc;
   MXDET_REQUIRE(d->KH == 1 && d->KW == 1 && d->stride == 1 && d->pad == 0 && !d->res_upsample, MXDET_ESHAPE,
                 "conv2d_fwd_splitk: 1x1 / stride 1 / pad 0 layers (fully connected) only");
   MXDET_REQUIRE(d->Cin % 64 == 0 && d->Cout % 8 == 0, MXDET_ESHAPE, "conv2d_fwd_splitk: Cin %% 64, Cout %% 8");
@@ -1016,6 +1042,7 @@
   clear_error();
   int rc = validate(d, "conv2d_dgrad");
   if (rc) return rc;
+  if ((rc = validate_rows(d, "conv2d_dgrad", false, true))) return rc;
   MXDET_REQUIRE(d->Cout % 64 == 0, MXDET_ESHAPE, "conv2d_dgrad: Cout %d must be a multiple of 64", d->Cout);
   MXDET_REQUIRE(d->Cin % 8 == 0, MXDET_ESHAPE, "conv2d_dgrad: Cin %d must be a multiple of 8", d->Cin);
   MXDET_REQUIRE(dy && wt && dx, MXDET_EINVAL, "conv2d_dgrad: null pointer");
@@ -1026,7 +1053,15 @@
   p.mask = (d->relu && !d->relu_bits) ? relu_mask : nullptr;
   p.bits_in = d->relu ? (const unsigned char*)d->relu_bits : nullptr;
   MXDET_REQUIRE(!d->relu || relu_mask || d->relu_bits, MXDET_EINVAL, "conv2d_dgrad: relu set without relu_mask / relu_bits");
-  return launch<true>(p, as_stream(stream));
+  return launch<true>(p, as_stream(stream), d->bulk_only != 0);
+}
+
+extern "C" int64_t mxdet_conv2d_bulk_rows(const mxdet_conv_desc_t* d, int32_t kind) {
+  clear_error();
+  if ((kind != 0 && kind != 1) || validate(d, "conv2d_bulk_rows") != MXDET_OK) return 0;
+  ConvP p;
+  if (kind == 0) fill_fwd(p, d); else fill_dgrad(p, d);
+  return (int64_t)bulk_tiles_m(p, kind == 1) * 256;
 }
 
 template <class T, bool DGRAD>
@@ -1067,6 +1102,12 @@
     if (rc) return rc;
     ConvP& p = t[i].p;
     if (kind == 0) fill_fwd(p, d); else fill_dgrad(p, d);
+    if ((rc = validate_rows(d, "conv2d_grouped_plan", true, false, p.M))) return rc;
+    if (d->row_end > 0) {
+      p.m_begin = d->row_begin;
+      p.M = d->row_end;
+    }
+    const int rows = p.M - p.m_begin;
     MXDET_REQUIRE(items[i].src && items[i].filt && items[i].dst, MXDET_EINVAL, "conv2d_grouped_plan: item %d: null pointer", i);
     if (kind == 0) {
       MXDET_REQUIRE(d->Cin % 64 == 0 && d->Cout % 8 == 0, MXDET_ESHAPE, "conv2d_grouped_plan: item %d: Cin %% 64, Cout %% 8", i);
@@ -1086,8 +1127,8 @@
                      : (d->KH == 1 && d->KW == 1 && d->pad == 0) ? 1 : (d->KH == 3 && d->KW == 3 && d->pad == 1) ? 2 : 0;
       tapclass = tapclass < 0 ? tc : (tapclass == tc ? tc : 0);
     }
-    t64 += (long long)ceil_div(p.M, 64) * ceil_div(p.Ncols, 128);
-    long long t128 = (long long)ceil_div(p.M, 128) * ceil_div(p.Ncols, 128);
+    t64 += (long long)ceil_div(rows, 64) * ceil_div(p.Ncols, 128);
+    long long t128 = (long long)ceil_div(rows, 128) * ceil_div(p.Ncols, 128);
     t128_max = t128 > t128_max ? t128 : t128_max;
     max_cols = p.Ncols > max_cols ? p.Ncols : max_cols;
     kmax = p.KH * p.KW * p.C > kmax ? p.KH * p.KW * p.C : kmax;
@@ -1106,7 +1147,7 @@
   long long blocks = 0;
   for (int i = 0; i < n; ++i) {
     ConvP& p = t[i].p;
-    p.tiles_m = ceil_div(p.M, BM);
+    p.tiles_m = ceil_div(p.M - p.m_begin, BM);
     p.tiles_n = ceil_div(p.Ncols, BN);
     t[i].nblocks = p.tiles_m * p.tiles_n;
     t[i].block0 = (int)blocks;
diff --git a/mxdetection_amd/models/necks/fpn.py b/mxdetection_amd/models/necks/fpn.py
--- a/mxdetection_amd/models/necks/fpn.py
+++ b/mxdetection_amd/models/necks/fpn.py
@@ -38,8 +38,7 @@
             inner[i] = self.lats[i].forward(feats[i], residual=res, res_upsample=res is not None,
                                             out=self._buf("inner%d" % i, shape))
         P = [self._buf("P%d" % i, inner[i].shape) for i in range(L)]
-        self.outs[0].forward(inner[0], out=P[0])
-        dense.conv2d_group("fwd", [self.outs[i].fwd_call(inner[i], out=P[i]) for i in range(1, L)], self.device)
+        self.outs[0].forward_lead(inner[0], [self.outs[i].fwd_call(inner[i], out=P[i]) for i in range(1, L)], out=P[0])
         if self.extra_p6:
             N, H, W, Cc = P[-1].shape
             P.append(dense.subsample2(P[-1], self._buf("P6", (N, (H + 1) // 2, (W + 1) // 2, Cc))))
@@ -53,9 +52,9 @@
         dinner = [self._buf("dinner%d" % i, self.inner[i].shape) for i in range(L)]
         for i in range(L):
             self.outs[i].backward_weight(self.inner[i], dP[i])
-        self.outs[0].backward_data(dP[0], self.inner[0].shape, out=dinner[0])
-        dense.conv2d_group("dgrad", [self.outs[i].dgrad_call(dP[i], self.inner[i].shape, out=dinner[i])
-                                     for i in range(1, L)], self.device)
+        self.outs[0].backward_data_lead(dP[0], self.inner[0].shape,
+                                        [self.outs[i].dgrad_call(dP[i], self.inner[i].shape, out=dinner[i]) for i in range(1, L)],
+                                        out=dinner[0])
         for i in range(1, L):
             dense.upsample2_backward(dinner[i - 1], dinner[i], accumulate=True)
         calls = []
diff --git a/mxdetection_amd/models/rpn_heads/rpn_head.py b/mxdetection_amd/models/rpn_heads/rpn_head.py
--- a/mxdetection_amd/models/rpn_heads/rpn_head.py
+++ b/mxdetection_amd/models/rpn_heads/rpn_head.py
@@ -81,9 +81,8 @@
         hb = [self._buf("h%d" % l, p.shape[:3] + (HEAD_CPAD,)) for l, p in enumerate(P)]
         self.tbits = [self._buf("tb%d" % l, p.shape[:3] + (p.shape[3] // 8,), dtype=torch.uint8) if RELU_BITS else None
                       for l, p in enumerate(P)]
-        self.conv.forward(P[0], relu=True, out=tb[0], bits_out=self.tbits[0])
-        dense.conv2d_group("fwd", [self.conv.fwd_call(P[l], relu=True, out=tb[l], bits_out=self.tbits[l])
-                                   for l in range(1, len(P))], self.device)
+        self.conv.forward_lead(P[0], [self.conv.fwd_call(P[l], relu=True, out=tb[l], bits_out=self.tbits[l])
+                                      for l in range(1, len(P))], relu=True, out=tb[0], bits_out=self.tbits[0])
         self.out.forward(tb[0], out=hb[0])
         dense.conv2d_group("fwd", [self.out.fwd_call(tb[l], out=hb[l]) for l in range(1, len(P))], self.device)
         self.t, self.h = tb, hb
diff --git a/mxdetection_amd/models/utils/layers.py b/mxdetection_amd/models/utils/layers.py
--- a/mxdetection_amd/models/utils/layers.py
+++ b/mxdetection_amd/models/utils/layers.py
@@ -172,11 +172,22 @@
         if self.trainable:
             dense.filter_transpose(self.w_bf16, self.wt)
 
-    def forward(self, x, relu=False, residual=None, res_upsample=False, out=None, bits_out=None):
+    def forward(self, x, relu=False, residual=None, res_upsample=False, out=None, bits_out=None, bulk_only=False):
         if dense.PF_TRACE is not None:
             dense.PF_TRACE.append((self, "f", dense.mem_range(self.w_bf16), None))
         return dense.conv2d_forward(x, self.w_bf16, self.bias_f32, residual, self.stride, self.pad, relu, res_upsample,
-                                    out, prefetch=self.pf_fwd, bits_out=bits_out)
+                                    out, prefetch=self.pf_fwd, bits_out=bits_out, **({"bulk_only": True} if bulk_only else {}))
+
+    def forward_lead(self, x, others, relu=False, out=None, bits_out=None):
+        dense.conv2d_lead_group("fwd", self.fwd_call(x, relu=relu, out=out, bits_out=bits_out),
+                                lambda **kw: self.forward(x, relu=relu, out=out, bits_out=bits_out, **kw), others, self.device)
+        return out
+
+    def backward_data_lead(self, dy, x_shape, others, accumulate=False, out=None):
+        dense.conv2d_lead_group("dgrad", self.dgrad_call(dy, x_shape, accumulate=accumulate, out=out),
+                                lambda **kw: self.backward_data(dy, x_shape, accumulate=accumulate, out=out, **kw), others,
+                                self.device)
+        return out
 
     def fwd_call(self, x, relu=False, residual=None, res_upsample=False, out=None, bits_out=None):
         t = (x, self.w_bf16, self.bias_f32, residual, self.stride, self.pad, relu, res_upsample, out)
@@ -186,12 +197,13 @@
         t = (dy, self.wt, tuple(x_shape), self.k, self.k, self.stride, self.pad, residual, relu_mask, accumulate, out)
         return t if relu_bits is None else t + (relu_bits,)
 
-    def backward_data(self, dy, x_shape, residual=None, relu_mask=None, accumulate=False, out=None, relu_bits=None):
+    def backward_data(self, dy, x_shape, residual=None, relu_mask=None, accumulate=False, out=None, relu_bits=None,
+                      bulk_only=False):
         if dense.PF_TRACE is not None:
             dense.PF_TRACE.append((self, "b", dense.mem_range(self.wt), None))
         return dense.conv2d_dgrad(dy, self.wt, x_shape, self.k, self.k, self.stride, self.pad, residual,
                                   None if relu_bits is not None else relu_mask, accumulate, out, prefetch=self.pf_bwd,
-                                  relu_bits=relu_bits)
+                                  relu_bits=relu_bits, **({"bulk_only": True} if bulk_only else {}))
 
     def backward_weight(self, x, dy, accumulate=False):
         if self.ws.grouping and not accumulate:
diff --git a/mxdetection_amd/ops/dense.py b/mxdetection_amd/ops/dense.py
--- a/mxdetection_amd/ops/dense.py
+++ b/mxdetection_amd/ops/dense.py
@@ -20,8 +20,11 @@
 
 
 def conv_desc(N, H, W, Cin, Cout, KH, KW, stride, pad, relu=False, res_upsample=False, accumulate=False, prefetch=None,
-              relu_bits=None):
+              relu_bits=None, rows=None, bulk_only=False):
     d = ConvDescT()
+    if rows is not None:
+        d.row_begin, d.row_end = rows
+    d.bulk_only = int(bulk_only)
     if relu_bits is not None:
         d.relu_bits = relu_bits.data_ptr()
     if prefetch is not None:
@@ -34,11 +37,12 @@
 
 
 def conv2d_forward(x, w, bias=None, residual=None, stride=1, pad=0, relu=False, res_upsample=False, out=None, prefetch=None,
-                   bits_out=None):
+                   bits_out=None, bulk_only=False):
     lib = _lib.load()
     N, H, W, Cin = x.shape
     Cout, KH, KW, _ = w.shape
-    d = conv_desc(N, H, W, Cin, Cout, KH, KW, stride, pad, relu, res_upsample, prefetch=prefetch, relu_bits=bits_out)
+    d = conv_desc(N, H, W, Cin, Cout, KH, KW, stride, pad, relu, res_upsample, prefetch=prefetch, relu_bits=bits_out,
+                  bulk_only=bulk_only)
     if out is None:
         out = torch.empty((N, d.Ho, d.Wo, Cout), dtype=torch.bfloat16, device=x.device)
     check(lib.mxdet_conv2d_fwd(C.byref(d), ptr(x), ptr(w), ptr(bias), ptr(residual), ptr(out), stream_ptr()),
@@ -78,12 +82,12 @@
 
 
 def conv2d_dgrad(dy, wt, x_shape, KH, KW, stride=1, pad=0, residual=None, relu_mask=None, accumulate=False, out=None,
-                 prefetch=None, relu_bits=None):
+                 prefetch=None, relu_bits=None, bulk_only=False):
     lib = _lib.load()
     N, H, W, Cin = x_shape
     Cout = dy.shape[3]
     d = conv_desc(N, H, W, Cin, Cout, KH, KW, stride, pad, relu=(relu_mask is not None or relu_bits is not None),
-                  accumulate=accumulate, prefetch=prefetch, relu_bits=relu_bits)
+                  accumulate=accumulate, prefetch=prefetch, relu_bits=relu_bits, bulk_only=bulk_only)
     if out is None:
         out = torch.empty(tuple(x_shape), dtype=torch.bfloat16, device=dy.device)
     check(lib.mxdet_conv2d_dgrad(C.byref(d), ptr(dy), ptr(wt), ptr(residual), ptr(relu_mask), ptr(out), stream_ptr()),
@@ -125,23 +129,28 @@
             if self.kind == 0:
                 x, w, bias, residual, stride, pad, relu, res_up, out = c[:9]
                 bits = c[9] if len(c) > 9 else None
+                rows = c[10] if len(c) > 10 else None
                 N, H, W, Cin = x.shape
                 Cout, KH, KW, _ = w.shape
-                it.desc = conv_desc(N, H, W, Cin, Cout, KH, KW, stride, pad, relu, res_up, prefetch=hint, relu_bits=bits)
+                it.desc = conv_desc(N, H, W, Cin, Cout, KH, KW, stride, pad, relu, res_up, prefetch=hint, relu_bits=bits,
+                                    rows=rows)
                 hint = None
                 it.src, it.filt, it.bias, it.residual, it.relu_mask, it.dst = dp(x), dp(w), dp(bias), dp(residual), None, dp(out)
-                self.flops += 2.0 * N * it.desc.Ho * it.desc.Wo * Cout * KH * KW * Cin
+                if rows is None:
+                    self.flops += 2.0 * N * it.desc.Ho * it.desc.Wo * Cout * KH * KW * Cin
             else:
                 dy, wt, x_shape, KH, KW, stride, pad, residual, relu_mask, accumulate, out = c[:11]
                 bits = c[11] if len(c) > 11 else None
+                rows = c[12] if len(c) > 12 else None
                 N, H, W, Cin = x_shape
                 Cout = dy.shape[3]
                 it.desc = conv_desc(N, H, W, Cin, Cout, KH, KW, stride, pad, relu=(relu_mask is not None or bits is not None),
-                                    accumulate=accumulate, prefetch=hint, relu_bits=bits)
+                                    accumulate=accumulate, prefetch=hint, relu_bits=bits, rows=rows)
                 hint = None
                 it.src, it.filt, it.bias, it.residual, it.relu_mask, it.dst = (dp(dy), dp(wt), None, dp(residual),
                                                                               None if bits is not None else dp(relu_mask), dp(out))
-                self.flops += 2.0 * N * dy.shape[1] * dy.shape[2] * Cout * KH * KW * Cin
+                if rows is None:
+                    self.flops += 2.0 * N * dy.shape[1] * dy.shape[2] * Cout * KH * KW * Cin
         nbytes = lib.mxdet_conv2d_grouped_table_bytes(n)
         host = (C.c_ubyte * nbytes)()
         cfg, grid = C.c_int32(0), C.c_int32(0)
@@ -162,8 +171,44 @@
 GROUP_HINTS = {}
 
 
+def _group_key(kind, calls):
+    return (kind,) + tuple(tuple(t.data_ptr() if torch.is_tensor(t) else t for t in c) for c in calls)
+
+
+def _call_dims(kind, c):
+    if kind == "fwd":
+        (N, H, W, Cin), (Cout, KH, KW, _), stride, pad = c[0].shape, c[1].shape, c[4], c[5]
+        return (N, H, W, Cin, Cout, KH, KW, stride, pad), N * ((H + 2 * pad - KH) // stride + 1) * ((W + 2 * pad - KW) // stride + 1)
+    (N, H, W, Cin), Cout, KH, KW, stride, pad = c[2], c[0].shape[3], c[3], c[4], c[5], c[6]
+    return (N, H, W, Cin, Cout, KH, KW, stride, pad), N * H * W
+
+
+def bulk_rows(kind, call):
+    dims, _ = _call_dims(kind, call)
+    return int(_lib.load().mxdet_conv2d_bulk_rows(C.byref(conv_desc(*dims)), 0 if kind == "fwd" else 1))
+
+
+def ranged_call(kind, call, rows):
+    n = 10 if kind == "fwd" else 12
+    return tuple(call) + (None,) * (n - len(call)) + (tuple(rows),)
+
+
+def conv2d_lead_group(kind, lead, single, others, device):
+    dims, M = _call_dims(kind, lead)
+    b = bulk_rows(kind, lead) if others else 0
+    if 0 < b < M:
+        calls = [ranged_call(kind, lead, (b, M))] + list(others)
+        if _group_key(kind, calls) in _group_plans or not torch.cuda.is_current_stream_capturing():
+            single(bulk_only=True)
+            conv2d_group(kind, calls, device)
+            return
+    single()
+    if others:
+        conv2d_group(kind, others, device)
+
+
 def conv2d_group(kind, calls, device):
-    key = (kind,) + tuple(tuple(t.data_ptr() if torch.is_tensor(t) else t for t in c) for c in calls)
+    key = _group_key(kind, calls)
     if PF_TRACE is not None and calls:
         PF_TRACE.append((None, "g", mem_range(*[c[1] for c in calls]), key if len(calls) > 1 else None))
     if len(calls) == 1:
@@ -177,6 +222,8 @@
         plan.launch()
         return
     for c in calls:
+        if len(c) > (10 if kind == "fwd" else 12) and c[-1] is not None:
+            raise _lib.MxdetError("conv2d_group: a ranged item needs its group plan (first seen under stream capture)")
         if kind == "fwd":
             x, w, bias, residual, stride, pad, relu, res_up, out = c[:9]
             conv2d_forward(x, w, bias, residual, stride, pad, relu, res_up, out, bits_out=c[9] if len(c) > 9 else None)
@@ -308,6 +355,7 @@
     return dcoarse
 
 
+
 def pixel_shuffle2_inv_relu(dy_up, act, out=None):
     R, H, W, C4 = act.shape
     if out is None:
```

Result: no change. 464.4 images/sec, median of 6 (+0.8%).
